# ma921/SOBER

Hardware: AMD Instinct MI355X
Metric: recombination-step candidates/sec (N_rec=100000, N_nys=500, d=10, batch=100) (higher is better)
Workload: dtype f64

## Files before the change

include/sober_hip.h:

```cpp
#ifndef SOBER_HIP_H
#define SOBER_HIP_H

#include <stdint.h>

#ifdef __cplusplus
extern "C" {
#endif

#define SOBER_ABI_VERSION 7

#define SOBER_KIND_RBF       0
#define SOBER_KIND_MATERN52  1
#define SOBER_KIND_TANIMOTO  2

#define SOBER_E_ARG      -1
#define SOBER_E_DIM      -2
#define SOBER_E_WS       -3
#define SOBER_E_EXCHANGE -5

int sober_abi_version(void);
int sober_diag_build(void);
int sober_reload_switches(void);
int sober_level_job_size(void);
int sober_nystrom_job_size(void);

int sober_padded_dim(int d);
int sober_bit_words(int d);

int sober_mt19937_uniform53(uint8_t* state, int64_t state_bytes, int64_t numel, double* out);
int sober_box_muller(const double* u, int64_t numel, double* out, void* stream);

int sober_scale_points(const double* X, int64_t n, int d, int64_t ldx,
                       const double* lengthscale, int ls_len,
                       double* out, int dt, void* stream);

int sober_scale_points_idx(const double* X, const int32_t* idx, int64_t n, int d, int64_t ldx, const double* lengthscale,
                           int ls_len, double* out, int dt, const double* gather_src, double* gather_out, void* stream);
int sober_pack_bits(const double* X, int64_t n, int d, int64_t ldx,
                    uint64_t* words, int nwords, double* norms, int32_t* bad_flag, void* stream);

int sober_pairwise(int kind, const void* a, const double* a_norm, int64_t m,
                   const void* b, const double* b_norm, const int32_t* idx, int64_t n,
                   int dt, double outputscale, double* out, int64_t ldo, void* stream);

int sober_kernel_matvec(int kind, const void* a, const double* a_norm, const double* v, int64_t m,
                        const void* b, const double* b_norm, int64_t n,
                        int dt, double outputscale, double c0, double* out, void* stream);

int sober_level_reduce(int kind, const void* rows, const double* rows_norm, int n_rows,
                       const void* cand, const double* cand_norm, int dt,
                       const int32_t* idx, int64_t pos0, int64_t count, int S,
                       const double* mu, const double* wmul, double outputscale,
                       int n_chunks, double* partG, int ldg, int col0,
                       double* partTot, int64_t tot_limit, void* stream);
int sober_aug_dim(int d);
int sober_augment_plan(const double* X_nys, int64_t M, int64_t ld_nys, const double* X_obs, int64_t n_obs, int64_t ld_obs,
                       const double* X_cand, int64_t N, int64_t ld_cand, int d, const double* lengthscale, int ls_len,
                       double* center, double* rows_aug, double* cand_aug, int da, void* stream);
int sober_augment_points(const double* X, int64_t n, int d, int64_t ldx, const double* lengthscale,
                         int ls_len, const double* center, int side, double* out, int da, void* stream);
int sober_level_reduce_mfma(int kind, const double* rows, int n_rows, const double* cand, int da,
                            const int32_t* idx, int64_t pos0, int64_t count, int S,
                            const double* mu, const double* wmul, double outputscale,
                            int n_chunks, double* partG, int ldg, int col0,
                            double* partTot, int64_t tot_limit, void* stream);

int64_t sober_nonzero_ws_bytes(int64_t N);
int sober_nonzero_i32(const double* mu, int64_t N, int32_t* idx_out, int64_t* count_out, void* ws, int64_t ws_bytes,
                      void* stream);

int sober_level_chunks(int n_rows, int64_t pos0, int64_t count, int S);
int sober_level_parts_mfma(int n_rows, int64_t pos0, int64_t count, int S);
int sober_level_parts_mfma_cap(int n_rows, int64_t e_total_ub, int S);

int sober_sum_partials(const double* partG, const double* partTot, int n_chunks, int n_rows,
                       int ldg, int S, const double* extraG, const double* extraTot,
                       int n_xchunks, int n_xcols, double* G, int ldo, double* tot, void* stream);

int sober_dgemm(int transa, int transb, int m, int n, int k, double alpha,
                const double* A, int lda, const double* B, int ldb,
                double beta, double* C, int ldc, void* stream);

int sober_barycentres(const double* Xtr, int ldx, int n, int S, const double* tot,
                      double* X_tmp, void* stream);
int sober_dgemm_coldiv_t(int m, int n, int k, const double* A, int lda, const double* B, int ldb, const double* coldiv,
                         double* Ct, int ldct, void* stream);

int sober_level_update(const int32_t* idx_cur, int64_t pos0, int64_t count, int S, int64_t E,
                       const int32_t* keep_rank, const double* w_star, const double* tot,
                       int n_keep, double* mu, int32_t* idx_new, int64_t new_pos0, void* stream);

int sober_scatter_weights(const int32_t* idx_cur, const int32_t* sel, const double* w, int n_sel,
                          double* mu, int64_t* out_idx, void* stream);

int sober_gather_f64(const double* src, const int32_t* idx, int64_t n, double* out, void* stream);
int sober_final_scatter(const int32_t* idx, int n, const int32_t* keep_rank, const double* w_star,
                        int64_t row_offset, double* mu, int64_t* out_idx, double* out_w, void* stream);
int sober_final_commit(const int32_t* idx, int n, const int32_t* keep_rank, const double* w_star, const int32_t* n_keep,
                       int64_t row_offset, double* mu, int64_t N, int64_t* out_idx, double* out_w, void* stream);

int sober_i64_to_i32(const int64_t* in, int64_t n, int32_t* out, void* stream);

int sober_car_pivot_host(double* h_Phi, int N, int m, double* h_mu);
int sober_car_pivot_host_fast(double* h_Phi, int N, int m, double* h_mu);

int sober_car_supported(int N, int m);
int64_t sober_car_ws_bytes(int N, int m);
int sober_car_device(const double* X, int ldx, int N, int m, const double* mu_in,
                     int32_t* keep_rank, double* w_star, int32_t* n_keep, double* mu_out,
                     double* phi_out, void* ws, int64_t ws_bytes, void* stream);
int sober_probe_rcp(const double* x, double* out, int64_t n, void* stream);

#define SOBER_CAR_DEFAULT 0
#define SOBER_CAR_SAFE 1
int sober_car_safe_supported(int N, int m);
int sober_car_giveup_forced(void);
int sober_car_device_ex(const double* X, int ldx, int N, int m, const double* mu_in,
                        int32_t* keep_rank, double* w_star, int32_t* n_keep, double* mu_out,
                        double* phi_out, void* ws, int64_t ws_bytes, int mode, void* stream);
int sober_obj_set_sums(const double* obj, const double* mu, const int32_t* idx, int64_t pos0, int64_t count, int S, int64_t E,
                       double* out, void* stream);
int sober_second_elimination(const double* phi, const double* objp, const double* w1, const int32_t* rank1, int n1,
                             int Nsets, int32_t* keep_rank, double* w_star, int32_t* n_keep, void* stream);
int sober_null_vector_supported(int nfun);
int sober_null_vector(const double* X, int ldx, int Nsets, int nfun, const int32_t* rank1, const int32_t* n_keep1, int n1,
                      double* null_row, int32_t* status, void* stream);
int sober_second_elimination_rows(const double* null_row, const double* obj_row, const double* w1, const int32_t* rank1,
                                  const int32_t* n_keep1, const int32_t* status, int n1, int Nsets, int32_t* keep_rank,
                                  double* w_star, int32_t* n_keep, void* stream);
int sober_obj_set_sums_queued(const double* obj, const double* mu, const int32_t* idx, int S, const int64_t* dR, int64_t R_known,
                              const double* tot, double* xcol, int ldx, double* ocol, void* stream);

int sober_car_mc_supported(int N, int m);
int64_t sober_car_mc_ws_bytes(int N, int m);
int sober_car_mc_device(const double* X, int ldx, int N, int m, const double* mu_in,
                        int32_t* keep_rank, double* w_star, int32_t* n_keep, double* mu_out,
                        double* phi_out, void* ws, int64_t ws_bytes, void* stream);
int sober_car_big_supported(int N, int m);
int64_t sober_car_big_ws_bytes(int N, int m);
int sober_car_big_device(const double* X, int ldx, int N, int m, const double* mu_in,
                         int32_t* keep_rank, double* w_star, int32_t* n_keep, double* mu_out,
                         double* phi_out, void* ws, int64_t ws_bytes, void* stream);
int sober_mc_selftest(const double* in, double* out, void* stream);

int sober_chol_max_n(void);
int sober_nystrom_max_n(void);
int sober_cholesky_probe_batched(const double* src, int n, int ld_src, const double* shifts, int n_shifts,
                                 double* work, int32_t* info, double* min_pivot, void* xinv_ws, int64_t ws_bytes,
                                 void* stream);
int sober_cholesky(double* A, int n, int ld, double shift, int32_t* info, double* min_pivot, void* stream);
int sober_cholesky_inv(double* A, int n, int ld, double shift, int32_t* info, double* min_pivot, double* xinv,
                       void* stream);
int sober_cholesky_inv_ratio(double* A, int n, int ld, double shift, int32_t* info, double* min_pivot, double* xinv,
                             double* ratio_out, void* stream);
int sober_trsm_blocks(const double* Y, int64_t m, int q, int ldy, const double* L, int ldl, const double* Xinv,
                      double* Q, int ldq, void* stream);
int sober_cholesky_probe(const double* src, int n, int ld_src, const double* shifts, int n_shifts,
                         double* work, int32_t* info, void* stream);
int sober_cholesky_probe_piv(const double* src, int n, int ld_src, const double* shifts, int n_shifts,
                             double* work, int32_t* info, double* min_pivot, void* stream);

int64_t sober_cholesky_probe_mc_ws_bytes(int n, int n_shifts);
int sober_cholesky_probe_mc(const double* src, int n, int ld_src, const double* shifts, int n_shifts,
                            double* work, int32_t* info, double* min_pivot, void* ws, int64_t ws_bytes,
// ... 235 lines not shown
```

sober_amd/_engine.py:

```python
from __future__ import annotations

import os
import time
import warnings
from typing import Optional

import numpy as np
import torch

from . import _native as nat
from ._utils import SafeTensorOperator


class SoloComm:
    rank, world = 0, 1

    def allreduce_sum(self, *tensors):
        return

    def allgather_counts(self, n: int):
        return [n]

    def allgather_rows(self, t: torch.Tensor, counts):
        return t
# ... 165 lines not shown
    ES = E * S
    if p <= ES:
        return (p // S) * n_keep + kept_prefix[p % S]
    return E * n_keep + ((p - ES) if last_kept else 0)


class RecombinationEngine:
    def __init__(self, ops, comm=None, row_offset: int = 0):
        self.ops = ops
        self.comm = comm or SoloComm()
        self.row_offset = int(row_offset)
        self.tm = SafeTensorOperator()
        self.trace = None
        self.timers = {}
        self.force_host_car = False
        self.force_host_nystrom = False
        self.basis_override = None
        self.cutover_R = int(os.environ.get("SOBER_CUTOVER_R", "32768"))
        self.force_sharded = bool(os.environ.get("SOBER_FORCE_SHARDED"))

    def _tick(self, name, t0):
        t1 = time.perf_counter()
        self.timers[name] = self.timers.get(name, 0.0) + (t1 - t0)
        return t1

    def nystrom_basis(self, plan, s: int, overlap=None, literal=False, early=None):
        if self.basis_override is not None:
            return self.basis_override
        t0 = time.perf_counter()
        dev_route = getattr(self.ops, "nystrom_basis_device", None)
        if dev_route is not None and not self.force_host_nystrom and not literal:
            res = dev_route(plan, s, self.tm.max_iter, overlap, early) if (overlap is not None or early is not None) \
                else dev_route(plan, s, self.tm.max_iter)
            if res is not None:
                U, gram = res
                self._tick("nystrom_device", t0)
                if self.trace is not None:
                    (gram_h, U_h) = self.ops.to_host(gram, U)
                    self.trace.update(gram=gram_h, U=U_h)
                return U
        gram = self.ops.gram(plan)
        (gram_h,) = self.ops.to_host(gram)
        t0 = self._tick("gram_device", t0)
        _, U = ker_svd_sparsify_host(gram_h, s, self.tm)
        self._tick("nystrom_host", t0)
        if self.trace is not None:
            self.trace.update(gram=gram_h.clone(), U=U.clone())
        return U

    def run(self, plan, mu: torch.Tensor, num_pts: int, obj: Optional[torch.Tensor] = None, live=None):
        ops, comm = self.ops, self.comm
        self.obj = obj
        self.obj_head = None
        if obj is not None:
            head = obj[:2 * num_pts].clone()
            if comm.world > 1:
                cnt = comm.allgather_counts(int(head.numel()))
                head = comm.allgather_rows(head, cnt)[:2 * num_pts]
            self.obj_head = head
        n = num_pts - 1
        S = 2 * (n + 1)
        state = {}
        can_start = getattr(ops, "nonzero_start", None) is not None and live is None
        pend = {}

        def start_list():
            if can_start and "p" not in pend:
                pend["p"] = ops.nonzero_start(mu)
        sharded = comm.world > 1 or (self.force_sharded and getattr(comm, "native_allreduce", None) is not None)

        def first_sums():
            if live is not None:
                idx_cur, count = live, int(live.numel())
            else:
                start_list()
                idx_cur, count = ops.nonzero_finish(pend["p"]) if "p" in pend else ops.nonzero_i32(mu)
            counts = comm.allgather_counts(count)
            bounds = [0]
            for c in counts:
                bounds.append(bounds[-1] + c)
            state.update(idx_cur=idx_cur, count=count, pos0=bounds[comm.rank], R=bounds[-1], bounds=bounds)
            cut = sharded and obj is None and self.cutover_R > 0 and state["R"] <= self.cutover_R
            if state["R"] > S and getattr(ops, "level_car", None) is not None and count > 0 and not cut:
                ops.level_moments(plan, idx_cur, state["pos0"], count, S, state["R"] // S, mu, phase=1, n=n)
                state["sums_ready"] = True

        def head_once():
            if not state:
                first_sums()

        n_fun = n + 1 + (1 if obj is not None else 0)
        car_on_host = self.force_host_car or getattr(ops, "car_supported", None) is None \
            or not ops.car_supported(S, n_fun) or (obj is not None and getattr(ops, "car_obj_device", None) is None)
        if car_on_host and not self.force_host_car and getattr(ops, "size_cliff", None) is not None \
                and getattr(ops, "car_supported", None) is not None and not ops.car_supported(S, n_fun):
            ops.size_cliff("car", f"batch = {n + 1}: a Caratheodory step on 2 x batch = {S} points with {n_fun} test functions is beyond "
                                  "the device kernels (registers of one compute unit: batch <= 100, of nine: batch <= 224, memory-resident: "
                                  "2 x batch <= 2048); every level's step runs on host LAPACK + the C++ pivots instead -- seconds per level")
        if comm.world > 1:
            start_list()
        U = self.nystrom_basis(plan, n, overlap=head_once if comm.world == 1 else None, literal=car_on_host,
                               early=start_list if comm.world == 1 else None)
        if comm.world > 1:
            U = comm.broadcast0(ops.from_host(U.contiguous()) if U.device != ops.device else U.contiguous())
            if hasattr(plan, "_proj_src"):
                plan._proj_src = None
        ops.set_projection(plan, U)
        head_once()
        idx_cur, count, pos0, R = state["idx_cur"], state["count"], state["pos0"], state["R"]
        bounds = state["bounds"]
        sums_ready = state.get("sums_ready", False)
        idx_new = ops.empty_i32(count)
        levels = [] if self.trace is not None else None

        if self.trace is not None:
            self.trace["levels"] = levels
        if not sharded and obj is None and levels is None and not self.force_host_car and R > S \
                and getattr(ops, "level_loop", None) is not None and ops.car_supported(S, n + 1):
            t0 = time.perf_counter()
            idx_cur, idx_new, R = ops.level_loop(plan, idx_cur, idx_new, R, S, mu, sums_ready, self.row_offset)
            pos0, count, bounds, sums_ready = 0, R, [0, R], False
            self._tick("levels_device", t0)
        elif not sharded and obj is not None and levels is None and not self.force_host_car and R > S \
                and getattr(ops, "level_loop_obj", None) is not None:
            t0 = time.perf_counter()
            res = ops.level_loop_obj(plan, idx_cur, idx_new, R, S, mu, obj, sums_ready)
            if res is not None and res[3] > 0:
                idx_cur, idx_new, R = res[:3]
                pos0, count, bounds, sums_ready = 0, R, [0, R], False
            self._tick("levels_device", t0)
        elif sharded and obj is None and levels is None and not self.force_host_car and R > S \
                and getattr(ops, "level_loop_sharded", None) is not None and ops.car_supported(S, n + 1) \
                and getattr(comm, "native_allreduce", None) is not None:
            t0 = time.perf_counter()
            idx_cur, idx_new, bounds = ops.level_loop_sharded(plan, idx_cur, idx_new, bounds, S, mu, sums_ready, comm,
                                                              self.cutover_R)
            R, pos0, count, sums_ready = bounds[-1], bounds[comm.rank], bounds[comm.rank + 1] - bounds[comm.rank], False
            self._tick("levels_device", t0)
            if R > S:
                return self._finish_replicated(plan, idx_cur, bounds, mu, num_pts, U)
        while True:
            if R <= n + 1:
                return self._finish_small(mu)
            if R <= S:
                return self._finish_direct(plan, idx_cur, bounds, R, mu, levels)

            E = R // S
            r = R - E * S
            t0 = time.perf_counter()
            if sums_ready:
                Xtr, tot = ops.level_moments(plan, idx_cur, pos0, count, S, E, mu, phase=2)
                sums_ready = False
            else:
                Xtr, tot = ops.level_moments(plan, idx_cur, pos0, count, S, E, mu)
            if obj is None:
                flat = getattr(ops, "level_flat", None)
                if flat is not None:
                    comm.allreduce_sum(flat(plan))
                else:
                    comm.allreduce_sum(Xtr, tot)
            else:
                orow = self._obj_set_sums(obj, mu, idx_cur, pos0, count, S, E)
                comm.allreduce_sum(Xtr, tot, orow)
                Xtr = torch.cat([Xtr, orow.unsqueeze(0)], 0)
            if obj is None and not self.force_host_car and getattr(ops, "level_car", None) is not None \
                    and ops.car_supported(S, n + 1):
                res = ops.level_car(plan, S)
# ... 169 lines not shown
```

sober_amd/_native.py:

```python
from __future__ import annotations

import ctypes as C
import os
from typing import Optional

import torch

_HERE = os.path.dirname(os.path.abspath(__file__))
LIB_PATH = os.environ.get("SOBER_HIP_LIB") or os.path.join(_HERE, "libsober_hip.so")
ABI_VERSION = 7

KIND_RBF, KIND_MATERN52, KIND_TANIMOTO = 0, 1, 2
KIND_BY_NAME = {"rbf": KIND_RBF, "matern52": KIND_MATERN52, "tanimoto": KIND_TANIMOTO}

_vp, _i32, _i64, _f64 = C.c_void_p, C.c_int, C.c_int64, C.c_double

SIGNATURES = {
    "sober_abi_version": (_i32, []),
    "sober_diag_build": (_i32, []),
    "sober_reload_switches": (_i32, []),
    "sober_level_job_size": (_i32, []),
    "sober_nystrom_job_size": (_i32, []),
    "sober_final_job_size": (_i32, []),
    "sober_set_i64": (_i32, [_vp, _i64, _vp]),
    "sober_rank_scatter": (_i32, [_vp, _i32, _i32, _i32, _vp, _vp, _i32, _vp, _vp, _vp]),
    "sober_plan_rows": (_i32, [_i32, _vp, _i32, _i64, _vp, _i32, _i64, _i32, _vp, _i32, _f64, _vp, _i32, _vp, _i32, _vp,
                               _vp, _vp, _vp, _vp]),
    "sober_level_loop_final": (_i32, [_vp, _vp, _i64, _vp, _vp, _i32, _vp, _i32, _vp, _vp, _vp, _vp, _vp]),
    "sober_padded_dim": (_i32, [_i32]),
    "sober_bit_words": (_i32, [_i32]),
    "sober_scale_points": (_i32, [_vp, _i64, _i32, _i64, _vp, _i32, _vp, _i32, _vp]),
    "sober_augment_plan": (_i32, [_vp, _i64, _i64, _vp, _i64, _i64, _vp, _i64, _i64, _i32, _vp, _i32, _vp, _vp, _vp, _i32, _vp]),
    "sober_scale_points_idx": (_i32, [_vp, _vp, _i64, _i32, _i64, _vp, _i32, _vp, _i32, _vp, _vp, _vp]),
    "sober_pack_bits": (_i32, [_vp, _i64, _i32, _i64, _vp, _i32, _vp, _vp, _vp]),
    "sober_mt19937_uniform53": (_i32, [_vp, _i64, _i64, _vp]),
    "sober_box_muller": (_i32, [_vp, _i64, _vp, _vp]),
    "sober_pairwise": (_i32, [_i32, _vp, _vp, _i64, _vp, _vp, _vp, _i64, _i32, _f64, _vp, _i64, _vp]),
    "sober_kernel_matvec": (_i32, [_i32, _vp, _vp, _vp, _i64, _vp, _vp, _i64, _i32, _f64, _f64, _vp, _vp]),
    "sober_level_reduce": (_i32, [_i32, _vp, _vp, _i32, _vp, _vp, _i32, _vp, _i64, _i64, _i32, _vp, _vp,
                                  _f64, _i32, _vp, _i32, _i32, _vp, _i64, _vp]),
    "sober_nonzero_ws_bytes": (_i64, [_i64]),
    "sober_nonzero_i32": (_i32, [_vp, _i64, _vp, _vp, _vp, _i64, _vp]),
    "sober_dgemm_coldiv_t": (_i32, [_i32, _i32, _i32, _vp, _i32, _vp, _i32, _vp, _vp, _i32, _vp]),
    "sober_level_chunks": (_i32, [_i32, _i64, _i64, _i32]),
    "sober_level_parts_mfma": (_i32, [_i32, _i64, _i64, _i32]),
    "sober_level_parts_mfma_cap": (_i32, [_i32, _i64, _i32]),
    "sober_aug_dim": (_i32, [_i32]),
    "sober_augment_points": (_i32, [_vp, _i64, _i32, _i64, _vp, _i32, _vp, _i32, _vp, _i32, _vp]),
    "sober_level_reduce_mfma": (_i32, [_i32, _vp, _i32, _vp, _i32, _vp, _i64, _i64, _i32, _vp, _vp, _f64, _i32,
                                       _vp, _i32, _i32, _vp, _i64, _vp]),
    "sober_sum_partials": (_i32, [_vp, _vp, _i32, _i32, _i32, _i32, _vp, _vp, _i32, _i32, _vp, _i32, _vp, _vp]),
    "sober_dgemm": (_i32, [_i32, _i32, _i32, _i32, _i32, _f64, _vp, _i32, _vp, _i32, _f64, _vp, _i32, _vp]),
    "sober_barycentres": (_i32, [_vp, _i32, _i32, _i32, _vp, _vp, _vp]),
    "sober_level_update": (_i32, [_vp, _i64, _i64, _i32, _i64, _vp, _vp, _vp, _i32, _vp, _vp, _i64, _vp]),
    "sober_scatter_weights": (_i32, [_vp, _vp, _vp, _i32, _vp, _vp, _vp]),
    "sober_i64_to_i32": (_i32, [_vp, _i64, _vp, _vp]),
    "sober_car_pivot_host": (_i32, [_vp, _i32, _i32, _vp]),
    "sober_car_pivot_host_fast": (_i32, [_vp, _i32, _i32, _vp]),
    "sober_car_supported": (_i32, [_i32, _i32]),
    "sober_car_ws_bytes": (_i64, [_i32, _i32]),
    "sober_car_device": (_i32, [_vp, _i32, _i32, _i32, _vp, _vp, _vp, _vp, _vp, _vp, _vp, _i64, _vp]),
    "sober_probe_rcp": (_i32, [_vp, _vp, _i64, _vp]),
    "sober_second_elimination": (_i32, [_vp, _vp, _vp, _vp, _i32, _i32, _vp, _vp, _vp, _vp]),
    "sober_car_mc_supported": (_i32, [_i32, _i32]),
    "sober_car_mc_ws_bytes": (_i64, [_i32, _i32]),
    "sober_car_mc_device": (_i32, [_vp, _i32, _i32, _i32, _vp, _vp, _vp, _vp, _vp, _vp, _vp, _i64, _vp]),
    "sober_car_big_supported": (_i32, [_i32, _i32]),
    "sober_car_big_ws_bytes": (_i64, [_i32, _i32]),
    "sober_car_big_device": (_i32, [_vp, _i32, _i32, _i32, _vp, _vp, _vp, _vp, _vp, _vp, _vp, _i64, _vp]),
    "sober_car_device_ex": (_i32, [_vp, _i32, _i32, _i32, _vp, _vp, _vp, _vp, _vp, _vp, _vp, _i64, _i32, _vp]),
    "sober_obj_set_sums": (_i32, [_vp, _vp, _vp, _i64, _i64, _i32, _i64, _vp, _vp]),
    "sober_null_vector_supported": (_i32, [_i32]),
    "sober_null_vector": (_i32, [_vp, _i32, _i32, _i32, _vp, _vp, _i32, _vp, _vp, _vp]),
    "sober_second_elimination_rows": (_i32, [_vp, _vp, _vp, _vp, _vp, _vp, _i32, _i32, _vp, _vp, _vp, _vp]),
    "sober_obj_set_sums_queued": (_i32, [_vp, _vp, _vp, _i32, _vp, _i64, _vp, _vp, _i32, _vp, _vp]),
    "sober_obj_job_size": (_i32, []),
    "sober_level_loop_obj": (_i32, [_vp, _vp, _i64, _vp, _vp, _i32, _i32, _vp, _vp, _vp, _vp, _vp]),
    "sober_car_safe_supported": (_i32, [_i32, _i32]),
    "sober_car_giveup_forced": (_i32, []),
    "sober_final_commit": (_i32, [_vp, _i32, _vp, _vp, _vp, _i64, _vp, _i64, _vp, _vp, _vp]),
    "sober_level_car_retry": (_i32, [_vp, _vp]),
    "sober_mc_selftest": (_i32, [_vp, _vp, _vp]),
    "sober_chol_max_n": (_i32, []),
    "sober_nystrom_max_n": (_i32, []),
    "sober_cholesky_probe_batched": (_i32, [_vp, _i32, _i32, _vp, _i32, _vp, _vp, _vp, _vp, _i64, _vp]),
    "sober_cholesky": (_i32, [_vp, _i32, _i32, _f64, _vp, _vp, _vp]),
    "sober_cholesky_inv": (_i32, [_vp, _i32, _i32, _f64, _vp, _vp, _vp, _vp]),
    "sober_cholesky_inv_ratio": (_i32, [_vp, _i32, _i32, _f64, _vp, _vp, _vp, _vp, _vp]),
    "sober_trsm_blocks": (_i32, [_vp, _i64, _i32, _i32, _vp, _i32, _vp, _vp, _i32, _vp]),
    "sober_cholesky_probe": (_i32, [_vp, _i32, _i32, _vp, _i32, _vp, _vp, _vp]),
    "sober_cholesky_probe_piv": (_i32, [_vp, _i32, _i32, _vp, _i32, _vp, _vp, _vp, _vp]),
    "sober_cholesky_probe_mc_ws_bytes": (_i64, [_i32, _i32]),
    "sober_cholesky_probe_mc": (_i32, [_vp, _i32, _i32, _vp, _i32, _vp, _vp, _vp, _vp, _i64, _vp]),
    "sober_abs_sym": (_i32, [_vp, _i32, _i32, _vp, _i32, _vp, _vp]),
    "sober_abs_sym_dmax": (_i32, [_vp, _i32, _i32, _vp, _i32, _vp, _vp, _vp]),
    "sober_jitter_ladder": (_i32, [_vp, _i32, _i32, _i32, _vp]),
    "sober_jitter_ladder_auto": (_i32, [_vp, _i32, _i32, _vp, _i32, _vp, _vp]),
    "sober_kmeans_ws_bytes": (_i64, [_i64, _i32, _i32]),
    "sober_kmeans_stat_offset": (_i64, [_i64, _i32, _i32]),
    "sober_kmeans_ws_bytes_screened": (_i64, [_i64, _i32, _i32]),
    "sober_kmeans_lloyd": (_i32, [_vp, _i64, _i32, _i32, _i32, _vp, _vp, _vp, _i64, _vp]),
    "sober_predict_fused_supported": (_i32, [_i32, _i32, _i32]),
    "sober_predict_fused": (_i32, [_i32, _vp, _vp, _i32, _vp, _vp, _i64, _i32, _f64, _vp, _i32, _vp, _f64, _f64, _f64, _vp, _vp,
                                   _f64, _vp, _vp, _i32, _vp]),
    "sober_predict_fused_root": (_i32, [_i32, _vp, _vp, _i32, _vp, _vp, _i64, _i32, _f64, _vp, _i32, _vp, _vp, _f64, _f64, _f64, _vp,
                                        _vp, _f64, _vp, _vp, _i32, _vp]),
    "sober_predict_finish": (_i32, [_vp, _vp, _i32, _i64, _i64, _vp, _f64, _vp, _f64, _f64, _vp, _f64, _vp, _i32, _vp]),
    "sober_reduce_ws_bytes": (_i64, [_i64]),
    "sober_cleansing_weights": (_i32, [_vp, _i64, _f64, _vp, _i64, _vp]),
    "sober_level_gather": (_i32, [_vp, _i32, _i64, _vp, _i64, _i64, _i32, _vp, _vp, _i32, _vp, _i32, _i32, _vp, _i64,
                                  _vp]),
    "sober_gspace_finish": (_i32, [_vp, _vp, _i64, _i32, _i64, _i64, _vp, _vp, _vp]),
    "sober_wkde_draw": (_i32, [_vp, _i64, _i32, _vp, _vp, _i32, _vp, _vp, _vp, _vp, _vp, _vp]),
    "sober_level_moments": (_i32, [_vp, _vp]),
    "sober_level_car": (_i32, [_vp, _vp]),
    "sober_level_reduce_tani_supported": (_i32, [_i32]),
    "sober_level_reduce_tani": (_i32, [_vp, _vp, _i32, _vp, _vp, _i32, _vp, _i64, _i64, _i32, _vp, _vp, _f64, _i32, _vp,
                                       _i32, _i32, _vp, _i64, _vp]),
    "sober_level_loop_sharded": (_i32, [_vp, _i32, _i32, _vp, _vp, _vp, _i32, _vp, _vp, _i64, _i32, _vp, _vp, _vp, _vp]),
    "sober_rccl_load": (_i32, [C.c_char_p]),
    "sober_rccl_unique_id": (_i32, [_vp]),
    "sober_rccl_comm_init": (_i32, [_vp, _i32, _i32, _vp]),
    "sober_rccl_comm_destroy": (_i32, [_vp]),
    "sober_rccl_allreduce_f64": (_i32, [_vp, _vp, _i64, _vp]),
    "sober_rccl_allreduce_ptr": (_i64, []),
    "sober_peer_region_bytes": (_i64, [_i64]),
    "sober_peer_create": (_i32, [_i32, _i32, _i64, _vp, _vp]),
    "sober_peer_connect": (_i32, [_vp, C.c_char_p]),
    "sober_peer_connect_ptrs": (_i32, [_vp, _vp]),
    "sober_peer_region": (_i64, [_vp]),
    "sober_peer_set_spin_limit": (_i32, [_vp, C.c_uint]),
    "sober_peer_allreduce_f64": (_i32, [_vp, _vp, _i64, _vp]),
    "sober_peer_allreduce_ptr": (_i64, []),
    "sober_peer_status": (_i32, [_vp, _vp, _i64, _vp]),
    "sober_peer_destroy": (_i32, [_vp]),
# ... 175 lines not shown

def fused_dim_supported(kind: int, d: int) -> bool:
    r = load().sober_bit_words(d) if kind == KIND_TANIMOTO else load().sober_padded_dim(d)
    return r > 0


def scale_points_idx(X, idx, n, lengthscale, out):
    _req(lengthscale, torch.float64, "lengthscale"); _req(out, torch.float64, "out"); _req(idx, torch.int32, "idx")
    if X.dtype != torch.float64 or X.stride(-1) != 1:
        raise SoberHipError("scale_points_idx: X must be float64 with unit inner stride")
    _check(load().sober_scale_points_idx(X.data_ptr(), idx.data_ptr(), int(n), X.shape[1], X.stride(0), lengthscale.data_ptr(),
                                         lengthscale.numel(), out.data_ptr(), out.shape[1], None, None, _stream(X)),
           "sober_scale_points_idx")


def scale_points(X, lengthscale, out):
    n, d = X.shape
    _req(X, torch.float64, "X"); _req(lengthscale, torch.float64, "lengthscale"); _req(out, torch.float64, "out")
    _check(load().sober_scale_points(X.data_ptr(), n, d, X.stride(0), lengthscale.data_ptr(),
                                     lengthscale.numel(), out.data_ptr(), out.shape[1], _stream(X)),
           "sober_scale_points")


def mt19937_uniform53(state, numel, out):
    _req(state, torch.uint8, "state"); _req(out, torch.float64, "out")
    if state.is_cuda or out.is_cuda or out.numel() < numel + 16:
        raise ValueError("mt19937_uniform53 takes host tensors, out of numel + 16 doubles")
    _check(load().sober_mt19937_uniform53(state.data_ptr(), state.numel(), numel, out.data_ptr()),
           "sober_mt19937_uniform53")


def box_muller(u, numel, out):
    _req(u, torch.float64, "u"); _req(out, torch.float64, "out")
    if u.numel() < numel + 16 or out.numel() < numel:
        raise ValueError("box_muller: u holds numel + 16 uniforms, out numel normals")
    _check(load().sober_box_muller(u.data_ptr(), numel, out.data_ptr(), _stream(out)), "sober_box_muller")


def pack_bits(X, words, norms, bad_flag):
    n, d = X.shape
    _req(X, torch.float64, "X"); _req(words, torch.int64, "words"); _req(norms, torch.float64, "norms")
    _req(bad_flag, torch.int32, "bad_flag")
    _check(load().sober_pack_bits(X.data_ptr(), n, d, X.stride(0), words.data_ptr(), words.shape[1],
                                  norms.data_ptr(), bad_flag.data_ptr(), _stream(X)), "sober_pack_bits")


def rank_scatter(X, n, ocol, rank, n1, Xp, objp):
    _req(X, torch.float64, "X"); _req(ocol, torch.float64, "ocol"); _req(rank, torch.int32, "rank")
    _check(load().sober_rank_scatter(X.data_ptr(), X.stride(0), X.shape[0], n, ocol.data_ptr(), rank.data_ptr(), n1,
                                     Xp.data_ptr(), objp.data_ptr(), _stream(X)), "sober_rank_scatter")


def plan_rows(kind, X_nys, X_obs, lengthscale, outputscale, S_cache, rows, Kall, W, T, G):
    M, d = X_nys.shape
    n_obs = 0 if X_obs is None else X_obs.shape[0]
    for t in (X_nys, X_obs, S_cache, rows, Kall, W, T, G):
        if t is not None and (t.dtype != torch.float64 or t.stride(-1) != 1):
            raise SoberHipError("plan_rows: float64 tensors with unit inner stride")
    _check(load().sober_plan_rows(kind, X_nys.data_ptr(), M, X_nys.stride(0), _ptr(X_obs), n_obs,
                                  X_obs.stride(0) if X_obs is not None else 0, d, lengthscale.data_ptr(),
                                  lengthscale.numel(), float(outputscale), _ptr(S_cache),
                                  S_cache.stride(0) if S_cache is not None else 0, rows.data_ptr(), rows.shape[1],
                                  _ptr(Kall), _ptr(W), _ptr(T), G.data_ptr(), _stream(G)), "sober_plan_rows")


def pairwise(kind, a, a_norm, b, b_norm, idx, n, dt, outputscale, out):
    _check(load().sober_pairwise(kind, a.data_ptr(), _ptr(a_norm), a.shape[0], b.data_ptr(), _ptr(b_norm),
                                 _ptr(idx), n, dt, float(outputscale), out.data_ptr(), out.stride(0),
                                 _stream(out)), "sober_pairwise")


def kernel_matvec(kind, a, a_norm, v, b, b_norm, dt, outputscale, c0, out):
    _check(load().sober_kernel_matvec(kind, a.data_ptr(), _ptr(a_norm), v.data_ptr(), a.shape[0],
                                      b.data_ptr(), _ptr(b_norm), b.shape[0], dt, float(outputscale),
                                      float(c0), out.data_ptr(), _stream(out)), "sober_kernel_matvec")


def nonzero_ws_bytes(N) -> int:
    r = load().sober_nonzero_ws_bytes(N)
    _check(min(int(r), 0), "sober_nonzero_ws_bytes")
    return int(r)


def nonzero_i32(mu, idx_out, count_out, ws):
    _req(mu, torch.float64, "mu"); _req(idx_out, torch.int32, "idx_out"); _req(count_out, torch.int64, "count_out")
    _check(load().sober_nonzero_i32(mu.data_ptr(), mu.numel(), idx_out.data_ptr(), count_out.data_ptr(), ws.data_ptr(),
                                    ws.numel() * ws.element_size(), _stream(mu)), "sober_nonzero_i32")


def level_chunks(n_rows, pos0, count, S) -> int:
    r = load().sober_level_chunks(n_rows, pos0, count, S)
    _check(min(r, 0), "sober_level_chunks")
    return r


def level_parts_mfma(n_rows, pos0, count, S) -> int:
    r = load().sober_level_parts_mfma(n_rows, pos0, count, S)
    _check(min(r, 0), "sober_level_parts_mfma")
    return r


def level_reduce(kind, rows, rows_norm, cand, cand_norm, dt, idx, idx_off, pos0, count, S, mu, wmul,
                 outputscale, n_chunks, partG, ldg, col0, partTot, tot_limit):
    _req(idx, torch.int32, "idx"); _req(mu, torch.float64, "mu")
    _check(load().sober_level_reduce(kind, rows.data_ptr(), _ptr(rows_norm), rows.shape[0], cand.data_ptr(),
                                     _ptr(cand_norm), dt, idx.data_ptr() + 4 * idx_off, pos0, count, S,
                                     mu.data_ptr(), _ptr(wmul), float(outputscale), n_chunks,
                                     partG.data_ptr(), ldg, col0, _ptr(partTot), tot_limit, _stream(mu)),
           "sober_level_reduce")


def aug_dim(d: int) -> int:
    r = load().sober_aug_dim(d)
    return r if r > 0 else -1


def augment_plan(X_nys, X_obs, X_cand, lengthscale, center, rows_aug, cand_aug):
    for t_, nm in ((X_nys, "X_nys"), (X_cand, "X_cand"), (X_obs, "X_obs")):
        if t_ is not None and (t_.dtype != torch.float64 or t_.stride(-1) != 1):
            raise SoberHipError(f"augment_plan: {nm} must be float64 with unit inner stride")
    _req(rows_aug, torch.float64, "rows_aug"); _req(cand_aug, torch.float64, "cand_aug"); _req(center, torch.float64, "center")
    n_obs = 0 if X_obs is None else X_obs.shape[0]
    _check(load().sober_augment_plan(X_nys.data_ptr(), X_nys.shape[0], X_nys.stride(0), _ptr(X_obs), n_obs,
                                     X_obs.stride(0) if n_obs else 0, X_cand.data_ptr(), X_cand.shape[0], X_cand.stride(0),
                                     X_nys.shape[1], lengthscale.data_ptr(), lengthscale.numel(), center.data_ptr(),
                                     rows_aug.data_ptr(), cand_aug.data_ptr(), rows_aug.shape[1], _stream(X_cand)),
           "sober_augment_plan")


def augment_points(X, lengthscale, center, side, out):
    n, d = X.shape
    _req(X, torch.float64, "X"); _req(out, torch.float64, "out"); _req(center, torch.float64, "center")
    _check(load().sober_augment_points(X.data_ptr(), n, d, X.stride(0), lengthscale.data_ptr(),
                                       lengthscale.numel(), center.data_ptr(), side, out.data_ptr(),
                                       out.shape[1], _stream(X)), "sober_augment_points")


def level_reduce_mfma(kind, rows, cand, da, idx, idx_off, pos0, count, S, mu, wmul, outputscale, n_chunks,
                      partG, ldg, col0, partTot, tot_limit):
    _req(idx, torch.int32, "idx"); _req(mu, torch.float64, "mu")
    _check(load().sober_level_reduce_mfma(kind, rows.data_ptr(), rows.shape[0], cand.data_ptr(), da,
                                          idx.data_ptr() + 4 * idx_off, pos0, count, S, mu.data_ptr(),
                                          _ptr(wmul), float(outputscale), n_chunks, partG.data_ptr(), ldg,
                                          col0, _ptr(partTot), tot_limit, _stream(mu)),
           "sober_level_reduce_mfma")


def sum_partials(partG, partTot, n_chunks, n_rows, ldg, S, extraG, extraTot, n_xchunks, n_xcols, G, tot):
    _check(load().sober_sum_partials(partG.data_ptr(), _ptr(partTot), n_chunks, n_rows, ldg, S,
                                     _ptr(extraG), _ptr(extraTot), n_xchunks, n_xcols, G.data_ptr(),
                                     G.stride(0), _ptr(tot), _stream(G)), "sober_sum_partials")


def dgemm(A, B, C_, transa=False, transb=False, alpha=1.0, beta=0.0):
    m, n = C_.shape
    k = A.shape[0] if transa else A.shape[1]
    for t, nm in ((A, "A"), (B, "B"), (C_, "C")):
        if t.dtype != torch.float64 or t.stride(1) != 1:
            raise SoberHipError(f"dgemm {nm}: need float64 with unit inner stride")
    ka = B.shape[1] if transb else B.shape[0]
    ma = A.shape[1] if transa else A.shape[0]
    na = B.shape[0] if transb else B.shape[1]
    if (ma, na, ka) != (m, n, k):
        raise SoberHipError(f"dgemm shape mismatch {A.shape} {B.shape} -> {C_.shape}")
    _check(load().sober_dgemm(int(transa), int(transb), m, n, k, float(alpha), A.data_ptr(), A.stride(0),
                              B.data_ptr(), B.stride(0), float(beta), C_.data_ptr(), C_.stride(0),
                              _stream(C_)), "sober_dgemm")


def barycentres(Xtr, n, S, tot, X_tmp):
# ... 456 lines not shown
```

sober_amd/_ops_hip.py:

```python
from __future__ import annotations

import os
import warnings

import torch

from . import _native as nat
from ._ops_levels import _LevelOps
from ._ops_nystrom import _NystromOps
from ._ops_plan import Plan, _PlanOps


class HipOps(_PlanOps, _NystromOps, _LevelOps):
    name = "hip"

    def __init__(self, device):
        self.device = torch.device(device)
        if self.device.type != "cuda":
            raise nat.SoberHipError("sober_amd needs a HIP device (torch device 'cuda'); got "
                                    f"{self.device}.  There is no CPU fallback.")
        nat.load()
        self._pin = {}
        self.prof = None
        self.use_mfma = True
        self.queue_levels = os.environ.get("SOBER_NO_QUEUE") is None
        self.level_classes = True
        self.obj_null_kernel = True
        self.queue_obj_levels = True
        self.lazy_scaled_pool = True
        self.last_levels = None
        self._probe_mc = torch.cuda.get_device_properties(self.device).multi_processor_count >= 256
        self.car_mode = nat.CAR_DEFAULT

    def size_cliff(self, which: str, message: str):
        seen = self.__dict__.setdefault("_cliffs_seen", set())
        if which not in seen:
            seen.add(which)
            import warnings
            warnings.warn("sober_amd: " + message, RuntimeWarning, stacklevel=3)

    def prof_reserve(self, n_pairs: int):
        pool = getattr(self, "_ev_pool", None)
        if pool is None:
            pool = self._ev_pool = []
        st = torch.cuda.current_stream(self.device)
        for _ in range(n_pairs):
            e0, e1 = torch.cuda.Event(enable_timing=True), torch.cuda.Event(enable_timing=True)
            e0.record(st); e1.record(st)
            pool.append((e0, e1))

    def _prof_pair(self):
        pool = getattr(self, "_ev_pool", None)
        if not pool:
            self.prof_reserve(1)
            pool = self._ev_pool
        return pool.pop()

    def _buf(self, p, name, numel):
        t = p.ws.get(name)
        if t is None or t.numel() < numel:
            t = torch.empty(numel, dtype=torch.float64, device=self.device)
            p.ws[name] = t
        return t

    def _buf_u8(self, p, name, nbytes):
        t = p.ws.get(name)
        if t is None or t.numel() < nbytes:
            t = torch.empty(max(nbytes, 8), dtype=torch.uint8, device=self.device)
            p.ws[name] = t
        return t

    def nonzero_start(self, mu):
        N = mu.numel()
        key = ("nz", N)
        bufs = self._pin.get(key)
        if bufs is None:
            ws = torch.zeros(nat.nonzero_ws_bytes(N), dtype=torch.uint8, device=self.device)
            bufs = self._pin[key] = (ws, torch.zeros(1, dtype=torch.int64, device=self.device),
                                     torch.zeros(1, dtype=torch.int64).pin_memory())
        ws, cnt, pin = bufs
        out = torch.empty(N, dtype=torch.int32, device=self.device)
        nat.nonzero_i32(mu, out, cnt, ws)
        pin.copy_(cnt, non_blocking=True)
        ev = torch.cuda.Event()
        ev.record(torch.cuda.current_stream(self.device))
        return out, pin, ev

    def nonzero_finish(self, pending):
        out, pin, ev = pending
        ev.synchronize()
        return out, int(pin[0])

    def nonzero_i32(self, mu):
        nz = torch.nonzero(mu != 0).flatten()
        out = torch.empty(max(nz.numel(), 1), dtype=torch.int32, device=self.device)
        if nz.numel():
            nat.i64_to_i32(nz, out)
        return out, int(nz.numel())

    def empty_i32(self, n):
        return torch.empty(max(n, 1), dtype=torch.int32, device=self.device)

    def to_host(self, *tensors, before_sync=None):
        outs = []
        for i, t in enumerate(tensors):
            key = (i, t.dtype, tuple(t.shape))
            buf = self._pin.get(key)
            if buf is None:
                buf = torch.empty(t.shape, dtype=t.dtype, pin_memory=True)
                self._pin[key] = buf
            buf.copy_(t, non_blocking=True)
            outs.append(buf)
        if before_sync is None:
            torch.cuda.current_stream(self.device).synchronize()
        else:
            ev = torch.cuda.Event()
            ev.record(torch.cuda.current_stream(self.device))
            before_sync()
            ev.synchronize()
        return [o.clone() for o in outs]

    def from_host(self, t, dtype=None):
        return t.to(self.device, dtype=dtype, non_blocking=False)


class MatrixKernelOps(HipOps):

    CHUNK_ROWS = 1 << 15

    def build_plan(self, kernel_fn, mode, X_nys, X_cand, pool_owner=None) -> Plan:
        p = Plan()
        p.kernel_fn, p.mode = kernel_fn, "matrix"
        p.X_nys, p.X_cand = X_nys, X_cand
        p.M = p.Mtot = X_nys.shape[0]
        p.weighted, p.T, p.P, p.wmul, p.da = False, None, None, None, -1
        p.ws = {}
        N = X_cand.shape[0]
        if hasattr(kernel_fn, "materialise"):
            p.Kmat = kernel_fn.materialise(X_cand, X_nys)
        else:
            p.Kmat = torch.empty(N, p.M, dtype=torch.float64, device=self.device)
            for lo in range(0, N, self.CHUNK_ROWS):
                hi = min(N, lo + self.CHUNK_ROWS)
                p.Kmat[lo:hi] = kernel_fn(X_nys, X_cand[lo:hi]).to(torch.float64).T
        if tuple(p.Kmat.shape) != (N, p.M) or p.Kmat.dtype != torch.float64 or p.Kmat.stride(1) != 1:
            raise nat.SoberHipError(f"kernel matrix must be ({N}, {p.M}) float64 row-major, got "
                                    f"{tuple(p.Kmat.shape)} {p.Kmat.dtype}")
        return p

    def gram(self, p):
        if hasattr(p.kernel_fn, "materialise"):
            return p.kernel_fn.materialise(p.X_nys, p.X_nys, gram=True)
        return p.kernel_fn(p.X_nys, p.X_nys).to(torch.float64).contiguous()

    def set_projection(self, p, U):
        p.P = U.to(self.device, torch.float64).contiguous()
        p.n = p.P.shape[0]

    def direct_columns(self, p, idx, count):
        Kc = p.Kmat[idx[:count].long()].contiguous()
        Xtr = torch.empty(p.n, count, dtype=torch.float64, device=self.device)
        nat.dgemm(p.P, Kc, Xtr, transb=True)
        out = torch.empty(count, p.n, dtype=torch.float64, device=self.device)
        nat.barycentres(Xtr, p.n, count, None, out)
        return out

# ... 3 lines not shown
```

sober_amd/_ops_levels.py:

```python
from __future__ import annotations

import warnings

import torch

from . import _native as nat
from ._ops_plan import Plan


class _LevelOps:

    def _job(self, p: Plan, S: int, n: int = None) -> nat.LevelJob:
        n = p.n if n is None else n
        job = p.ws.get("job")
        if job is not None and job.S == S and job.n == n:
            if p.P is not None and job.P != p.P.data_ptr():
                if p.P.stride(0) != p.Mtot or p.P.stride(1) != 1:
                    p.P = p.P.contiguous()
                job.P = p.P.data_ptr()
            job.car_mode = min(self.car_mode, nat.CAR_SAFE)
            return job
        dev, f64 = self.device, torch.float64
        job = nat.LevelJob()
        Kmat = getattr(p, "Kmat", None)
        if Kmat is not None:
            job.variant, job.kind = nat.LEVEL_GATHER, 0
            job.cand, job.kmat_ld, job.n_rows = Kmat.data_ptr(), Kmat.stride(0), Kmat.shape[1]
            job.outputscale = 1.0
        elif p.da > 0:
            job.variant, job.kind = nat.LEVEL_MFMA, p.kind
            job.rows, job.cand, job.dim, job.n_rows = p.rows_aug.data_ptr(), p.cand_aug.data_ptr(), p.da, p.Mtot
            job.outputscale = float(p.spec.outputscale)
        else:
            tani = p.kind == nat.KIND_TANIMOTO and self.use_mfma and bool(nat.load().sober_level_reduce_tani_supported(p.rows.dt))
            job.variant, job.kind = (nat.LEVEL_TANI if tani else nat.LEVEL_VALU), p.kind
            job.rows, job.rows_norm = p.rows.data.data_ptr(), nat._ptr(p.rows.norm)
            job.cand, job.cand_norm = p.cand.data.data_ptr(), nat._ptr(p.cand.norm)
            job.dim, job.n_rows = p.rows.dt, p.Mtot
            job.outputscale = float(p.spec.outputscale)
        job.wmul = nat._ptr(p.wmul)
        if p.P is not None and (p.P.stride(0) != p.Mtot or p.P.stride(1) != 1):
            p.P = p.P.contiguous()
        job.S, job.n, job.P = S, n, nat._ptr(p.P)
        nr, mc, xs = job.n_rows, nat.LEVEL_MAX_CHUNKS, nat.LEVEL_XS
        w = p.ws
        w["partG"], w["partTot"] = torch.empty(mc * nr * S, dtype=f64, device=dev), torch.empty(mc * S, dtype=f64, device=dev)
        w["extraG"], w["extraTot"] = torch.empty(mc * nr * xs, dtype=f64, device=dev), torch.empty(mc * xs, dtype=f64, device=dev)
        w["G"] = torch.empty(nr, S, dtype=f64, device=dev)
        w["XT"] = torch.empty(n * S + S, dtype=f64, device=dev)
        w["Xtr"], w["tot"] = w["XT"][:n * S].view(n, S), w["XT"][n * S:]
        w["X_tmp"] = torch.empty(S, n, dtype=f64, device=dev)
        w["keep_rank"] = torch.empty(S + 1, dtype=torch.int32, device=dev)
        w["w_star"], w["mu_out"] = torch.empty(S, dtype=f64, device=dev), torch.empty(S, dtype=f64, device=dev)
        w["h_flags"] = torch.empty(S + 1, dtype=torch.int32, pin_memory=True)
        w["h_flags_np"] = w["h_flags"].numpy()
        if job.variant in (nat.LEVEL_MFMA, nat.LEVEL_TANI) and self.queue_levels:
            w["dR"] = torch.empty(nat.LEVEL_QUEUE + 1, dtype=torch.int64, device=dev)
            w["h_dR"] = torch.zeros(nat.LEVEL_QUEUE + 1, dtype=torch.int64, pin_memory=True)
            job.dR, job.h_dR = w["dR"].data_ptr(), w["h_dR"].data_ptr()
            if S % 2 == 0:
                cl = 1 << nat.CLASS_MAX_DEPTH
                w["Gc"] = [torch.empty(nr * S * (cl >> k), dtype=f64, device=dev) for k in (0, 1)]
                w["totc"] = [torch.empty(S * (cl >> k), dtype=f64, device=dev) for k in (0, 1)]
                w["cls_scale"], w["cls_sof"] = torch.empty(S, dtype=f64, device=dev), torch.empty(S, dtype=torch.int32, device=dev)
                for k in (0, 1):
                    job.Gc[k], job.totc[k] = w["Gc"][k].data_ptr(), w["totc"][k].data_ptr()
                job.cls_scale, job.cls_sof = w["cls_scale"].data_ptr(), w["cls_sof"].data_ptr()
        for k in ("partG", "partTot", "extraG", "extraTot", "G", "Xtr", "tot", "X_tmp", "keep_rank", "w_star", "mu_out",
                  "h_flags"):
            setattr(job, k, w[k].data_ptr())
        if nat.car_supported(S, n + 1):
            nbytes = nat.car_ws_bytes(S, n + 1)
            w["car_ws"] = torch.empty(max(nbytes // 8, 1), dtype=f64, device=dev)
            job.car_ws, job.car_ws_bytes = w["car_ws"].data_ptr(), nbytes
        job.car_mode = min(self.car_mode, nat.CAR_SAFE)
        w["job"] = job
        return job

    def _car_downgrade(self, mode: int, why: str):
        if mode > self.car_mode:
            self.car_mode = mode
            warnings.warn("sober_amd: a multi-workgroup Caratheodory launch gave up waiting for its partner workgroups "
                          f"({why}); this and the following steps use "
                          + ("the kernels without such waits (one workgroup, or a launch per dependency beyond batch 100)" if mode == nat.CAR_SAFE
                             else "the host LAPACK route")
                          + " for that step -- same result, slower")

    def level_moments(self, p: Plan, idx, pos0, count, S, E, mu, phase: int = 0, n: int = None):
        job = self._job(p, S, n)
        job.phase = phase
        if count <= 0 and phase != 2:
            p.ws["XT"].zero_(); p.ws["G"].zero_()
            return p.ws["Xtr"], p.ws["tot"]
        if phase == 2:
            nat.level_moments(job, nat._stream(p.ws["G"]))
            return p.ws["Xtr"], p.ws["tot"]
        nat._req(idx, torch.int32, "idx"); nat._req(mu, torch.float64, "mu")
        job.idx, job.pos0, job.count, job.E, job.mu = idx.data_ptr(), pos0, count, E, mu.data_ptr()
        job.class_depth = 0
        if phase == 1 and pos0 == 0 and count == E * S and job.Gc[0] and job.dR and self.level_classes:
            job.class_depth = int(nat.load().sober_level_class_depth(job.variant, job.n_rows, count, S))
        pair = None
        if self.prof is not None:
            n_left = max(pos0 + count - max(pos0, E * S), 0)
            pair, pair2 = self._prof_pair(), (self._prof_pair() if n_left > 0 else None)
            job.ev[0], job.ev[1] = pair[0].cuda_event, pair[1].cuda_event
            job.ev[2], job.ev[3] = (pair2[0].cuda_event, pair2[1].cuda_event) if pair2 else (None, None)
        nat.level_moments(job, nat._stream(mu))
        if pair is not None:
            self.prof.append((pair[0], pair[1], int(count * job.n_rows), 1))
            if pair2 is not None:
                self.prof.append((pair2[0], pair2[1], int(n_left * job.n_rows), 1))
            for k in range(4):
                job.ev[k] = None
        return p.ws["Xtr"], p.ws["tot"]

    def level_loop_obj(self, p: Plan, idx_cur, idx_new, R: int, S: int, mu, obj, sums_ready: bool):
        job = self._job(p, S)
        n = job.n
        if not self.queue_obj_levels or not self.queue_levels or not job.dR or job.variant not in (nat.LEVEL_MFMA, nat.LEVEL_TANI):
            return None
        if self.car_mode == nat.CAR_HOST or not self.obj_null_kernel or not self.car_supported(S, n + 2) \
                or not bool(nat.load().sober_null_vector_supported(n)):
            return None
        nat._req(mu, torch.float64, "mu"); nat._req(idx_cur, torch.int32, "idx"); nat._req(idx_new, torch.int32, "idx")
        nat._req(obj, torch.float64, "obj")
        dev, f64, w = self.device, torch.float64, p.ws
        if "obj_job" not in w:
            oj = nat.ObjJob()
            w["obj_X"] = torch.empty(S, n + 1, dtype=f64, device=dev)
            w["obj_f"] = torch.empty(3, S, dtype=f64, device=dev)
            w["obj_i"] = torch.empty(S + 2, dtype=torch.int32, device=dev)
            nbytes = nat.car_ws_bytes(S, n + 2)
            w["obj_car_ws"] = (torch.empty(max(nbytes // 8, 1), dtype=f64, device=dev), nbytes)
            oj.X_tmp, oj.ocol, oj.w1, oj.null_row = (w["obj_X"].data_ptr(), w["obj_f"][0].data_ptr(), w["obj_f"][1].data_ptr(),
                                                       w["obj_f"][2].data_ptr())
            oj.kr1, oj.nk1, oj.status = w["obj_i"].data_ptr(), w["obj_i"][S:].data_ptr(), w["obj_i"][S + 1:].data_ptr()
            w["obj_job"] = oj
        oj = w["obj_job"]
        oj.obj = obj.data_ptr()
        job.mu = mu.data_ptr()
        saved = (job.car_ws, job.car_ws_bytes, job.class_depth)
        job.car_ws, job.car_ws_bytes, job.class_depth = w["obj_car_ws"][0].data_ptr(), w["obj_car_ws"][1], 0
        try:
            level_R, R_final, in_b = nat.level_loop_obj(job, oj, R, idx_cur, idx_new, sums_ready, nat._stream(mu))
        finally:
            job.car_ws, job.car_ws_bytes, job.class_depth = saved
        if in_b:
            idx_cur, idx_new = idx_new, idx_cur
        return idx_cur, idx_new, R_final, len(level_R)

    def level_loop(self, p: Plan, idx_cur, idx_new, R: int, S: int, mu, sums_ready: bool, row_offset: int = 0):
        import math
        job = self._job(p, S)
        nat._req(mu, torch.float64, "mu"); nat._req(idx_cur, torch.int32, "idx"); nat._req(idx_new, torch.int32, "idx")
        job.mu = mu.data_ptr()
        if not sums_ready:
            job.class_depth = 0
        events = pairs = None
        if self.prof is not None:
            n_max = min(nat.MAX_LEVELS, int(math.log2(max(R / S, 1.0))) + 3)
            pairs = [(self._prof_pair(), self._prof_pair()) for _ in range(n_max)]
            events = [None] * (4 * nat.MAX_LEVELS)
            for l, (a, b) in enumerate(pairs):
                events[4 * l:4 * l + 4] = [a[0].cuda_event, a[1].cuda_event, b[0].cuda_event, b[1].cuda_event]
        fin = None
        p.ws.pop("final_done", None)
        if not p.weighted and getattr(p, "Kmat", None) is None and self.car_mode != nat.CAR_HOST and job.car_ws:
            fin = self._final_job(p, S, mu, row_offset)
        level_R, R_final, in_b, gave_up = nat.level_loop(job, R, idx_cur, idx_new, sums_ready, events, nat._stream(mu), fin)
        self.last_levels = {"R": [int(v) for v in level_R], "derived": int(job.class_depth) if sums_ready else 0}
        if fin is not None and fin.done:
            n_keep = int(p.ws["h_flags_np"][S])
            if n_keep >= 0:
                lst = idx_new if in_b else idx_cur
                p.ws["final_done"] = (lst.data_ptr(), R_final, row_offset, p._fin_out[0][:n_keep], p._fin_out[1][:n_keep])
        if job.car_mode > min(self.car_mode, nat.CAR_SAFE):
            self._car_downgrade(nat.CAR_SAFE, "level loop")
        if gave_up:
            self._car_downgrade(nat.CAR_HOST, "level loop")
        if pairs is not None:
            for l, (a, b) in enumerate(pairs):
                Rl = level_R[l] if l < len(level_R) else 0
# ... 210 lines not shown
```

sober_amd/_ops_nystrom.py:

```python
from __future__ import annotations

import os
import warnings

import torch

from . import _native as nat
from . import _rng
from ._ops_plan import Plan


class _NystromOps:

    NITER = 2

    def nystrom_basis_device(self, p: Plan, s: int, max_iter: int = 10, overlap=None, early=None):
        dev, M = self.device, p.M
        if M > nat.nystrom_max_n() or s > 2 * nat.chol_max_n() or s >= M:
            if s < M:
                self.size_cliff("nystrom", f"N_nys = {M}, batch = {s + 1}: beyond the device Nystrom route (N_nys <= "
                                           f"{nat.nystrom_max_n()}, batch <= {2 * nat.chol_max_n() + 1}); make_cov_psd and svd_lowrank run on host LAPACK "
                                           "instead -- about 5-10x the device route's time for this phase")
            self.gram(p)
            return None
        G = self.gram(p)
        n_r, niter = max_iter + 1, self.NITER
        n_orth2 = 2 * (1 + 2 * niter)
        if getattr(p, "ws", None) is None:
            p.ws = {}
        key = ("nys", M, s, n_r)
        st = self._pin.get(key)
        if st is None:
            f64 = torch.float64
            nbytes = nat.nystrom_flags_bytes(n_r, niter)
            st = self._pin[key] = {
                "job": nat.NystromJob(), "C": torch.empty(M, M, dtype=f64, device=dev),
                "Y0": torch.empty(M, s, dtype=f64, device=dev), "Y1": torch.empty(M, s, dtype=f64, device=dev),
                "Gm": torch.empty(s, s, dtype=f64, device=dev),
                "xinv": torch.empty(((s + 31) // 32) * 1024, dtype=f64, device=dev),
                "flags": torch.empty(nbytes, dtype=torch.uint8, device=dev),
                "h_flags": torch.empty(nbytes, dtype=torch.uint8, pin_memory=True),
                "Ut": torch.empty(s, M, dtype=f64, device=dev),
            }
            skey = ("shifts", n_r)
            if skey not in self._pin:
                self._pin[skey] = torch.tensor([1e-5 * (2 ** k - 1) for k in range(n_r)], dtype=f64, device=dev)
            j = st["job"]
            j.M, j.s, j.n_rungs, j.niter = M, s, n_r, niter
            j.shifts, j.C = self._pin[skey].data_ptr(), st["C"].data_ptr()
            j.Y[0], j.Y[1], j.Gm, j.xinv = st["Y0"].data_ptr(), st["Y1"].data_ptr(), st["Gm"].data_ptr(), st["xinv"].data_ptr()
            j.flags_block, j.flags_bytes, j.h_flags_block = st["flags"].data_ptr(), nbytes, st["h_flags"].data_ptr()
            j.Ut = st["Ut"].data_ptr()
        j = st["job"]
        work = self._buf(p, "chol_work", n_r * M * M)
        j.G, j.chol_work = G.data_ptr(), work.data_ptr()
        j.probe_mc = 1 if (M >= self.PROBE_MC_MIN and n_r <= 16 and self._probe_mc and M <= nat.chol_max_n()) else 0
        if j.probe_mc:
            pws = self._buf_u8(p, "chol_mc_ws", nat.cholesky_probe_mc_ws_bytes(M, n_r))
            j.probe_ws, j.probe_ws_bytes = pws.data_ptr(), pws.numel()
        elif M > nat.chol_max_n():
            pws = self._buf_u8(p, "chol_cb_ws", n_r * 8192)
            j.probe_ws, j.probe_ws_bytes = pws.data_ptr(), pws.numel()
        proj = hasattr(p, "weighted")
        if proj:
            T = p.T
            P = torch.empty(s, p.Mtot if T is not None else M, dtype=torch.float64, device=dev)
            j.T, j.n_obs = nat._ptr(T), (T.shape[1] if T is not None else 0)
            j.mean_nys, j.P = (p.mean_nys.data_ptr() if p.weighted else None), P.data_ptr()
        else:
            j.P = None
        stream = torch.cuda.current_stream(dev)
        nat.nystrom_basis(j, 1, stream.cuda_stream)
        if early is not None:
            early()
        rng_state = torch.get_rng_state()
        R = _rng.device_randn(M, s, dev)
        j.R = R.data_ptr()
        nat.nystrom_basis(j, 2, stream.cuda_stream)
        ev = torch.cuda.Event()
        ev.record(stream)
        Ut = st["Ut"]
        if proj:
            p.P, p.n, p._proj_src = P, s, Ut
        if overlap is not None:
            overlap()
        ev.synchronize()
        hb = st["h_flags"]
        n8 = 8 * (n_r + 1 + n_orth2)
        f64s, i32s = hb[:n8].view(torch.float64), hb[n8:].view(torch.int32)
        piv_h, pivs_rf = f64s[:n_r + 1], f64s[n_r + 1:n_r + 1 + n_orth2]
        flags_h, infos_rf = i32s[:2 + n_r], i32s[2 + n_r:]
        if any(int(v) == nat.PROBE_NO_VERDICT for v in flags_h[2:]):
            self._probe_mc = False
            warnings.warn("sober_amd: the multi-CU Cholesky probe lost contact between its workgroups; "
                          "falling back to one workgroup per rung")
            torch.set_rng_state(rng_state)
            return None
        last = 2 * niter
        if os.environ.get("SOBER_NYSTROM_DEBUG"):
            print("nystrom: pivot ratios of the range finder's blocks", [float(pivs_rf[k + 1]) for k in range(0, n_orth2, 2)])
        single = [k for k in range(0, n_orth2, 2) if k // 2 != last]
        rank_lost = bool((infos_rf != 0).any()) or float(pivs_rf[2 * last + 1]) < 0.5 \
            or any(not (float(pivs_rf[k + 1]) >= self.ORTH1_MIN_RATIO) for k in single)
        if int(flags_h[0]) == 0 or rank_lost or self.ladder_borderline(flags_h[2:], piv_h[:n_r], float(piv_h[n_r])):
            torch.set_rng_state(rng_state)
            return None
        warnings.warn("Estimated covariance matrix was not positive semi-definite. Conveting...")
        return Ut, G

    LADDER_GUARD = 1e-9
    PROBE_MC_MIN = 160

    @classmethod
    def ladder_borderline(cls, info, min_pivot, dmax) -> bool:
        thr = cls.LADDER_GUARD * max(dmax, 0.0)
        ok = [int(v) == 0 for v in info]
        piv = [float(v) for v in min_pivot]
        if not (dmax == dmax) or any(v != v for v in piv):
            return True
        k = ok.index(True) if any(ok) else len(ok)
        if k < len(ok) and piv[k] < thr:
            return True
        if k > 0 and piv[k - 1] > -thr:
            return True
# ... 18 lines not shown
```

sober_amd/csrc/compact.hip:

```cpp
#include "common.hpp"

namespace sober {

constexpr int NZ_T = 256, NZ_PER = 8, NZ_TILE = NZ_T * NZ_PER;
constexpr unsigned long long NZ_LOCAL = 1ull << 32, NZ_INCL = 2ull << 32;

__device__ __forceinline__ int nz_wave_sum(int v) {
#pragma unroll
    for (int o = 32; o > 0; o >>= 1) v += __shfl_xor(v, o);
    return v;
}

__global__ __launch_bounds__(NZ_T) void k_nonzero(const double* __restrict__ mu, int64_t N, int32_t* __restrict__ out,
                                                  int64_t* __restrict__ count_out, unsigned long long* __restrict__ ws, int nb) {
    __shared__ int s_tile, s_total, s_prefix, s_last;
    __shared__ int s_cnt[NZ_PER * 4];
    if (threadIdx.x == 0) s_tile = (int)atomicAdd((unsigned*)ws, 1u);
    __syncthreads();
    const int tile = s_tile;
    const int lane = threadIdx.x & 63, w = threadIdx.x >> 6;
    const int64_t base = (int64_t)tile * NZ_TILE;
    unsigned long long m[NZ_PER];
#pragma unroll
    for (int k = 0; k < NZ_PER; ++k) {
        const int64_t i = base + k * NZ_T + threadIdx.x;
        const bool nz = i < N && mu[i] != 0.0;
        m[k] = __ballot(nz);
        if (lane == 0) s_cnt[k * 4 + w] = __popcll(m[k]);
    }
    __syncthreads();
    unsigned long long* status = ws + 2;
    if (w == 0) {
        const int v = lane < NZ_PER * 4 ? s_cnt[lane] : 0;
        int incl = v;
#pragma unroll
        for (int o = 1; o < NZ_PER * 4; o <<= 1) {
            const int u = __shfl_up(incl, o);
            if (lane >= o) incl += u;
        }
        if (lane < NZ_PER * 4) s_cnt[lane] = incl - v;
        const int total = __shfl(incl, NZ_PER * 4 - 1);
        int run = 0;
        if (tile == 0) {
            if (lane == 0) __hip_atomic_store(status, NZ_INCL | (unsigned long long)total, __ATOMIC_RELEASE, __HIP_MEMORY_SCOPE_AGENT);
        } else {
            if (lane == 0)
                __hip_atomic_store(status + tile, NZ_LOCAL | (unsigned long long)total, __ATOMIC_RELEASE, __HIP_MEMORY_SCOPE_AGENT);
            for (int p = tile - 1; p >= 0; p -= 64) {
                const int q = p - lane;
                unsigned long long st = 0;
                if (q >= 0) {
                    do st = __hip_atomic_load(status + q, __ATOMIC_RELAXED, __HIP_MEMORY_SCOPE_AGENT); while ((st >> 32) == 0);
                }
                const unsigned long long bi = __ballot(q >= 0 && (st >> 32) == 2);
                if (bi != 0) {
                    const int first = __ffsll((long long)bi) - 1;
                    run += nz_wave_sum(lane <= first ? (int)(unsigned)st : 0);
                    break;
                }
                run += nz_wave_sum(q >= 0 ? (int)(unsigned)st : 0);
            }
            if (lane == 0)
                __hip_atomic_store(status + tile, NZ_INCL | (unsigned long long)(run + total), __ATOMIC_RELEASE, __HIP_MEMORY_SCOPE_AGENT);
        }
        if (lane == 0) { s_prefix = run; s_total = total; }
    }
    __syncthreads();
    const int prefix = s_prefix;
#pragma unroll
    for (int k = 0; k < NZ_PER; ++k) {
        if ((m[k] >> lane) & 1ull)
            out[prefix + s_cnt[k * 4 + w] + __popcll(m[k] & ((1ull << lane) - 1ull))] = (int32_t)(base + k * NZ_T + threadIdx.x);
    }
    if (threadIdx.x == 0) {
        if (tile == nb - 1) *count_out = (int64_t)prefix + s_total;
        s_last = atomicAdd((unsigned*)(ws + 1), 1u) == (unsigned)(nb - 1);
    }
    __syncthreads();
    if (s_last)
        for (int t = threadIdx.x; t < nb + 2; t += NZ_T) ws[t] = 0ull;
}

}

extern "C" int64_t sober_nonzero_ws_bytes(int64_t N) {
    if (N <= 0 || N > 0x7fffffffLL) return SOBER_E_ARG;
    const int64_t nb = (N + sober::NZ_TILE - 1) / sober::NZ_TILE;
    return ((2 + nb) * 8 + 255) / 256 * 256;
}

extern "C" int sober_nonzero_i32(const double* mu, int64_t N, int32_t* idx_out, int64_t* count_out, void* ws,
                                 int64_t ws_bytes, void* stream) {
    if (!mu || !idx_out || !count_out || !ws || N <= 0 || N > 0x7fffffffLL) return SOBER_E_ARG;
    if (ws_bytes < sober_nonzero_ws_bytes(N)) return SOBER_E_WS;
    const int nb = (int)((N + sober::NZ_TILE - 1) / sober::NZ_TILE);
    hipLaunchKernelGGL(sober::k_nonzero, dim3((unsigned)nb), dim3(sober::NZ_T), 0, (hipStream_t)stream, mu, N, idx_out, count_out,
                       (unsigned long long*)ws, nb);
    LAUNCH_CHECK();
    return 0;
}
```

sober_amd/csrc/dgemm.hip:

```cpp
#include "common.hpp"

namespace sober {

typedef double double4_t __attribute__((ext_vector_type(4)));

__device__ __forceinline__ double ld_op(const double* M, int ld, int trans, int r, int c, int R, int C) {
    const bool ok = (r < R) & (c < C);
    const int rc = min(r, R - 1), cc = min(c, C - 1);
    const double v = trans ? M[(size_t)cc * ld + rc] : M[(size_t)rc * ld + cc];
    return ok ? v : 0.0;
}

template <int SPLIT>
__global__ __launch_bounds__(256) void k_dgemm(int transa, int transb, int m, int n, int k,
                                               double alpha, const double* __restrict__ A, int lda,
                                               const double* __restrict__ B, int ldb, double beta,
                                               double* __restrict__ C, int ldc,
                                               const double* __restrict__ coldiv, double* __restrict__ Ct, int ldct) {
    __shared__ double red[SPLIT == 4 ? 3 * 256 : 1];
    const int wave = threadIdx.x >> 6, lane = threadIdx.x & 63;
    int i0, j0, kbeg, kend;
    if constexpr (SPLIT == 4) {
        i0 = blockIdx.y * 16;
        j0 = blockIdx.x * 16;
        const int kq = (((k + 3) / 4) + 15) / 16 * 16;
        kbeg = min(wave * kq, k);
        kend = min(kbeg + kq, k);
    } else {
        i0 = blockIdx.y * 32 + (wave >> 1) * 16;
        j0 = blockIdx.x * 32 + (wave & 1) * 16;
        kbeg = 0;
        kend = k;
        if (i0 >= m || j0 >= n) return;
    }
    const int li = lane & 15, lk = lane >> 4;

    double4_t acc = (double4_t){0.0, 0.0, 0.0, 0.0};
    double af[4], bf[4], an[4], bn[4];
#define DG_LOAD(AF, BF, K0)                                                                   \
    _Pragma("unroll") for (int u = 0; u < 4; ++u) {                                           \
        AF[u] = ld_op(A, lda, transa, i0 + li, (K0) + 4 * u + lk, m, kend);                   \
        BF[u] = ld_op(B, ldb, transb, (K0) + 4 * u + lk, j0 + li, kend, n);                   \
    }
    DG_LOAD(af, bf, kbeg)
    for (int k0 = kbeg; k0 < kend; k0 += 16) {
        DG_LOAD(an, bn, k0 + 16)
#pragma unroll
        for (int u = 0; u < 4; ++u)
            acc = __builtin_amdgcn_mfma_f64_16x16x4f64(af[u], bf[u], acc, 0, 0, 0);
#pragma unroll
        for (int u = 0; u < 4; ++u) { af[u] = an[u]; bf[u] = bn[u]; }
    }
#undef DG_LOAD
    if constexpr (SPLIT == 4) {
        if (wave > 0) {
#pragma unroll
            for (int r = 0; r < 4; ++r) red[(wave - 1) * 256 + r * 64 + lane] = acc[r];
        }
        __syncthreads();
        if (wave > 0) return;
#pragma unroll
        for (int r = 0; r < 4; ++r) acc[r] = ((acc[r] + red[r * 64 + lane]) + red[256 + r * 64 + lane]) + red[512 + r * 64 + lane];
    }
#pragma unroll
    for (int r = 0; r < 4; ++r) {
        const int row = i0 + lk + 4 * r;
        const int col = j0 + li;
        if (row < m && col < n) {
            const double v = alpha * acc[r];
            if (Ct != nullptr) {
                Ct[(size_t)col * ldct + row] = coldiv ? v / coldiv[col] : v;
            } else {
                double* c = C + (size_t)row * ldc + col;
                *c = (beta == 0.0) ? v : fma(beta, *c, v);
            }
        }
    }
}

}

extern "C" int sober_dgemm(int transa, int transb, int m, int n, int k, double alpha, const double* A,
                           int lda, const double* B, int ldb, double beta, double* C, int ldc,
                           void* stream) {
    if (!A || !B || !C || m <= 0 || n <= 0 || k <= 0) return SOBER_E_ARG;
    if (lda < (transa ? m : k) || ldb < (transb ? k : n) || ldc < n) return SOBER_E_ARG;
    const long tiles = (long)((n + 15) / 16) * ((m + 15) / 16);
    if (tiles <= 2048 && k >= 64) {
        dim3 grid((n + 15) / 16, (m + 15) / 16);
        hipLaunchKernelGGL(sober::k_dgemm<4>, grid, dim3(256), 0, (hipStream_t)stream, transa, transb, m, n, k,
                           alpha, A, lda, B, ldb, beta, C, ldc, (const double*)nullptr, (double*)nullptr, 0);
    } else {
        dim3 grid((n + 31) / 32, (m + 31) / 32);
        hipLaunchKernelGGL(sober::k_dgemm<1>, grid, dim3(256), 0, (hipStream_t)stream, transa, transb, m, n, k,
                           alpha, A, lda, B, ldb, beta, C, ldc, (const double*)nullptr, (double*)nullptr, 0);
    }
    LAUNCH_CHECK();
    return 0;
}

extern "C" int sober_dgemm_coldiv_t(int m, int n, int k, const double* A, int lda, const double* B, int ldb,
                                    const double* coldiv, double* Ct, int ldct, void* stream) {
    if (!A || !B || !Ct || m <= 0 || n <= 0 || k <= 0 || lda < k || ldb < n || ldct < m) return SOBER_E_ARG;
    const long tiles = (long)((n + 15) / 16) * ((m + 15) / 16);
    if (tiles <= 2048 && k >= 64) {
        dim3 grid((n + 15) / 16, (m + 15) / 16);
        hipLaunchKernelGGL(sober::k_dgemm<4>, grid, dim3(256), 0, (hipStream_t)stream, 0, 0, m, n, k, 1.0, A, lda, B, ldb,
                           0.0, (double*)nullptr, 0, coldiv, Ct, ldct);
    } else {
        dim3 grid((n + 31) / 32, (m + 31) / 32);
        hipLaunchKernelGGL(sober::k_dgemm<1>, grid, dim3(256), 0, (hipStream_t)stream, 0, 0, m, n, k, 1.0, A, lda, B, ldb,
                           0.0, (double*)nullptr, 0, coldiv, Ct, ldct);
    }
    LAUNCH_CHECK();
    return 0;
}
```

sober_amd/csrc/internal.hpp:

```cpp
#pragma once
#include <cstdint>

namespace sober {

int scale_points2(const double* Xa, int64_t na, int64_t lda, const double* Xb, int64_t nb, int64_t ldb, int d,
                  const double* lengthscale, int ls_len, double* out, int dt, void* stream);

int transpose_projection(const double* Q, int s, int M, const double* mean, double* Ut, double* P, int ldp, void* stream);

int64_t probe_mc_flag_bytes(int n_shifts);
int nystrom_flags_init(void* flags_block, int64_t flags_bytes, void* probe_ws, int64_t ws_flag_bytes, int32_t* info,
                       int n_info, void* stream);
int cholesky_probe_mc(const double* src, int n, int ld_src, const double* shifts, int n_shifts, double* work, int32_t* info,
                      double* min_pivot, void* ws, int64_t ws_bytes, bool init, void* stream);

int orth_merge(int32_t* info, double* piv, double* ratio, const int32_t* info2, const double* piv2, const double* ratio2, void* stream);

}
```

sober_amd/csrc/level_exec.cpp:

```cpp
#include <hip/hip_runtime.h>
#include <cstdio>
#include <cstdlib>

#include "../../include/sober_hip.h"
#include "switches.hpp"

extern "C" int sober_level_job_size(void) { return (int)sizeof(sober_level_job); }
extern "C" int sober_obj_job_size(void) { return (int)sizeof(sober_obj_job); }

#define LX_TRY(call)                 \
    do {                             \
        const int rc_ = (call);      \
        if (rc_ != 0) return rc_;    \
    } while (0)

static inline bool lx_timed_in_dispatch(const sober_level_job* j) {
    return j->variant == SOBER_LEVEL_MFMA || j->variant == SOBER_LEVEL_TANI;
}
#define LX_EVENTS_BEFORE(A, B)                                                                   \
    if ((A) && (B)) {                                                                            \
        if (lx_timed_in_dispatch(j)) { LX_TRY(sober_set_launch_events((A), (B))); }              \
        else { const hipError_t e_ = hipEventRecord((hipEvent_t)(A), (hipStream_t)stream); if (e_ != hipSuccess) return (int)e_; } \
    }
#define LX_EVENTS_AFTER(A, B)                                                                    \
    if ((A) && (B) && !lx_timed_in_dispatch(j)) {                                                \
        const hipError_t e_ = hipEventRecord((hipEvent_t)(B), (hipStream_t)stream);              \
        if (e_ != hipSuccess) return (int)e_;                                                    \
    }

static int lx_reduce(const sober_level_job* j, const int32_t* idx, int64_t pos0, int64_t count, int S, int n_chunks,
                     double* partG, double* partTot, int64_t tot_limit, void* stream) {
    switch (j->variant) {
        case SOBER_LEVEL_MFMA:
            return sober_level_reduce_mfma(j->kind, (const double*)j->rows, j->n_rows, (const double*)j->cand, j->dim,
                                           idx, pos0, count, S, j->mu, j->wmul, j->outputscale, n_chunks, partG, S, 0,
                                           partTot, tot_limit, stream);
        case SOBER_LEVEL_VALU:
            return sober_level_reduce(j->kind, j->rows, j->rows_norm, j->n_rows, j->cand, j->cand_norm, j->dim, idx,
                                      pos0, count, S, j->mu, j->wmul, j->outputscale, n_chunks, partG, S, 0, partTot,
                                      tot_limit, stream);
        case SOBER_LEVEL_TANI:
            return sober_level_reduce_tani(j->rows, j->rows_norm, j->n_rows, j->cand, j->cand_norm, j->dim, idx, pos0, count,
                                           S, j->mu, j->wmul, j->outputscale, n_chunks, partG, S, 0, partTot, tot_limit,
                                           stream);
        case SOBER_LEVEL_GATHER:
            return sober_level_gather((const double*)j->cand, j->n_rows, j->kmat_ld, idx, pos0, count, S, j->mu,
                                      j->wmul, n_chunks, partG, S, 0, partTot, tot_limit, stream);
        default:
            return SOBER_E_ARG;
    }
}

extern "C" int sober_level_class_depth(int variant, int n_rows, int64_t R, int S) {
    if (n_rows <= 0 || R <= 0 || S <= 0 || (S & 1) || sober::switches().level_no_classes) return 0;
    if (variant != SOBER_LEVEL_MFMA && variant != SOBER_LEVEL_TANI) return 0;
    int D = 0;
    while (D < SOBER_CLASS_MAX_DEPTH) {
        const int64_t SC = (int64_t)S << (D + 1);
        if (R % SC != 0 || R / SC < 2) break;
        int slots;
        if (variant == SOBER_LEVEL_MFMA) {
            const int wpt = sober_level_class_wpt(n_rows, R / SC, (int)SC);
            slots = wpt > 0 ? sober_level_class_slots(wpt) : 0;
        } else {
            slots = sober_level_chunks_tani(n_rows, 0, R, (int)SC);
            const int64_t rb = (n_rows + 255) / 256;
            const int64_t wg_c = (int64_t)slots * ((SC + 15) / 16 + 1) * rb;
            const int64_t wg_0 = (int64_t)sober_level_chunks_tani(n_rows, 0, R, S) * ((S + 15) / 16 + 1) * rb;
            if (slots > 0 && wg_c * 100 < wg_0 * 85) break;
        }
        if (slots <= 0 || slots * (1 << (D + 1)) > SOBER_LEVEL_MAX_CHUNKS) break;
        ++D;
    }
    return D;
}

static int lx_class_first(const sober_level_job* j, void* stream) {
    const int S = j->S, D = j->class_depth, CL = 1 << D, SC = S * CL;
    if ((j->variant != SOBER_LEVEL_MFMA && j->variant != SOBER_LEVEL_TANI) || D < 1 || D > SOBER_CLASS_MAX_DEPTH ||
        j->pos0 != 0 || j->count % SC != 0 || j->count / SC < 2 || !j->Gc[0] || !j->totc[0])
        return SOBER_E_ARG;
    int nch;
    if (j->variant == SOBER_LEVEL_MFMA) {
        const int wpt = sober_level_class_wpt(j->n_rows, j->count / SC, SC);
        if (wpt <= 0) return wpt < 0 ? wpt : SOBER_E_ARG;
        nch = sober_level_class_slots(wpt);
        if (nch <= 0 || nch * CL > SOBER_LEVEL_MAX_CHUNKS) return SOBER_E_WS;
// ... 28 lines not shown
    const bool tani_k = j->variant == SOBER_LEVEL_TANI;
    const int n_chunks = mfma ? sober_level_parts_mfma(j->n_rows, j->pos0, j->count, S)
                              : (tani_k ? sober_level_chunks_tani(j->n_rows, j->pos0, j->count, S)
                                        : sober_level_chunks(j->n_rows, j->pos0, j->count, S));
    if (n_chunks <= 0 || n_chunks > SOBER_LEVEL_MAX_CHUNKS) return n_chunks <= 0 ? n_chunks : SOBER_E_WS;
    LX_EVENTS_BEFORE(j->ev[0], j->ev[1])
    LX_TRY(lx_reduce(j, j->idx, j->pos0, j->count, S, n_chunks, j->partG, j->partTot, ES, stream));
    LX_EVENTS_AFTER(j->ev[0], j->ev[1])
    const int64_t lo = j->pos0 > ES ? j->pos0 : ES;
    const int64_t n_left = j->pos0 + j->count - lo;
    int n_xchunks = 0;
    if (n_left > 0) {
        if (!j->extraG || !j->extraTot) return SOBER_E_ARG;
        n_xchunks = mfma ? sober_level_parts_mfma(j->n_rows, 0, n_left, SOBER_LEVEL_XS)
                         : (tani_k ? sober_level_chunks_tani(j->n_rows, 0, n_left, SOBER_LEVEL_XS)
                                   : sober_level_chunks(j->n_rows, 0, n_left, SOBER_LEVEL_XS));
        if (n_xchunks <= 0 || n_xchunks > SOBER_LEVEL_MAX_CHUNKS) return n_xchunks <= 0 ? n_xchunks : SOBER_E_WS;
        LX_EVENTS_BEFORE(j->ev[2], j->ev[3])
        LX_TRY(lx_reduce(j, j->idx + (lo - j->pos0), 0, n_left, SOBER_LEVEL_XS, n_xchunks, j->extraG, j->extraTot,
                         n_left, stream));
        LX_EVENTS_AFTER(j->ev[2], j->ev[3])
    }
    LX_TRY(sober_sum_partials(j->partG, j->partTot, n_chunks, j->n_rows, S, S, n_left > 0 ? j->extraG : nullptr,
                              n_left > 0 ? j->extraTot : nullptr, n_xchunks, SOBER_LEVEL_XS, j->G, S, j->tot, stream));
    if (j->phase == 1) return 0;
    return sober_dgemm(0, 0, j->n, S, j->n_rows, 1.0, j->P, j->n_rows, j->G, S, 0.0, j->Xtr, S, stream);
}

extern "C" int sober_level_car(const sober_level_job* j, void* stream) {
    if (!j || !j->Xtr || !j->tot || !j->X_tmp || !j->keep_rank || !j->w_star || !j->mu_out || !j->car_ws || !j->h_flags)
        return SOBER_E_ARG;
    const int S = j->S, n = j->n;
    if (!sober_car_supported(S, n + 1)) return SOBER_E_DIM;
    LX_TRY(sober_barycentres(j->Xtr, S, n, S, j->tot, j->X_tmp, stream));
    LX_TRY(sober_car_device_ex(j->X_tmp, n, S, n + 1, j->tot, j->keep_rank, j->w_star, j->keep_rank + S, j->mu_out,
                               nullptr, j->car_ws, j->car_ws_bytes, j->car_mode, stream));
    const hipError_t e = hipMemcpyAsync(j->h_flags, j->keep_rank, sizeof(int32_t) * (size_t)(S + 1),
                                        hipMemcpyDeviceToHost, (hipStream_t)stream);
    return e == hipSuccess ? 0 : (int)e;
}

extern "C" int sober_level_car_retry(sober_level_job* j, void* stream) {
    if (!j || !j->X_tmp || !j->tot || !j->keep_rank || !j->w_star || !j->mu_out || !j->car_ws || !j->h_flags) return SOBER_E_ARG;
    const int S = j->S, n = j->n;
    if (j->car_mode == SOBER_CAR_SAFE || !sober_car_safe_supported(S, n + 1)) return SOBER_E_EXCHANGE;
    j->car_mode = SOBER_CAR_SAFE;
    LX_TRY(sober_car_device_ex(j->X_tmp, n, S, n + 1, j->tot, j->keep_rank, j->w_star, j->keep_rank + S, j->mu_out,
                               nullptr, j->car_ws, j->car_ws_bytes, SOBER_CAR_SAFE, stream));
    hipError_t e = hipMemcpyAsync(j->h_flags, j->keep_rank, sizeof(int32_t) * (size_t)(S + 1), hipMemcpyDeviceToHost,
                                  (hipStream_t)stream);
    if (e == hipSuccess) e = hipStreamSynchronize((hipStream_t)stream);
    if (e != hipSuccess) return (int)e;
    return j->h_flags[S] < 0 ? SOBER_E_EXCHANGE : 0;
}

static int lx_chunks(int n_rows, int64_t e_total, int S) { return sober_level_parts_mfma_cap(n_rows, e_total, S); }

static int lx_loop_queued(sober_level_job* j, const sober_obj_job* oj, int64_t R0, int32_t* idx_a, int32_t* idx_b,
                          int first_sums_ready, void** events, int max_levels, int64_t* level_R, int* done, int64_t* R_out,
                          void* stream) {
    const int S = j->S, n = j->n, b = n + 1;
    *done = 0;
    *R_out = R0;
    int64_t Rlo[SOBER_LEVEL_QUEUE + 1], Rub[SOBER_LEVEL_QUEUE + 1];
    Rlo[0] = Rub[0] = R0;
    int L = 0;
    while (L < SOBER_LEVEL_QUEUE && L < max_levels && Rlo[L] > S) {
        Rlo[L + 1] = (Rlo[L] / S) * b;
        Rub[L + 1] = (Rub[L] / S) * b + (Rlo[L] == Rub[L] ? Rub[L] % S : S - 1);
        ++L;
    }
    if (L < 2) return 0;
    if (!sober_car_supported(S, oj ? b + 1 : b)) return SOBER_E_DIM;
    if (oj && (!sober_null_vector_supported(n) || b + 1 > 512)) return SOBER_E_DIM;
    int D = 0;
    if (first_sums_ready && j->class_depth > 0 && !oj) {
        D = j->class_depth;
        if ((j->variant != SOBER_LEVEL_MFMA && j->variant != SOBER_LEVEL_TANI) || D > SOBER_CLASS_MAX_DEPTH || D >= L ||
            R0 % ((int64_t)S << D) != 0 ||
            !j->Gc[0] || !j->Gc[1] || !j->totc[0] || !j->totc[1] || !j->cls_scale || !j->cls_sof)
            return SOBER_E_ARG;
    }
    hipStream_t st = (hipStream_t)stream;
    if (!first_sums_ready) LX_TRY(sober_set_i64(j->dR, R0, stream));
    hipError_t e = hipSuccess;
    for (int l = 0; l < L; ++l) {
        int32_t* cur = (l & 1) ? idx_b : idx_a;
        int32_t* nxt = (l & 1) ? idx_a : idx_b;
        for (int k = 0; k < 4; ++k) j->ev[k] = events ? events[4 * l + k] : nullptr;
        if (l >= 1 && l <= D) {
            LX_TRY(sober_class_derive_queued(j->Gc[(l - 1) & 1], j->totc[(l - 1) & 1], j->n_rows, S, 1 << (D - l + 1),
                                             j->cls_scale, j->cls_sof, j->Gc[l & 1], j->totc[l & 1], j->G, j->tot, j->dR + l,
                                             stream));
        } else if (!(l == 0 && first_sums_ready)) {
            const bool tani = j->variant == SOBER_LEVEL_TANI;
            const int64_t e_ub = (Rub[l] + S - 1) / S, ex_ub = (S - 1 + SOBER_LEVEL_XS - 1) / SOBER_LEVEL_XS;
            const int nch = tani ? sober_level_chunks_tani_cap(j->n_rows, e_ub, S) : lx_chunks(j->n_rows, e_ub, S);
            const int nxch = tani ? sober_level_chunks_tani_cap(j->n_rows, ex_ub, SOBER_LEVEL_XS) : lx_chunks(j->n_rows, ex_ub, SOBER_LEVEL_XS);
            if (nch <= 0 || nch > SOBER_LEVEL_MAX_CHUNKS || nxch <= 0 || nxch > SOBER_LEVEL_MAX_CHUNKS) return SOBER_E_WS;
            LX_EVENTS_BEFORE(j->ev[0], j->ev[1])
            if (j->ev[0] && j->ev[1]) j->ev_used[0] |= 1ull << l;
            const bool no_left = Rlo[l] == Rub[l] && Rub[l] % S == 0;
            if (tani && !no_left && !sober::switches().level_two_launches) {
                LX_TRY(sober_level_reduce_tani_queued_pair(j->rows, j->rows_norm, j->n_rows, j->cand, j->cand_norm, j->dim, cur,
                                                           Rub[l], S, SOBER_LEVEL_XS, j->mu, j->wmul, j->outputscale, nch,
                                                           j->partG, S, j->partTot, nxch, j->extraG, j->extraTot, j->dR + l,
                                                           stream));
            } else if (tani) {
                LX_TRY(sober_level_reduce_tani_queued(j->rows, j->rows_norm, j->n_rows, j->cand, j->cand_norm, j->dim, cur,
                                                      Rub[l], S, S, 0, j->mu, j->wmul, j->outputscale, nch, j->partG, S,
                                                      j->partTot, j->dR + l, stream));
                if (!no_left) {
                    LX_EVENTS_BEFORE(j->ev[2], j->ev[3])
                    if (j->ev[2] && j->ev[3]) j->ev_used[1] |= 1ull << l;
                    LX_TRY(sober_level_reduce_tani_queued(j->rows, j->rows_norm, j->n_rows, j->cand, j->cand_norm, j->dim, cur,
                                                          S - 1, SOBER_LEVEL_XS, S, 1, j->mu, j->wmul, j->outputscale, nxch,
                                                          j->extraG, SOBER_LEVEL_XS, j->extraTot, j->dR + l, stream));
                }
            } else if (no_left || sober::switches().level_two_launches) {
                LX_TRY(sober_level_reduce_mfma_queued(j->kind, (const double*)j->rows, j->n_rows, (const double*)j->cand,
                                                      j->dim, cur, Rub[l], S, S, 0, j->mu, j->wmul, j->outputscale, nch,
                                                      j->partG, S, j->partTot, j->dR + l, stream));
                if (!no_left) {
                    LX_EVENTS_BEFORE(j->ev[2], j->ev[3])
                    if (j->ev[2] && j->ev[3]) j->ev_used[1] |= 1ull << l;
                    LX_TRY(sober_level_reduce_mfma_queued(j->kind, (const double*)j->rows, j->n_rows, (const double*)j->cand,
                                                          j->dim, cur, S - 1, SOBER_LEVEL_XS, S, 1, j->mu, j->wmul,
                                                          j->outputscale, nxch, j->extraG, SOBER_LEVEL_XS, j->extraTot,
                                                          j->dR + l, stream));
                }
            } else {
                LX_TRY(sober_level_reduce_mfma_queued_pair(j->kind, (const double*)j->rows, j->n_rows, (const double*)j->cand,
                                                           j->dim, cur, Rub[l], S, SOBER_LEVEL_XS, j->mu, j->wmul,
                                                           j->outputscale, nch, j->partG, S, j->partTot, nxch, j->extraG,
                                                           j->extraTot, j->dR + l, stream));
            }
            LX_TRY(sober_sum_partials_queued(j->partG, j->partTot, j->n_rows, S, S, j->extraG, j->extraTot,
                                             SOBER_LEVEL_XS, j->G, S, j->tot, j->dR + l, tani ? 1 : 0, stream));
        }
        if (oj) {
            LX_TRY(sober_dgemm_coldiv_t(n, S, j->n_rows, j->P, j->n_rows, j->G, S, j->tot, oj->X_tmp, n + 1, stream));
            LX_TRY(sober_obj_set_sums_queued(oj->obj, j->mu, cur, S, j->dR + l, (l == 0 && first_sums_ready) ? R0 : (int64_t)-1,
                                             j->tot, oj->X_tmp + n, n + 1, oj->ocol, stream));
            LX_TRY(sober_car_device_ex(oj->X_tmp, n + 1, S, n + 2, j->tot, oj->kr1, oj->w1, oj->nk1, j->mu_out, nullptr,
                                       j->car_ws, j->car_ws_bytes, j->car_mode, stream));
            LX_TRY(sober_null_vector(oj->X_tmp, n + 1, S, n, oj->kr1, oj->nk1, n + 2, oj->null_row, oj->status, stream));
            LX_TRY(sober_second_elimination_rows(oj->null_row, oj->ocol, oj->w1, oj->kr1, oj->nk1, oj->status, n + 2, S,
                                                 j->keep_rank, j->w_star, j->keep_rank + S, stream));
        } else {
            LX_TRY(sober_dgemm_coldiv_t(n, S, j->n_rows, j->P, j->n_rows, j->G, S, j->tot, j->X_tmp, n, stream));
            LX_TRY(sober_car_device_ex(j->X_tmp, n, S, n + 1, j->tot, j->keep_rank, j->w_star, j->keep_rank + S, j->mu_out,
                                       nullptr, j->car_ws, j->car_ws_bytes, j->car_mode, stream));
        }
        LX_TRY(sober_level_update_queued_ex(cur, Rub[l], S, j->keep_rank, j->w_star, j->tot, j->mu, nxt, j->dR + l,
                                            j->dR + l + 1, Rub[l + 1], l < D ? b : 0, j->cls_scale, j->cls_sof,
                                            (l == 0 && first_sums_ready) ? R0 : (int64_t)-1, stream));
    }
    for (int k = 0; k < 4; ++k) j->ev[k] = nullptr;
    e = hipMemcpyAsync(j->h_dR, j->dR, sizeof(int64_t) * (size_t)(L + 1), hipMemcpyDeviceToHost, st);
    if (e != hipSuccess) return (int)e;
    e = hipStreamSynchronize(st);
    if (e != hipSuccess) return (int)e;
    j->h_dR[0] = R0;
    int d = 0;
    while (d < L && j->h_dR[d + 1] >= 0) { level_R[d] = j->h_dR[d]; ++d; }
    *done = d;
    *R_out = j->h_dR[d];
    return 0;
}

extern "C" int sober_level_loop_obj(sober_level_job* j, const sober_obj_job* oj, int64_t R, int32_t* idx_a, int32_t* idx_b,
                                    int first_sums_ready, int max_levels, int64_t* level_R, int32_t* n_levels, int64_t* R_final,
                                    int32_t* in_b, void* stream) {
    if (!j || !oj || !idx_a || !idx_b || !level_R || !n_levels || !R_final || !in_b || !j->mu || R <= 0 || !j->dR || !j->h_dR)
        return SOBER_E_ARG;
    if (!oj->obj || !oj->X_tmp || !oj->ocol || !oj->kr1 || !oj->w1 || !oj->nk1 || !oj->null_row || !oj->status) return SOBER_E_ARG;
    if (j->variant != SOBER_LEVEL_MFMA && j->variant != SOBER_LEVEL_TANI) return SOBER_E_ARG;
    int done = 0;
    int64_t R_after = R;
    j->ev_used[0] = j->ev_used[1] = 0;
    LX_TRY(lx_loop_queued(j, oj, R, idx_a, idx_b, first_sums_ready, nullptr, max_levels, level_R, &done, &R_after, stream));
    *n_levels = done;
    *R_final = R_after;
    *in_b = (done & 1) ? 1 : 0;
    return 0;
}

extern "C" int sober_level_loop(sober_level_job* j, int64_t R, int32_t* idx_a, int32_t* idx_b, int first_sums_ready,
                                void** events, int max_levels, int64_t* level_R, int32_t* n_levels, int64_t* R_final,
                                int32_t* in_b, void* stream) {
    if (!j || !idx_a || !idx_b || !level_R || !n_levels || !R_final || !in_b || !j->h_flags || !j->mu || R <= 0)
        return SOBER_E_ARG;
    const int S = j->S;
    int32_t *cur = idx_a, *nxt = idx_b;
    int levels = 0;
    j->ev_used[0] = j->ev_used[1] = 0;
    if (j->dR && j->h_dR && (j->variant == SOBER_LEVEL_MFMA || (j->variant == SOBER_LEVEL_TANI && !sober::switches().tani_no_queue))) {
        int done = 0;
        int64_t R_after = R;
        LX_TRY(lx_loop_queued(j, nullptr, R, idx_a, idx_b, first_sums_ready, events, max_levels, level_R, &done, &R_after, stream));
        if (done > 0) {
            levels = done;
            R = R_after;
            first_sums_ready = 0;
            if (done & 1) { cur = idx_b; nxt = idx_a; }
        }
    }
    while (R > S) {
        if (levels >= max_levels) return SOBER_E_WS;
        const int64_t E = R / S, r = R - E * S;
        j->idx = cur; j->pos0 = 0; j->count = R; j->E = E;
        j->phase = (levels == 0 && first_sums_ready) ? 2 : 0;
        for (int k = 0; k < 4; ++k) j->ev[k] = (events && levels < max_levels) ? events[4 * levels + k] : nullptr;
        if (j->phase != 2 && levels < 64) {
            if (j->ev[0] && j->ev[1]) j->ev_used[0] |= 1ull << levels;
            if (j->ev[2] && j->ev[3] && r > 0) j->ev_used[1] |= 1ull << levels;
        }
        LX_TRY(sober_level_moments(j, stream));
        LX_TRY(sober_level_car(j, stream));
        const hipError_t e = hipStreamSynchronize((hipStream_t)stream);
        if (e != hipSuccess) return (int)e;
        if (j->h_flags[S] < 0) {
            const int rc = sober_level_car_retry(j, stream);
            if (rc != 0) {
                *n_levels = levels; *R_final = R; *in_b = (cur == idx_b) ? 1 : 0;
                for (int k = 0; k < 4; ++k) j->ev[k] = nullptr;
                j->phase = 0;
                return rc;
            }
        }
        const int n_keep = j->h_flags[S];
        const bool last_kept = j->h_flags[S - 1] >= 0;
        const int64_t R_new = E * n_keep + (last_kept ? r : 0);
        level_R[levels++] = R;
        if (R_new >= R) { *n_levels = levels; return SOBER_E_NOPROGRESS; }
        LX_TRY(sober_level_update(cur, 0, R, S, E, j->keep_rank, j->w_star, j->tot, n_keep, j->mu, nxt, 0, stream));
        int32_t* t = cur; cur = nxt; nxt = t;
        R = R_new;
    }
    for (int k = 0; k < 4; ++k) j->ev[k] = nullptr;
    j->phase = 0;
    *n_levels = levels;
    *R_final = R;
    *in_b = (cur == idx_b) ? 1 : 0;
    return 0;
}

extern "C" int sober_level_final_job(const sober_level_job* j, const sober_final_job* f, const int32_t* idx, int R,
                                     void* stream) {
    if (!j || !f || !f->rows_sc || (!f->cand_sc && (!f->cand_raw || !f->ls || !f->sc_buf)) || !idx || !f->K || !f->mu_live ||
        !f->out_idx || !f->out_w || !j->P || !j->Xtr || !j->X_tmp || !j->keep_rank || !j->w_star || !j->mu_out || !j->car_ws ||
        !j->h_flags || !j->mu)
        return SOBER_E_ARG;
    const int S = j->S, n = j->n;
    if (R <= n + 1 || R > S || f->N <= 0) return SOBER_E_ARG;
    if (!sober_car_supported(R, n + 1)) return SOBER_E_DIM;
    if (f->cand_sc) {
        LX_TRY(sober_pairwise(j->kind, f->rows_sc, f->rows_norm, j->n_rows, f->cand_sc, f->cand_norm, idx, R, f->dt,
                              j->outputscale, f->K, R, stream));
    } else {
        LX_TRY(sober_scale_points_idx(f->cand_raw, idx, R, f->d_raw, f->ld_raw, f->ls, f->ls_len, f->sc_buf, f->dt, j->mu,
                                      f->mu_live, stream));
        LX_TRY(sober_pairwise(j->kind, f->rows_sc, f->rows_norm, j->n_rows, f->sc_buf, nullptr, nullptr, R, f->dt,
                              j->outputscale, f->K, R, stream));
    }
    LX_TRY(sober_dgemm_coldiv_t(n, R, j->n_rows, j->P, j->n_rows, f->K, R, nullptr, j->X_tmp, n, stream));
    if (f->cand_sc) LX_TRY(sober_gather_f64(j->mu, idx, R, f->mu_live, stream));
    LX_TRY(sober_car_device_ex(j->X_tmp, n, R, n + 1, f->mu_live, j->keep_rank, j->w_star, j->keep_rank + S, j->mu_out,
                               nullptr, j->car_ws, j->car_ws_bytes, j->car_mode, stream));
    LX_TRY(sober_final_commit(idx, R, j->keep_rank, j->w_star, j->keep_rank + S, f->row_offset, j->mu, f->N, f->out_idx,
                              f->out_w, stream));
    hipError_t e = hipMemcpyAsync(j->h_flags + S, j->keep_rank + S, sizeof(int32_t), hipMemcpyDeviceToHost, (hipStream_t)stream);
    return e == hipSuccess ? 0 : (int)e;
}

extern "C" int sober_level_final(const sober_level_job* j, const void* rows_sc, const double* rows_norm,
                                 const void* cand_sc, const double* cand_norm, int dt, const int32_t* idx, int R,
                                 int64_t N, int64_t row_offset, double* K, double* mu_live, int64_t* out_idx,
                                 double* out_w, void* stream) {
    if (!cand_sc) return SOBER_E_ARG;
    sober_final_job f = {};
    f.rows_sc = rows_sc; f.rows_norm = rows_norm; f.cand_sc = cand_sc; f.cand_norm = cand_norm; f.dt = dt;
    f.N = N; f.row_offset = row_offset; f.K = K; f.mu_live = mu_live; f.out_idx = out_idx; f.out_w = out_w;
    return sober_level_final_job(j, &f, idx, R, stream);
}

extern "C" int sober_final_job_size(void) { return (int)sizeof(sober_final_job); }

extern "C" int sober_level_loop_final(sober_level_job* j, sober_final_job* f, int64_t R, int32_t* idx_a, int32_t* idx_b,
                                      int first_sums_ready, void** events, int max_levels, int64_t* level_R,
                                      int32_t* n_levels, int64_t* R_final, int32_t* in_b, void* stream) {
    if (f) f->done = 0;
    const int rc = sober_level_loop(j, R, idx_a, idx_b, first_sums_ready, events, max_levels, level_R, n_levels, R_final,
                                    in_b, stream);
    if (rc != 0 || !f) return rc;
    const int S = j->S, n = j->n;
    const int64_t Rf = *R_final;
    if (Rf <= n + 1 || Rf > S) return 0;
    if (j->car_mode != SOBER_CAR_DEFAULT && j->car_mode != SOBER_CAR_SAFE) return 0;
    if (!sober_car_supported((int)Rf, n + 1)) return 0;
    if (j->car_mode == SOBER_CAR_SAFE && !sober_car_safe_supported((int)Rf, n + 1)) return 0;
    LX_TRY(sober_level_final_job(j, f, *in_b ? idx_b : idx_a, (int)Rf, stream));
    const hipError_t e = hipStreamSynchronize((hipStream_t)stream);
    if (e != hipSuccess) return (int)e;
    f->done = 1;
    return 0;
}

extern "C" int sober_record_event_pair(void* ev0, void* ev1, void* stream) {
    if (!ev0 || !ev1) return SOBER_E_ARG;
    hipError_t e = hipEventRecord((hipEvent_t)ev0, (hipStream_t)stream);
    if (e == hipSuccess) e = hipEventRecord((hipEvent_t)ev1, (hipStream_t)stream);
    return e == hipSuccess ? 0 : (int)e;
}

static int64_t lx_survivors_before(int64_t p, int S, int64_t E, const int32_t* kept_prefix, int n_keep, bool last_kept) {
    const int64_t ES = E * S;
    if (p <= ES) return (p / S) * n_keep + kept_prefix[p % S];
    return E * (int64_t)n_keep + (last_kept ? (p - ES) : 0);
}

extern "C" int sober_level_loop_sharded(sober_level_job* j, int rank, int world, int64_t* bounds, int32_t* idx_a,
                                        int32_t* idx_b, int first_sums_ready, sober_allreduce_fn allreduce,
                                        void* comm, int64_t R_stop, int max_levels, int64_t* level_R,
                                        int32_t* n_levels, int32_t* in_b, void* stream) {
    if (!j || !bounds || !idx_a || !idx_b || !allreduce || !level_R || !n_levels || !in_b || !j->h_flags || !j->mu ||
        world <= 0 || rank < 0 || rank >= world || world > 1024)
        return SOBER_E_ARG;
    const int S = j->S, n = j->n;
    if (j->Xtr + (size_t)n * S != j->tot) return SOBER_E_ARG;
    if (!sober_car_supported(S, n + 1)) return SOBER_E_DIM;
    hipStream_t st = (hipStream_t)stream;
    int32_t *cur = idx_a, *nxt = idx_b;
    int levels = 0;
    int32_t kept_prefix[1024 + 1];
    if (S > 1024) return SOBER_E_DIM;
    while (bounds[world] > S && bounds[world] > R_stop) {
        if (levels >= max_levels) return SOBER_E_WS;
        const int64_t R = bounds[world], E = R / S, r = R - E * S;
        const int64_t pos0 = bounds[rank], count = bounds[rank + 1] - bounds[rank];
        if (levels == 0 && first_sums_ready) {
            j->phase = 2;
            LX_TRY(sober_level_moments(j, stream));
        } else if (count > 0) {
            j->idx = cur; j->pos0 = pos0; j->count = count; j->E = E; j->phase = 0;
            LX_TRY(sober_level_moments(j, stream));
        } else {
            hipError_t e = hipMemsetAsync(j->Xtr, 0, sizeof(double) * ((size_t)n * S + S), st);
            if (e != hipSuccess) return (int)e;
        }
        if (world > 1 || comm) LX_TRY(allreduce(comm, j->Xtr, (int64_t)n * S + S, stream));
        LX_TRY(sober_level_car(j, stream));
        hipError_t e = hipStreamSynchronize(st);
        if (e != hipSuccess) return (int)e;
// ... 28 lines not shown
```

sober_amd/csrc/misc.hip:

```cpp
#include "common.hpp"
#include "internal.hpp"

namespace sober {

__global__ void k_scale_points(const double* __restrict__ X, int64_t n, int d, int64_t ldx,
                               const double* __restrict__ ls, int ls_len, double* __restrict__ out,
                               int dt) {
    const int64_t t = (int64_t)blockIdx.x * blockDim.x + threadIdx.x;
    if (t >= n * dt) return;
    const int64_t i = t / dt;
    const int j = (int)(t % dt);
    double v = 0.0;
    if (j < d) v = X[i * ldx + j] / ls[ls_len == 1 ? 0 : j];
    out[t] = v;
}

__global__ void k_scale_points2(const double* __restrict__ Xa, int64_t na, int64_t lda, const double* __restrict__ Xb, int64_t nb,
                                int64_t ldb, int d, const double* __restrict__ ls, int ls_len, double* __restrict__ out, int dt) {
    const int64_t t = (int64_t)blockIdx.x * blockDim.x + threadIdx.x;
    if (t >= (na + nb) * dt) return;
    const int64_t i = t / dt;
    const int j = (int)(t % dt);
    double v = 0.0;
    if (j < d) v = (i < na ? Xa[i * lda + j] : Xb[(i - na) * ldb + j]) / ls[ls_len == 1 ? 0 : j];
// ... 48 lines not shown

template <int KIND, int DT>
__global__ __launch_bounds__(256) void k_kernel_matvec(
    const double* __restrict__ a, const double* __restrict__ an, const double* __restrict__ v,
    int64_t m, const double* __restrict__ b, const double* __restrict__ bn, int64_t n, double os,
    double c0, double* __restrict__ out) {
    constexpr int TA = 64;
    __shared__ double s_a[TA][DT];
    __shared__ double s_v[TA];
    __shared__ double s_n[TA];
    const int64_t j = (int64_t)blockIdx.x * blockDim.x + threadIdx.x;
    double y[DT];
    double ny = 0.0;
    if (j < n) {
#pragma unroll
        for (int q = 0; q < DT; ++q) y[q] = b[j * DT + q];
        if constexpr (KIND == SOBER_KIND_TANIMOTO) ny = bn[j];
    } else {
#pragma unroll
        for (int q = 0; q < DT; ++q) y[q] = 0.0;
    }
    double acc = 0.0;
    for (int64_t i0 = 0; i0 < m; i0 += TA) {
        const int cnt = (int)min((int64_t)TA, m - i0);
        __syncthreads();
        for (int t = threadIdx.x; t < cnt * DT; t += blockDim.x) s_a[t / DT][t % DT] = a[i0 * DT + t];
        if (threadIdx.x < cnt) {
            s_v[threadIdx.x] = v[i0 + threadIdx.x];
            s_n[threadIdx.x] = (KIND == SOBER_KIND_TANIMOTO) ? an[i0 + threadIdx.x] : 0.0;
        }
        __syncthreads();
        for (int i = 0; i < cnt; ++i) {
            double xa[DT];
#pragma unroll
            for (int q = 0; q < DT; ++q) xa[q] = s_a[i][q];
            acc = fma(kern_eval<KIND, DT>(xa, s_n[i], y, ny, os), s_v[i], acc);
        }
    }
    if (j < n) out[j] = c0 + acc;
}

__global__ void k_sum_partials(const double* __restrict__ partG, const double* __restrict__ partTot,
                               int n_chunks, int n_rows, int ldg, int S,
                               const double* __restrict__ extraG, const double* __restrict__ extraTot,
                               int n_xchunks, int n_xcols,
                               double* __restrict__ G, int ldo, double* __restrict__ tot,
                               const int64_t* __restrict__ dR, int chunked) {
    const int s = blockIdx.x * blockDim.x + threadIdx.x;
    const int row = blockIdx.y;
    if (s >= S) return;
    if (dR != nullptr) {
        const int64_t R = __hip_atomic_load(dR, __ATOMIC_RELAXED, __HIP_MEMORY_SCOPE_AGENT);
        if (R <= S) return;
        const int64_t E = R / S, left = R - E * S;
        n_chunks = chunked ? level_chunks_tani_for(n_rows, (R + S - 1) / S, S) : level_parts_mfma_for(n_rows, (R + S - 1) / S, S);
        n_xchunks = left <= 0 ? 0 : (chunked ? level_chunks_tani_for(n_rows, (left + n_xcols - 1) / n_xcols, n_xcols)
                                             : level_parts_mfma_for(n_rows, (left + n_xcols - 1) / n_xcols, n_xcols));
        if (left <= 0) { extraG = nullptr; extraTot = nullptr; }
    }
    const bool fold = (extraG != nullptr) && (s == S - 1);
    if (row < n_rows) {
        double acc = 0.0;
        for (int c = 0; c < n_chunks; ++c) acc += partG[((size_t)c * n_rows + row) * ldg + s];
        if (fold) {
            double ex = 0.0;
            for (int c = 0; c < n_xchunks; ++c)
                for (int q = 0; q < n_xcols; ++q) ex += extraG[((size_t)c * n_rows + row) * n_xcols + q];
            acc += ex;
        }
        G[(size_t)row * ldo + s] = acc;
    } else if (tot != nullptr && partTot != nullptr) {
        double acc = 0.0;
        for (int c = 0; c < n_chunks; ++c) acc += partTot[(size_t)c * ldg + s];
        if (fold && extraTot != nullptr) {
            double ex = 0.0;
            for (int c = 0; c < n_xchunks; ++c)
                for (int q = 0; q < n_xcols; ++q) ex += extraTot[(size_t)c * n_xcols + q];
            acc += ex;
        }
        tot[s] = acc;
    }
}

__global__ void k_barycentres(const double* __restrict__ Xtr, int ldx, int n, int S,
                              const double* __restrict__ tot, double* __restrict__ X_tmp) {
    const int t = blockIdx.x * blockDim.x + threadIdx.x;
    if (t >= n * S) return;
    const int s = t / n, i = t % n;
    double v = Xtr[(size_t)i * ldx + s];
    if (tot) v = v / tot[s];
    X_tmp[t] = v;
}

__global__ void k_level_update(const int32_t* __restrict__ idx_cur, int64_t pos0, int64_t count, int S,
                               int64_t E, const int32_t* __restrict__ keep_rank,
                               const double* __restrict__ w_star, const double* __restrict__ tot,
                               int n_keep, double* __restrict__ mu, int32_t* __restrict__ idx_new,
                               int64_t new_pos0) {
    const int64_t t = (int64_t)blockIdx.x * blockDim.x + threadIdx.x;
    if (t >= count) return;
    const int64_t p = pos0 + t;
    const int64_t ES = E * S;
    const int c = idx_cur[t];
    int s;
    int64_t dst;
    if (p < ES) {
        s = (int)(p % S);
        const int k = keep_rank[s];
        dst = (k >= 0) ? (p / S) * n_keep + k : -1;
    } else {
        s = S - 1;
        dst = (keep_rank[s] >= 0) ? E * n_keep + (p - ES) : -1;
    }
    if (dst >= 0) {
        const int k = keep_rank[s];
        mu[c] = (mu[c] * w_star[k]) / tot[s];
        idx_new[dst - new_pos0] = c;
    } else {
        mu[c] = 0.0;
    }
}

__global__ void k_level_update_queued(const int32_t* __restrict__ idx_cur, int S, const int32_t* __restrict__ keep_rank,
                                      const double* __restrict__ w_star, const double* __restrict__ tot,
                                      double* __restrict__ mu, int32_t* __restrict__ idx_new,
                                      const int64_t* __restrict__ dR_cur, int64_t* __restrict__ dR_next,
                                      int64_t R_ub_next, int need_keep, double* __restrict__ cls_scale,
                                      int32_t* __restrict__ cls_sof, int64_t R_known) {
    const int64_t t = (int64_t)blockIdx.x * blockDim.x + threadIdx.x;
    const int64_t R = R_known >= 0 ? R_known : __hip_atomic_load(dR_cur, __ATOMIC_RELAXED, __HIP_MEMORY_SCOPE_AGENT);
    const int64_t E = R > 0 ? R / S : 0, ES = E * S, r = R - ES;
    const int n_keep = keep_rank[S];
    const bool last_kept = keep_rank[S - 1] >= 0;
    const int64_t R_new = E * (int64_t)n_keep + (last_kept ? r : 0);
    const bool stop = R <= S || n_keep <= 0 || n_keep > S || R_new >= R || R_new > R_ub_next ||
                      (need_keep > 0 && (n_keep != need_keep || r != 0));
    if (t == 0) *dR_next = stop ? -1 : R_new;
    if (stop) return;
    if (cls_scale != nullptr && t < S) {
        const int k = keep_rank[t];
        if (k >= 0) { cls_sof[k] = (int32_t)t; cls_scale[k] = w_star[k] / tot[t]; }
    }
    if (t >= R) return;
    const int c = idx_cur[t];
    int s;
    int64_t dst;
    if (t < ES) {
        s = (int)(t % S);
        const int k = keep_rank[s];
        dst = (k >= 0) ? (t / S) * n_keep + k : -1;
    } else {
        s = S - 1;
        dst = last_kept ? E * n_keep + (t - ES) : -1;
    }
    if (dst >= 0) {
        mu[c] = (mu[c] * w_star[keep_rank[s]]) / tot[s];
        idx_new[dst] = c;
    } else {
        mu[c] = 0.0;
    }
}

__global__ void k_scatter_weights(const int32_t* __restrict__ idx_cur, const int32_t* __restrict__ sel,
                                  const double* __restrict__ w, int n_sel, double* __restrict__ mu,
                                  int64_t* __restrict__ out_idx) {
    const int k = blockIdx.x * blockDim.x + threadIdx.x;
    if (k >= n_sel) return;
    const int c = idx_cur[sel[k]];
    mu[c] = w[k];
    out_idx[k] = c;
}

__global__ void k_gather_f64(const double* __restrict__ src, const int32_t* __restrict__ idx, int64_t n,
                             double* __restrict__ out) {
    const int64_t t = (int64_t)blockIdx.x * blockDim.x + threadIdx.x;
    if (t < n) out[t] = src[idx[t]];
}

__global__ void k_final_scatter(const int32_t* __restrict__ idx, int n, const int32_t* __restrict__ keep_rank,
                                const double* __restrict__ w_star, int64_t row_offset, double* __restrict__ mu,
                                int64_t* __restrict__ out_idx, double* __restrict__ out_w) {
    const int t = blockIdx.x * blockDim.x + threadIdx.x;
    if (t >= n) return;
    const int k = keep_rank[t];
    if (k < 0) return;
    const int c = idx[t];
    const double w = w_star[k];
    mu[c] = w;
    out_idx[k] = (int64_t)c + row_offset;
    out_w[k] = w;
}

__global__ void k_zero_unless_failed(double* __restrict__ mu, int64_t N, const int32_t* __restrict__ n_keep) {
    if (*n_keep < 0) return;
    for (int64_t t = (int64_t)blockIdx.x * blockDim.x + threadIdx.x; t < N; t += (int64_t)gridDim.x * blockDim.x) mu[t] = 0.0;
}
__global__ void k_final_scatter_guarded(const int32_t* __restrict__ idx, int n, const int32_t* __restrict__ keep_rank,
                                        const double* __restrict__ w_star, const int32_t* __restrict__ n_keep,
                                        int64_t row_offset, double* __restrict__ mu, int64_t* __restrict__ out_idx,
                                        double* __restrict__ out_w) {
    if (*n_keep < 0) return;
    const int t = blockIdx.x * blockDim.x + threadIdx.x;
    if (t >= n) return;
    const int k = keep_rank[t];
    if (k < 0) return;
    const int c = idx[t];
    const double w = w_star[k];
    mu[c] = w;
    out_idx[k] = (int64_t)c + row_offset;
    out_w[k] = w;
}

__global__ __launch_bounds__(256) void k_final_commit(const int32_t* __restrict__ idx, int n, const int32_t* __restrict__ keep_rank,
                                                      const double* __restrict__ w_star, const int32_t* __restrict__ n_keep,
                                                      int64_t row_offset, double* __restrict__ mu, int64_t N,
                                                      int64_t* __restrict__ out_idx, double* __restrict__ out_w) {
    const int nk = *n_keep;
    if (nk < 0) return;
    __shared__ int s_c[512];
    __shared__ double s_w[512];
    __shared__ int s_unsorted;
    if (threadIdx.x == 0) s_unsorted = 0;
    __syncthreads();
    for (int t = threadIdx.x; t < n; t += blockDim.x) {
        const int k = keep_rank[t];
        if (k >= 0 && k < 512) { s_c[k] = idx[t]; s_w[k] = w_star[k]; }
    }
    __syncthreads();
    for (int k = threadIdx.x + 1; k < nk; k += blockDim.x)
        if (s_c[k] <= s_c[k - 1]) s_unsorted = 1;
    __syncthreads();
    const bool sorted = s_unsorted == 0;
    if (blockIdx.x == 0)
        for (int k = threadIdx.x; k < nk; k += blockDim.x) { out_idx[k] = (int64_t)s_c[k] + row_offset; out_w[k] = s_w[k]; }
    for (int64_t t = (int64_t)blockIdx.x * blockDim.x + threadIdx.x; t < N; t += (int64_t)gridDim.x * blockDim.x) {
        double v = 0.0;
        if (sorted) {
            int lo = 0, hi = nk;
            while (lo < hi) { const int mid = (lo + hi) >> 1; if ((int64_t)s_c[mid] < t) lo = mid + 1; else hi = mid; }
            if (lo < nk && (int64_t)s_c[lo] == t) v = s_w[lo];
        } else {
            for (int k = 0; k < nk; ++k) if ((int64_t)s_c[k] == t) v = s_w[k];
        }
        mu[t] = v;
    }
}

__global__ __launch_bounds__(256) void k_obj_set_sums(const double* __restrict__ obj, const double* __restrict__ mu,
                                                      const int32_t* __restrict__ idx, int64_t pos0, int64_t count, int S,
                                                      int64_t E, double* __restrict__ out) {
    __shared__ double s_p[256];
    const int s = blockIdx.x, tid = threadIdx.x;
    const int64_t ES = E * (int64_t)S, end = pos0 + count;
    double acc = 0.0;
    int64_t p = pos0 + ((s - pos0 % S) % S + S) % S;
    for (p += (int64_t)tid * S; p < end; p += (int64_t)256 * S) { const int c = idx[p - pos0]; acc += obj[c] * mu[c]; }
    if (s == S - 1)
        for (int64_t q = max(pos0, ES) + tid; q < end; q += 256) { const int c = idx[q - pos0]; acc += obj[c] * mu[c]; }
    s_p[tid] = acc;
    __syncthreads();
    for (int h = 128; h > 0; h >>= 1) {
        if (tid < h) s_p[tid] += s_p[tid + h];
        __syncthreads();
    }
    if (tid == 0) out[s] = s_p[0];
}

__global__ __launch_bounds__(256) void k_obj_set_sums_queued(const double* __restrict__ obj, const double* __restrict__ mu,
                                                             const int32_t* __restrict__ idx, int S, const int64_t* __restrict__ dR,
                                                             int64_t R_known, const double* __restrict__ tot,
                                                             double* __restrict__ xcol, int ldx, double* __restrict__ ocol) {
    __shared__ double s_p[256];
    const int s = blockIdx.x, tid = threadIdx.x;
    const int64_t R = R_known >= 0 ? R_known : __hip_atomic_load(dR, __ATOMIC_RELAXED, __HIP_MEMORY_SCOPE_AGENT);
    if (R <= S) return;
    const int64_t ES = (R / S) * (int64_t)S;
    double acc = 0.0;
    for (int64_t p = s + (int64_t)tid * S; p < R; p += (int64_t)256 * S) { const int c = idx[p]; acc += obj[c] * mu[c]; }
    if (s == S - 1)
        for (int64_t q = ES + tid; q < R; q += 256) { const int c = idx[q]; acc += obj[c] * mu[c]; }
    s_p[tid] = acc;
    __syncthreads();
    for (int h = 128; h > 0; h >>= 1) {
        if (tid < h) s_p[tid] += s_p[tid + h];
        __syncthreads();
    }
    if (tid == 0) {
        const double v = s_p[0] / tot[s];
        xcol[(size_t)s * ldx] = v;
        ocol[s] = v;
    }
}

__global__ void k_projection_left(const double* __restrict__ Ut, int s, int M, const double* __restrict__ mean,
                                  double* __restrict__ P, int ldp) {
    const int t = blockIdx.x * blockDim.x + threadIdx.x;
    if (t >= s * M) return;
    const int r = t / M, c = t - r * M;
    P[(size_t)r * ldp + c] = mean ? Ut[t] * mean[c] : Ut[t];
}

__global__ void k_transpose_projection(const double* __restrict__ Q, int s, int M, const double* __restrict__ mean,
                                       double* __restrict__ Ut, double* __restrict__ P, int ldp) {
    const int t = blockIdx.x * blockDim.x + threadIdx.x;
    if (t >= s * M) return;
    const int r = t / M, c = t - r * M;
    const double v = Q[(size_t)c * s + r];
    Ut[t] = v;
    if (P != nullptr) P[(size_t)r * ldp + c] = mean ? v * mean[c] : v;
}

__global__ void k_i64_to_i32(const int64_t* __restrict__ in, int64_t n, int32_t* __restrict__ out) {
    const int64_t t = (int64_t)blockIdx.x * blockDim.x + threadIdx.x;
    if (t < n) out[t] = (int32_t)in[t];
}

__global__ void k_predict_finish(const double* __restrict__ KX, const double* __restrict__ V, int n_obs,
                                 int64_t N, int64_t ld, const double* __restrict__ mean, double kxx_const,
                                 const double* __restrict__ norms, double outputscale, double noise,
                                 double* __restrict__ var_out, double eta, double* __restrict__ lfi_out,
                                 int log_flag) {
    const int64_t j = (int64_t)blockIdx.x * blockDim.x + threadIdx.x;
    if (j >= N) return;
    double q0 = 0.0, q1 = 0.0;
    int i = 0;
    for (; i + 1 < n_obs; i += 2) {
        q0 = fma(KX[(size_t)i * ld + j], V[(size_t)i * ld + j], q0);
        q1 = fma(KX[(size_t)(i + 1) * ld + j], V[(size_t)(i + 1) * ld + j], q1);
    }
    if (i < n_obs) q0 = fma(KX[(size_t)i * ld + j], V[(size_t)i * ld + j], q0);
    double kxx = kxx_const;
    if (norms != nullptr) {
        const double n2 = norms[j];
        kxx = (n2 + 1e-6) / (1e-6 + n2) * outputscale;
    }
    const double var = kxx - (q0 + q1) + noise;
    var_out[j] = var;
    if (lfi_out != nullptr) {
        const double z = (mean[j] - eta) / sqrt(var);
        double p = 0.5 * erfc(-z * 0.70710678118654752440);
        if (log_flag) p = log(p + 1.1920928955078125e-07);
        lfi_out[j] = p;
    }
}

constexpr int CW_BLOCKS = 256, CW_THREADS = 256;

__global__ __launch_bounds__(CW_THREADS) void k_clean_partial(double* __restrict__ w, int64_t n,
                                                              double eps, double* __restrict__ part) {
    __shared__ double s[CW_THREADS];
    double acc = 0.0;
    for (int64_t i = (int64_t)blockIdx.x * CW_THREADS + threadIdx.x; i < n;
         i += (int64_t)CW_BLOCKS * CW_THREADS) {
        double v = w[i];
        if (v < eps) v = 0.0;
        if (isinf(v)) v = eps;
        if (isnan(v)) v = eps;
        w[i] = v;
        acc += v;
    }
    s[threadIdx.x] = acc;
    __syncthreads();
    for (int o = CW_THREADS / 2; o > 0; o >>= 1) {
        if (threadIdx.x < o) s[threadIdx.x] += s[threadIdx.x + o];
        __syncthreads();
    }
    if (threadIdx.x == 0) part[blockIdx.x] = s[0];
}

__global__ __launch_bounds__(CW_BLOCKS) void k_clean_scale(double* __restrict__ w, int64_t n, const double* __restrict__ part) {
    __shared__ double s[CW_BLOCKS];
    s[threadIdx.x] = part[threadIdx.x];
    __syncthreads();
    for (int o = CW_BLOCKS / 2; o > 0; o >>= 1) {
        if (threadIdx.x < o) s[threadIdx.x] += s[threadIdx.x + o];
        __syncthreads();
    }
    const double tot = s[0];
    const int64_t i = (int64_t)blockIdx.x * blockDim.x + threadIdx.x;
    if (i >= n) return;
    w[i] = (tot != 0.0) ? w[i] / tot : 1.0 / (double)n;
}

__global__ void k_wkde_draw(const double* __restrict__ eps, int64_t n, int d, const int32_t* __restrict__ comp,
                            const double* __restrict__ Xobs, int ldx, const double* __restrict__ L,
                            const double* __restrict__ lo, const double* __restrict__ hi,
                            double* __restrict__ x, int32_t* __restrict__ inside) {
    extern __shared__ double sL[];
    for (int t = threadIdx.x; t < d * d; t += blockDim.x) sL[t] = L[t];
    __syncthreads();
    const int64_t r = (int64_t)blockIdx.x * blockDim.x + threadIdx.x;
    if (r >= n) return;
    const double* e = eps + r * d;
    const double* loc = Xobs + (size_t)comp[r] * ldx;
    bool ok = true;
    for (int k = 0; k < d; ++k) {
        double acc = 0.0;
        for (int j = 0; j <= k; ++j) acc = fma(sL[k * d + j], e[j], acc);
        const double v = loc[k] + acc;
        x[r * d + k] = v;
        if (lo) ok = ok && !(v < lo[k]) && !(v > hi[k]);
    }
    if (inside) inside[r] = ok ? 1 : 0;
}

}

#include <cstdlib>
using namespace sober;

static inline unsigned nblk(int64_t n, int b) { return (unsigned)((n + b - 1) / b); }

extern "C" int sober_abi_version(void) { return SOBER_ABI_VERSION; }
extern "C" int sober_diag_build(void) {
#ifdef SOBER_DIAG_BUILD
    return 1;
#else
    return 0;
#endif
}

namespace sober {
static Switches read_switches() {
    Switches w;
    w.level_two_launches = getenv("SOBER_LEVEL_TWO_LAUNCHES") != nullptr;
    w.tani_no_queue = getenv("SOBER_TANI_NO_QUEUE") != nullptr;
    w.car_force_giveup = getenv("SOBER_CAR_FORCE_GIVEUP") != nullptr;
    w.car_unfused = getenv("SOBER_CAR_UNFUSED") != nullptr;
    w.level_no_classes = getenv("SOBER_LEVEL_NO_CLASSES") != nullptr;
    w.car_exact_ratio = getenv("SOBER_CAR_EXACT_RATIO") != nullptr;
    return w;
}
static Switches g_switches = read_switches();
const Switches& switches() { return g_switches; }
}
extern "C" int sober_reload_switches(void) { sober::g_switches = sober::read_switches(); return 0; }
namespace sober {
LaunchEvents& launch_events() {
    static thread_local LaunchEvents le;
    return le;
}
}
extern "C" int sober_set_launch_events(void* start, void* stop) {
    if ((start == nullptr) != (stop == nullptr)) return SOBER_E_ARG;
    sober::launch_events() = sober::LaunchEvents{(hipEvent_t)start, (hipEvent_t)stop};
    return 0;
}

extern "C" int sober_padded_dim(int d) {
    if (d <= 0) return SOBER_E_ARG;
    const int dts[] = {4, 8, 12, 16, 20, 24, 32};
    for (int v : dts)
        if (d <= v) return v;
    return SOBER_E_DIM;
}

extern "C" int sober_bit_words(int d) {
    if (d <= 0) return SOBER_E_ARG;
    const int w = (d + 63) / 64;
    const int ws[] = {1, 2, 4, 8, 16, 32};
    for (int v : ws)
        if (w <= v) return v;
    return SOBER_E_DIM;
}

__global__ void k_box_muller(const double* __restrict__ u, int64_t numel, double* __restrict__ out) {
    const int64_t t = (int64_t)blockIdx.x * blockDim.x + threadIdx.x;
    const int64_t full = numel / 16;
    const bool tail = (numel % 16) != 0;
    const int64_t npairs = (full + (tail ? 1 : 0)) * 8;
    if (t >= npairs) return;
    const int64_t g = t >> 3;
    const int j = (int)(t & 7);
    const bool is_tail = g == full;
    const int64_t ub = is_tail ? numel : g * 16, ob = is_tail ? numel - 16 : g * 16;
    const double u1 = 1.0 - u[ub + j], u2 = u[ub + j + 8];
    const double radius = sqrt(-2.0 * log(u1));
    const double theta = 6.283185307179586 * u2;
    double sn, cs;
    sincos(theta, &sn, &cs);
    const int64_t keep_below = tail ? numel - 16 : numel;
    if (is_tail || ob + j < keep_below) out[ob + j] = radius * cs;
    if (is_tail || ob + j + 8 < keep_below) out[ob + j + 8] = radius * sn;
}

extern "C" int sober_box_muller(const double* u, int64_t numel, double* out, void* stream) {
    if (!u || !out || numel < 16) return SOBER_E_ARG;
    const int64_t npairs = ((numel + 15) / 16) * 8;
    hipLaunchKernelGGL(k_box_muller, dim3(nblk(npairs, 256)), dim3(256), 0, (hipStream_t)stream, u, numel, out);
    LAUNCH_CHECK();
    return 0;
}

extern "C" int sober_scale_points(const double* X, int64_t n, int d, int64_t ldx,
                                  const double* lengthscale, int ls_len, double* out, int dt,
                                  void* stream) {
    if (!X || !lengthscale || !out || n <= 0 || d <= 0 || dt < d || ldx < d) return SOBER_E_ARG;
    if (ls_len != 1 && ls_len != d) return SOBER_E_ARG;
    hipLaunchKernelGGL(k_scale_points, dim3(nblk(n * dt, 256)), dim3(256), 0, (hipStream_t)stream, X,
                       n, d, ldx, lengthscale, ls_len, out, dt);
    LAUNCH_CHECK();
    return 0;
}

int sober::scale_points2(const double* Xa, int64_t na, int64_t lda, const double* Xb, int64_t nb, int64_t ldb, int d,
                         const double* lengthscale, int ls_len, double* out, int dt, void* stream) {
    if (!Xa || !Xb || !lengthscale || !out || na <= 0 || nb <= 0 || d <= 0 || dt < d || lda < d || ldb < d) return SOBER_E_ARG;
    if (ls_len != 1 && ls_len != d) return SOBER_E_ARG;
    hipLaunchKernelGGL(k_scale_points2, dim3(nblk((na + nb) * dt, 256)), dim3(256), 0, (hipStream_t)stream, Xa, na, lda, Xb, nb,
                       ldb, d, lengthscale, ls_len, out, dt);
    LAUNCH_CHECK();
    return 0;
}

int sober::transpose_projection(const double* Q, int s, int M, const double* mean, double* Ut, double* P, int ldp, void* stream) {
    if (!Q || !Ut || s <= 0 || M <= 0 || (P && ldp < M)) return SOBER_E_ARG;
    hipLaunchKernelGGL(k_transpose_projection, dim3(nblk((int64_t)s * M, 256)), dim3(256), 0, (hipStream_t)stream, Q, s, M, mean,
                       Ut, P, ldp);
    LAUNCH_CHECK();
    return 0;
}

extern "C" int sober_scale_points_idx(const double* X, const int32_t* idx, int64_t n, int d, int64_t ldx,
                                      const double* lengthscale, int ls_len, double* out, int dt, const double* gather_src,
                                      double* gather_out, void* stream) {
    if (!X || !idx || !lengthscale || !out || n <= 0 || d <= 0 || dt < d || ldx < d) return SOBER_E_ARG;
    if ((ls_len != 1 && ls_len != d) || (gather_src && !gather_out)) return SOBER_E_ARG;
    hipLaunchKernelGGL(k_scale_points_idx, dim3(nblk(n * dt, 256)), dim3(256), 0, (hipStream_t)stream, X, idx, n, d, ldx,
                       lengthscale, ls_len, out, dt, gather_src, gather_out);
    LAUNCH_CHECK();
    return 0;
}

extern "C" int sober_pack_bits(const double* X, int64_t n, int d, int64_t ldx, uint64_t* words,
                               int nwords, double* norms, int32_t* bad_flag, void* stream) {
    if (!X || !words || !norms || !bad_flag || n <= 0 || d <= 0 || nwords * 64 < d || ldx < d)
        return SOBER_E_ARG;
    hipLaunchKernelGGL(k_pack_bits, dim3(nblk(n, 4)), dim3(256), 0, (hipStream_t)stream, X, n, d, ldx,
                       words, nwords, norms, bad_flag);
    LAUNCH_CHECK();
    return 0;
}

extern "C" int sober_pairwise(int kind, const void* a, const double* a_norm, int64_t m, const void* b,
                              const double* b_norm, const int32_t* idx, int64_t n, int dt,
                              double outputscale, double* out, int64_t ldo, void* stream) {
    if (!a || !b || !out || m <= 0 || n <= 0 || dt <= 0 || ldo < n || m > 65535) return SOBER_E_ARG;
    if (kind == SOBER_KIND_TANIMOTO && (!a_norm || !b_norm)) return SOBER_E_ARG;
    dim3 grid(nblk(n, 256), (unsigned)m);
    hipStream_t st = (hipStream_t)stream;
    const double* A = (const double*)a;
    const double* B = (const double*)b;
    switch (kind) {
        case SOBER_KIND_RBF:
            hipLaunchKernelGGL(k_pairwise<SOBER_KIND_RBF>, grid, dim3(256), 0, st, A, a_norm, m, B,
                               b_norm, idx, n, dt, outputscale, out, ldo);
            break;
        case SOBER_KIND_MATERN52:
            hipLaunchKernelGGL(k_pairwise<SOBER_KIND_MATERN52>, grid, dim3(256), 0, st, A, a_norm, m, B,
                               b_norm, idx, n, dt, outputscale, out, ldo);
            break;
        case SOBER_KIND_TANIMOTO:
            hipLaunchKernelGGL(k_pairwise<SOBER_KIND_TANIMOTO>, grid, dim3(256), 0, st, A, a_norm, m, B,
                               b_norm, idx, n, dt, outputscale, out, ldo);
            break;
        default: return SOBER_E_ARG;
    }
    LAUNCH_CHECK();
    return 0;
}

template <int KIND, int DT>
static int launch_mv(const void* a, const double* an, const double* v, int64_t m, const void* b,
                     const double* bn, int64_t n, double os, double c0, double* out, hipStream_t st) {
    hipLaunchKernelGGL((k_kernel_matvec<KIND, DT>), dim3(nblk(n, 256)), dim3(256), 0, st,
                       (const double*)a, an, v, m, (const double*)b, bn, n, os, c0, out);
    LAUNCH_CHECK();
    return 0;
}

extern "C" int sober_kernel_matvec(int kind, const void* a, const double* a_norm, const double* v,
                                   int64_t m, const void* b, const double* b_norm, int64_t n, int dt,
                                   double outputscale, double c0, double* out, void* stream) {
    if (!a || !v || !b || !out || m <= 0 || n <= 0) return SOBER_E_ARG;
    if (kind == SOBER_KIND_TANIMOTO && (!a_norm || !b_norm)) return SOBER_E_ARG;
    hipStream_t st = (hipStream_t)stream;
#define MV_CASE(K, D) \
    case D: return launch_mv<K, D>(a, a_norm, v, m, b, b_norm, n, outputscale, c0, out, st);
    switch (kind) {
        case SOBER_KIND_RBF:
            switch (dt) { MV_CASE(SOBER_KIND_RBF, 4) MV_CASE(SOBER_KIND_RBF, 8) MV_CASE(SOBER_KIND_RBF, 12)
                          MV_CASE(SOBER_KIND_RBF, 16) MV_CASE(SOBER_KIND_RBF, 20)
                          MV_CASE(SOBER_KIND_RBF, 24) MV_CASE(SOBER_KIND_RBF, 32)
                          default: return SOBER_E_DIM; }
        case SOBER_KIND_MATERN52:
            switch (dt) { MV_CASE(SOBER_KIND_MATERN52, 4) MV_CASE(SOBER_KIND_MATERN52, 8)
                          MV_CASE(SOBER_KIND_MATERN52, 12) MV_CASE(SOBER_KIND_MATERN52, 16)
                          MV_CASE(SOBER_KIND_MATERN52, 20) MV_CASE(SOBER_KIND_MATERN52, 24)
                          MV_CASE(SOBER_KIND_MATERN52, 32) default: return SOBER_E_DIM; }
        case SOBER_KIND_TANIMOTO:
            switch (dt) { MV_CASE(SOBER_KIND_TANIMOTO, 1) MV_CASE(SOBER_KIND_TANIMOTO, 2)
                          MV_CASE(SOBER_KIND_TANIMOTO, 4) MV_CASE(SOBER_KIND_TANIMOTO, 8)
                          MV_CASE(SOBER_KIND_TANIMOTO, 16) MV_CASE(SOBER_KIND_TANIMOTO, 32)
                          default: return SOBER_E_DIM; }
        default: return SOBER_E_ARG;
    }
#undef MV_CASE
}

extern "C" int sober_level_update_queued(const int32_t* idx_cur, int64_t R_ub, int S, const int32_t* keep_rank,
                                         const double* w_star, const double* tot, double* mu, int32_t* idx_new,
                                         const int64_t* dR_cur, int64_t* dR_next, int64_t R_ub_next, void* stream) {
    if (!idx_cur || !keep_rank || !w_star || !tot || !mu || !idx_new || !dR_cur || !dR_next || R_ub <= 0 || S <= 0)
        return SOBER_E_ARG;
    hipLaunchKernelGGL(k_level_update_queued, dim3(nblk(R_ub, 256)), dim3(256), 0, (hipStream_t)stream, idx_cur, S,
                       keep_rank, w_star, tot, mu, idx_new, dR_cur, dR_next, R_ub_next, 0, (double*)nullptr, (int32_t*)nullptr, (int64_t)-1);
    LAUNCH_CHECK();
    return 0;
}

extern "C" int sober_level_update_queued_ex(const int32_t* idx_cur, int64_t R_ub, int S, const int32_t* keep_rank,
                                            const double* w_star, const double* tot, double* mu, int32_t* idx_new,
                                            const int64_t* dR_cur, int64_t* dR_next, int64_t R_ub_next, int need_keep,
                                            double* cls_scale, int32_t* cls_sof, int64_t R_known, void* stream) {
    if (!idx_cur || !keep_rank || !w_star || !tot || !mu || !idx_new || (!dR_cur && R_known < 0) || !dR_next || R_ub <= 0 ||
        S <= 0 || need_keep < 0 || need_keep > S || (need_keep > 0 && (!cls_scale || !cls_sof)))
        return SOBER_E_ARG;
    hipLaunchKernelGGL(k_level_update_queued, dim3(nblk(R_ub, 256)), dim3(256), 0, (hipStream_t)stream, idx_cur, S,
                       keep_rank, w_star, tot, mu, idx_new, dR_cur, dR_next, R_ub_next, need_keep,
                       need_keep > 0 ? cls_scale : nullptr, need_keep > 0 ? cls_sof : nullptr, R_known);
    LAUNCH_CHECK();
    return 0;
}

extern "C" int sober_level_update_queued_cls(const int32_t* idx_cur, int64_t R_ub, int S, const int32_t* keep_rank,
                                             const double* w_star, const double* tot, double* mu, int32_t* idx_new,
                                             const int64_t* dR_cur, int64_t* dR_next, int64_t R_ub_next, int need_keep,
                                             double* cls_scale, int32_t* cls_sof, void* stream) {
    if (!idx_cur || !keep_rank || !w_star || !tot || !mu || !idx_new || !dR_cur || !dR_next || R_ub < S || S <= 0 ||
        need_keep <= 0 || need_keep > S || !cls_scale || !cls_sof)
        return SOBER_E_ARG;
    hipLaunchKernelGGL(k_level_update_queued, dim3(nblk(R_ub, 256)), dim3(256), 0, (hipStream_t)stream, idx_cur, S,
                       keep_rank, w_star, tot, mu, idx_new, dR_cur, dR_next, R_ub_next, need_keep, cls_scale, cls_sof, (int64_t)-1);
    LAUNCH_CHECK();
    return 0;
}

extern "C" int sober_sum_partials(const double* partG, const double* partTot, int n_chunks,
                                  int n_rows, int ldg, int S, const double* extraG,
                                  const double* extraTot, int n_xchunks, int n_xcols, double* G,
                                  int ldo, double* tot, void* stream) {
    if (!partG || !G || n_chunks <= 0 || n_rows <= 0 || S <= 0 || ldg < S || ldo < S) return SOBER_E_ARG;
    if (extraG && (n_xchunks <= 0 || n_xcols <= 0)) return SOBER_E_ARG;
    dim3 grid(nblk(S, 64), (unsigned)(n_rows + 1));
    hipLaunchKernelGGL(k_sum_partials, grid, dim3(64), 0, (hipStream_t)stream, partG, partTot, n_chunks,
                       n_rows, ldg, S, extraG, extraTot, n_xchunks, n_xcols, G, ldo, tot, (const int64_t*)nullptr, 0);
    LAUNCH_CHECK();
    return 0;
}

extern "C" int sober_sum_partials_queued(const double* partG, const double* partTot, int n_rows, int ldg, int S,
                                         const double* extraG, const double* extraTot, int n_xcols, double* G,
                                         int ldo, double* tot, const int64_t* dR, int chunked, void* stream) {
    if (!partG || !partTot || !extraG || !extraTot || !G || !tot || !dR || n_rows <= 0 || S <= 0 || ldg < S || ldo < S ||
        n_xcols <= 0)
        return SOBER_E_ARG;
    dim3 grid(nblk(S, 64), (unsigned)(n_rows + 1));
    hipLaunchKernelGGL(k_sum_partials, grid, dim3(64), 0, (hipStream_t)stream, partG, partTot, 0, n_rows, ldg, S,
                       extraG, extraTot, 0, n_xcols, G, ldo, tot, dR, chunked);
    LAUNCH_CHECK();
    return 0;
}


extern "C" int sober_barycentres(const double* Xtr, int ldx, int n, int S, const double* tot,
                                 double* X_tmp, void* stream) {
    if (!Xtr || !X_tmp || n <= 0 || S <= 0 || ldx < S) return SOBER_E_ARG;
    hipLaunchKernelGGL(k_barycentres, dim3(nblk((int64_t)n * S, 256)), dim3(256), 0,
                       (hipStream_t)stream, Xtr, ldx, n, S, tot, X_tmp);
    LAUNCH_CHECK();
    return 0;
}

extern "C" int sober_level_update(const int32_t* idx_cur, int64_t pos0, int64_t count, int S, int64_t E,
                                  const int32_t* keep_rank, const double* w_star, const double* tot,
                                  int n_keep, double* mu, int32_t* idx_new, int64_t new_pos0,
                                  void* stream) {
    if (!idx_cur || !keep_rank || !w_star || !tot || !mu || !idx_new) return SOBER_E_ARG;
    if (pos0 < 0 || count <= 0 || S <= 0 || E <= 0 || n_keep < 0 || n_keep > S || new_pos0 < 0)
        return SOBER_E_ARG;
    hipLaunchKernelGGL(k_level_update, dim3(nblk(count, 256)), dim3(256), 0, (hipStream_t)stream,
                       idx_cur, pos0, count, S, E, keep_rank, w_star, tot, n_keep, mu, idx_new, new_pos0);
    LAUNCH_CHECK();
    return 0;
}

extern "C" int sober_scatter_weights(const int32_t* idx_cur, const int32_t* sel, const double* w,
                                     int n_sel, double* mu, int64_t* out_idx, void* stream) {
    if (!idx_cur || !sel || !w || !mu || !out_idx || n_sel <= 0) return SOBER_E_ARG;
    hipLaunchKernelGGL(k_scatter_weights, dim3(nblk(n_sel, 256)), dim3(256), 0, (hipStream_t)stream,
                       idx_cur, sel, w, n_sel, mu, out_idx);
    LAUNCH_CHECK();
    return 0;
}

extern "C" int sober_gather_f64(const double* src, const int32_t* idx, int64_t n, double* out, void* stream) {
    if (!src || !idx || !out || n <= 0) return SOBER_E_ARG;
    hipLaunchKernelGGL(k_gather_f64, dim3(nblk(n, 256)), dim3(256), 0, (hipStream_t)stream, src, idx, n, out);
    LAUNCH_CHECK();
    return 0;
}

extern "C" int sober_final_scatter(const int32_t* idx, int n, const int32_t* keep_rank, const double* w_star,
                                   int64_t row_offset, double* mu, int64_t* out_idx, double* out_w, void* stream) {
    if (!idx || !keep_rank || !w_star || !mu || !out_idx || !out_w || n <= 0) return SOBER_E_ARG;
    hipLaunchKernelGGL(k_final_scatter, dim3(nblk(n, 256)), dim3(256), 0, (hipStream_t)stream, idx, n, keep_rank, w_star,
                       row_offset, mu, out_idx, out_w);
    LAUNCH_CHECK();
    return 0;
}

__global__ void k_set_i64(int64_t* dst, int64_t v) { *dst = v; }

__global__ void k_rank_scatter(const double* __restrict__ X, int ldx, int N, int n, const double* __restrict__ ocol,
                               const int32_t* __restrict__ rank, int n1, double* __restrict__ Xp, double* __restrict__ objp) {
    const int64_t t = (int64_t)blockIdx.x * blockDim.x + threadIdx.x;
    if (t >= (int64_t)N * (n + 1)) return;
    const int s = (int)(t / (n + 1)), j = (int)(t - (int64_t)s * (n + 1));
    const int r = rank[s];
    if (r < 0 || r >= n1) return;
    if (j < n) Xp[(size_t)r * n + j] = X[(size_t)s * ldx + j];
    else objp[r] = ocol[s];
}

extern "C" int sober_rank_scatter(const double* X, int ldx, int N, int n, const double* ocol, const int32_t* rank, int n1,
                                  double* Xp, double* objp, void* stream) {
    if (!X || !ocol || !rank || !Xp || !objp || N <= 0 || n <= 0 || n1 <= 0 || ldx < n) return SOBER_E_ARG;
    hipLaunchKernelGGL(k_rank_scatter, dim3(nblk((int64_t)N * (n + 1), 256)), dim3(256), 0, (hipStream_t)stream, X, ldx, N, n, ocol,
                       rank, n1, Xp, objp);
    LAUNCH_CHECK();
    return 0;
}

extern "C" int sober_set_i64(int64_t* dst, int64_t v, void* stream) {
    if (!dst) return SOBER_E_ARG;
    hipLaunchKernelGGL(k_set_i64, dim3(1), dim3(1), 0, (hipStream_t)stream, dst, v);
    LAUNCH_CHECK();
    return 0;
}

extern "C" int sober_final_commit(const int32_t* idx, int n, const int32_t* keep_rank, const double* w_star,
                                  const int32_t* n_keep, int64_t row_offset, double* mu, int64_t N, int64_t* out_idx,
                                  double* out_w, void* stream) {
    if (!idx || !keep_rank || !w_star || !n_keep || !mu || !out_idx || !out_w || n <= 0 || N <= 0) return SOBER_E_ARG;
    int64_t nb = nblk(N, 256);
    if (nb > 4096) nb = 4096;
    if (n <= 512) {
        hipLaunchKernelGGL(k_final_commit, dim3((unsigned)nb), dim3(256), 0, (hipStream_t)stream, idx, n, keep_rank, w_star, n_keep,
                           row_offset, mu, N, out_idx, out_w);
        LAUNCH_CHECK();
        return 0;
    }
    hipLaunchKernelGGL(k_zero_unless_failed, dim3((unsigned)nb), dim3(256), 0, (hipStream_t)stream, mu, N, n_keep);
    LAUNCH_CHECK();
    hipLaunchKernelGGL(k_final_scatter_guarded, dim3(nblk(n, 256)), dim3(256), 0, (hipStream_t)stream, idx, n, keep_rank,
                       w_star, n_keep, row_offset, mu, out_idx, out_w);
    LAUNCH_CHECK();
    return 0;
}

extern "C" int sober_obj_set_sums(const double* obj, const double* mu, const int32_t* idx, int64_t pos0, int64_t count, int S,
                                  int64_t E, double* out, void* stream) {
    if (!obj || !mu || !idx || !out || pos0 < 0 || count <= 0 || S <= 0 || E < 0) return SOBER_E_ARG;
    hipLaunchKernelGGL(k_obj_set_sums, dim3((unsigned)S), dim3(256), 0, (hipStream_t)stream, obj, mu, idx, pos0, count, S, E, out);
    LAUNCH_CHECK();
    return 0;
}

extern "C" int sober_obj_set_sums_queued(const double* obj, const double* mu, const int32_t* idx, int S, const int64_t* dR,
                                        int64_t R_known, const double* tot, double* xcol, int ldx, double* ocol, void* stream) {
    if (!obj || !mu || !idx || !tot || !xcol || !ocol || S <= 0 || ldx <= 0 || (!dR && R_known < 0)) return SOBER_E_ARG;
    hipLaunchKernelGGL(k_obj_set_sums_queued, dim3((unsigned)S), dim3(256), 0, (hipStream_t)stream, obj, mu, idx, S, dR, R_known,
                       tot, xcol, ldx, ocol);
    LAUNCH_CHECK();
    return 0;
}

extern "C" int sober_projection(const double* Ut, int s, int M, const double* mean, const double* T, int n_obs, double* P,
                                void* stream) {
    if (!Ut || !P || s <= 0 || M <= 0 || (T && n_obs <= 0)) return SOBER_E_ARG;
    const int ldp = M + (T ? n_obs : 0);
    hipLaunchKernelGGL(k_projection_left, dim3(nblk((int64_t)s * M, 256)), dim3(256), 0, (hipStream_t)stream, Ut, s, M,
                       mean, P, ldp);
    LAUNCH_CHECK();
    if (!T) return 0;
    return sober_dgemm(0, 0, s, n_obs, M, -1.0, P, ldp, T, n_obs, 0.0, P + M, ldp, stream);
}

extern "C" int sober_i64_to_i32(const int64_t* in, int64_t n, int32_t* out, void* stream) {
    if (!in || !out || n <= 0) return SOBER_E_ARG;
    hipLaunchKernelGGL(k_i64_to_i32, dim3(nblk(n, 256)), dim3(256), 0, (hipStream_t)stream, in, n, out);
    LAUNCH_CHECK();
    return 0;
}

extern "C" int sober_predict_finish(const double* KX, const double* V, int n_obs, int64_t N, int64_t ld,
                                    const double* mean, double kxx_const, const double* norms,
                                    double outputscale, double noise, double* var_out, double eta,
                                    double* lfi_out, int log_flag, void* stream) {
    if (!KX || !V || !var_out || n_obs <= 0 || N <= 0 || ld < N) return SOBER_E_ARG;
    if (lfi_out && !mean) return SOBER_E_ARG;
    hipLaunchKernelGGL(k_predict_finish, dim3(nblk(N, 256)), dim3(256), 0, (hipStream_t)stream, KX, V, n_obs, N, ld,
                       mean, kxx_const, norms, outputscale, noise, var_out, eta, lfi_out, log_flag);
    LAUNCH_CHECK();
    return 0;
}

extern "C" int64_t sober_reduce_ws_bytes(int64_t n) { (void)n; return (CW_BLOCKS + 1) * sizeof(double); }

extern "C" int sober_cleansing_weights(double* w, int64_t n, double eps, void* ws, int64_t ws_bytes,
                                       void* stream) {
    if (!w || !ws || n <= 0) return SOBER_E_ARG;
    if (ws_bytes < sober_reduce_ws_bytes(n)) return SOBER_E_WS;
    hipStream_t st = (hipStream_t)stream;
    double* part = (double*)ws;
    hipLaunchKernelGGL(k_clean_partial, dim3(CW_BLOCKS), dim3(CW_THREADS), 0, st, w, n, eps, part);
    LAUNCH_CHECK();
    hipLaunchKernelGGL(k_clean_scale, dim3(nblk(n, CW_BLOCKS)), dim3(CW_BLOCKS), 0, st, w, n, part);
    LAUNCH_CHECK();
    return 0;
}

extern "C" int sober_wkde_draw(const double* eps, int64_t n, int d, const int32_t* comp, const double* Xobs,
                               int ldx, const double* L, const double* lo, const double* hi, double* x,
                               int32_t* inside, void* stream) {
    if (!eps || !comp || !Xobs || !L || !x || n <= 0 || d <= 0 || d > 64 || ldx < d) return SOBER_E_ARG;
    if ((lo == nullptr) != (hi == nullptr) || (lo && !inside)) return SOBER_E_ARG;
    hipLaunchKernelGGL(k_wkde_draw, dim3(nblk(n, 256)), dim3(256), (size_t)d * d * sizeof(double),
                       (hipStream_t)stream, eps, n, d, comp, Xobs, ldx, L, lo, hi, x, inside);
    LAUNCH_CHECK();
    return 0;
}
```

sober_amd/csrc/nystrom_exec.cpp:

```cpp
#include <hip/hip_runtime.h>

#include "../../include/sober_hip.h"
#include "internal.hpp"

extern "C" int sober_nystrom_job_size(void) { return (int)sizeof(sober_nystrom_job); }

#define NX_TRY(call)                 \
    do {                             \
        const int rc_ = (call);      \
        if (rc_ != 0) return rc_;    \
    } while (0)
#define NX_HIP(call)                                   \
    do {                                               \
        const hipError_t e_ = (call);                  \
        if (e_ != hipSuccess) return (int)e_;          \
    } while (0)

extern "C" int64_t sober_nystrom_flags_bytes(int n_rungs, int niter) {
    const int64_t n_orth2 = 2 * (1 + 2 * (int64_t)niter);
    return 8 * (n_rungs + 1 + n_orth2) + 4 * (2 + n_rungs + n_orth2);
}

static int nx_orth_halves(const sober_nystrom_job* j, double* Y, double* O, int32_t* info, double* piv, double* ratio, void* stream) {
    const int M = j->M, s = j->s, s1 = (s + 1) / 2, s2 = s - s1;
// ... 2 lines not shown
    double* tail = j->xinv + (size_t)((s + 31) / 32 - 1) * 1024;
    double *piv2 = tail, *ratio2 = tail + 1;
    int32_t* info2 = (int32_t*)(tail + 2);
    NX_TRY(sober_dgemm(1, 0, s1, s1, M, 1.0, Y, s, Y, s, 0.0, G1, s1, stream));
    NX_TRY(sober_cholesky_inv_ratio(G1, s1, s1, 0.0, info, piv, j->xinv, ratio, stream));
    NX_TRY(sober_trsm_blocks(Y, M, s1, s, G1, s1, j->xinv, O, s, stream));
    NX_TRY(sober_dgemm(1, 0, s1, s2, M, 1.0, O, s, Y + s1, s, 0.0, W, s2, stream));
    NX_TRY(sober_dgemm(0, 0, M, s2, s1, -1.0, O, s, W, s2, 1.0, Y + s1, s, stream));
    NX_TRY(sober_dgemm(1, 0, s2, s2, M, 1.0, Y + s1, s, Y + s1, s, 0.0, G1, s2, stream));
    NX_TRY(sober_cholesky_inv_ratio(G1, s2, s2, 0.0, info2, piv2, j->xinv, ratio ? ratio2 : nullptr, stream));
    NX_TRY(sober_trsm_blocks(Y + s1, M, s2, s, G1, s2, j->xinv, O + s1, s, stream));
    return sober::orth_merge(info, piv, ratio, info2, piv2, ratio ? ratio2 : nullptr, stream);
}

static int nx_orth(const sober_nystrom_job* j, double** Y, double** other, int32_t* infos, double* pivs, int slot,
                   int passes, void* stream) {
    const int M = j->M, s = j->s;
    for (int it = 0; it < passes; ++it) {
        if (s > sober_chol_max_n()) {
            NX_TRY(nx_orth_halves(j, *Y, *other, infos + slot + it, pivs + slot + it, passes == 1 ? pivs + slot + 1 : nullptr, stream));
        } else {
            NX_TRY(sober_dgemm(1, 0, s, s, M, 1.0, *Y, s, *Y, s, 0.0, j->Gm, s, stream));
            NX_TRY(sober_cholesky_inv_ratio(j->Gm, s, s, 0.0, infos + slot + it, pivs + slot + it, j->xinv,
                                            passes == 1 ? pivs + slot + 1 : nullptr, stream));
            NX_TRY(sober_trsm_blocks(*Y, M, s, s, j->Gm, s, j->xinv, *other, s, stream));
        }
        double* t = *Y; *Y = *other; *other = t;
    }
    return 0;
}

extern "C" int sober_nystrom_basis(const sober_nystrom_job* j, int phase, void* stream) {
    if (phase < 0 || phase > 2) return SOBER_E_ARG;
    if (!j || !j->G || !j->shifts || (!j->R && phase != 1) || !j->C || !j->chol_work || !j->Y[0] || !j->Y[1] || !j->Gm ||
        !j->xinv || !j->flags_block || !j->h_flags_block || !j->Ut)
        return SOBER_E_ARG;
    const int M = j->M, s = j->s, n_r = j->n_rungs, niter = j->niter;
    if (M <= 0 || s <= 0 || s >= M || s > 2 * sober_chol_max_n() || n_r <= 0 || n_r > 64 || niter < 0 || niter > 8) return SOBER_E_ARG;
    if (M > sober_nystrom_max_n()) return SOBER_E_DIM;
    if (j->flags_bytes < sober_nystrom_flags_bytes(n_r, niter)) return SOBER_E_WS;
    hipStream_t st = (hipStream_t)stream;
    const int n_orth2 = 2 * (1 + 2 * niter);
    double* pivots = (double*)j->flags_block;
    double* pivs_rf = pivots + n_r + 1;
    int32_t* flags = (int32_t*)(pivs_rf + n_orth2);
    int32_t* infos_rf = flags + 2 + n_r;
    if (phase != 2) {
        const bool mc = M <= sober_chol_max_n() && j->probe_mc && j->probe_ws && (j->flags_bytes & 3) == 0 &&
                        j->probe_ws_bytes >= sober_cholesky_probe_mc_ws_bytes(M, n_r);
        if (mc) NX_TRY(sober::nystrom_flags_init(j->flags_block, j->flags_bytes, j->probe_ws, sober::probe_mc_flag_bytes(n_r),
                                                 flags + 2, n_r, stream));
        else NX_HIP(hipMemsetAsync(j->flags_block, 0, (size_t)j->flags_bytes, st));
        NX_TRY(sober_abs_sym_dmax(j->G, M, M, j->C, M, flags, pivots + n_r, stream));
        if (M > sober_chol_max_n()) {
            if (!j->probe_ws) return SOBER_E_ARG;
            NX_TRY(sober_cholesky_probe_batched(j->C, M, M, j->shifts, n_r, j->chol_work, flags + 2, pivots, j->probe_ws,
                                                j->probe_ws_bytes, stream));
        } else if (j->probe_mc) {
            if (!j->probe_ws) return SOBER_E_ARG;
            NX_TRY(sober::cholesky_probe_mc(j->C, M, M, j->shifts, n_r, j->chol_work, flags + 2, pivots, j->probe_ws,
                                            j->probe_ws_bytes, !mc, stream));
        } else {
            NX_TRY(sober_cholesky_probe_piv(j->C, M, M, j->shifts, n_r, j->chol_work, flags + 2, pivots, stream));
        }
        NX_TRY(sober_jitter_ladder_auto(j->C, M, M, flags + 2, n_r, flags + 1, stream));
    }
    if (phase == 1) return 0;
    const int last = 2 * niter;
    double *Q = j->Y[0], *free_buf = j->Y[1];
    NX_TRY(sober_dgemm(0, 0, M, s, M, 1.0, j->C, M, j->R, s, 0.0, Q, s, stream));
    NX_TRY(nx_orth(j, &Q, &free_buf, infos_rf, pivs_rf, 0, last > 0 ? 1 : 2, stream));
    int slot = 2, k = 0;
    for (int it = 0; it < niter; ++it) {
        for (int half = 0; half < 2; ++half) {
            ++k;
            NX_TRY(sober_dgemm(half == 0 ? 1 : 0, 0, M, s, M, 1.0, j->C, M, Q, s, 0.0, free_buf, s, stream));
            double* t = Q; Q = free_buf; free_buf = t;
            NX_TRY(nx_orth(j, &Q, &free_buf, infos_rf, pivs_rf, slot, (half == 1 && k == last) ? 2 : 1, stream));
            slot += 2;
        }
    }
    if (j->P && (j->T ? j->n_obs <= 0 : false)) return SOBER_E_ARG;
    const int ldp = M + (j->T ? j->n_obs : 0);
    NX_TRY(sober::transpose_projection(Q, s, M, j->mean_nys, j->Ut, j->P, ldp, stream));
    if (j->P && j->T) NX_TRY(sober_dgemm(0, 0, s, j->n_obs, M, -1.0, j->P, ldp, j->T, j->n_obs, 0.0, j->P + M, ldp, stream));
    NX_HIP(hipMemcpyAsync(j->h_flags_block, j->flags_block, (size_t)sober_nystrom_flags_bytes(n_r, niter),
                          hipMemcpyDeviceToHost, st));
    return 0;
}

extern "C" int sober_plan_rows(int kind, const double* X_nys, int M, int64_t ld_nys, const double* X_obs, int n_obs,
                               int64_t ld_obs, int d, const double* lengthscale, int ls_len, double outputscale,
                               const double* S_cache, int ld_s, double* rows, int dt, double* Kall, double* W, double* T,
                               double* G, void* stream) {
    if (!X_nys || !lengthscale || !rows || !G || M <= 0 || d <= 0 || n_obs < 0 || dt < d) return SOBER_E_ARG;
    if (kind != SOBER_KIND_RBF && kind != SOBER_KIND_MATERN52) return SOBER_E_ARG;
    if (n_obs == 0) {
        NX_TRY(sober_scale_points(X_nys, M, d, ld_nys, lengthscale, ls_len, rows, dt, stream));
        return sober_pairwise(kind, rows, nullptr, M, rows, nullptr, nullptr, M, dt, outputscale, G, M, stream);
    }
    if (!X_obs || !S_cache || !Kall || !W || !T || ld_s < n_obs) return SOBER_E_ARG;
    NX_TRY(sober::scale_points2(X_nys, M, ld_nys, X_obs, n_obs, ld_obs, d, lengthscale, ls_len, rows, dt, stream));
    NX_TRY(sober_pairwise(kind, rows, nullptr, (int64_t)M + n_obs, rows, nullptr, nullptr, M, dt, outputscale, Kall, M, stream));
    NX_TRY(sober_dgemm(0, 1, n_obs, n_obs, n_obs, 1.0, S_cache, ld_s, S_cache, ld_s, 0.0, W, n_obs, stream));
    const double* KXn = Kall + (size_t)M * M;
    NX_TRY(sober_dgemm(1, 0, M, n_obs, n_obs, 1.0, KXn, M, W, n_obs, 0.0, T, n_obs, stream));
    NX_HIP(hipMemcpyAsync(G, Kall, sizeof(double) * (size_t)M * M, hipMemcpyDeviceToDevice, (hipStream_t)stream));
    return sober_dgemm(0, 0, M, M, n_obs, -1.0, T, n_obs, KXn, M, 1.0, G, M, stream);
}
```

sober_amd/csrc/switches.hpp:

```cpp
#pragma once
namespace sober {
struct Switches {
    bool level_two_launches;
    bool tani_no_queue;
    bool car_force_giveup;
    bool car_unfused;
    bool car_exact_ratio;
    bool level_no_classes;
};
const Switches& switches();
}
```

Baseline: 27.40 million.

## Write readback flags directly to mapped host memory and fuse small copies into kernels

Kernels such as nonzero compaction, the Nystrom projection and the level updates now write their counts and flags straight into a device-visible mirror of pinned host memory, so the separate device-to-host memcpys are no longer issued. The dgemm gains a separate C-input pointer, which removes the device-to-device copy of Kall before the rank update. Partial-sum reduction moves to a flat grid-stride kernel. Level moments can skip class derivation in some modes. These changes cut launches and copies on a latency-bound path, at the cost of relying on host-mapped memory coherence.

```diff
diff --git a/include/sober_hip.h b/include/sober_hip.h
--- a/include/sober_hip.h
+++ b/include/sober_hip.h
@@ -7,7 +7,7 @@
 extern "C" {
 #endif
 
-#define SOBER_ABI_VERSION 7
+#define SOBER_ABI_VERSION 8
 
 #define SOBER_KIND_RBF       0
 #define SOBER_KIND_MATERN52  1
@@ -68,6 +68,8 @@
 int64_t sober_nonzero_ws_bytes(int64_t N);
 int sober_nonzero_i32(const double* mu, int64_t N, int32_t* idx_out, int64_t* count_out, void* ws, int64_t ws_bytes,
                       void* stream);
+int sober_nonzero_i32_host(const double* mu, int64_t N, int32_t* idx_out, int64_t* count_out, int64_t* h_count, void* ws,
+                           int64_t ws_bytes, void* stream);
 
 int sober_level_chunks(int n_rows, int64_t pos0, int64_t count, int S);
 int sober_level_parts_mfma(int n_rows, int64_t pos0, int64_t count, int S);
@@ -76,10 +78,17 @@
 int sober_sum_partials(const double* partG, const double* partTot, int n_chunks, int n_rows,
                        int ldg, int S, const double* extraG, const double* extraTot,
                        int n_xchunks, int n_xcols, double* G, int ldo, double* tot, void* stream);
+int sober_sum_partials_ref(const double* partG, const double* partTot, int n_chunks, int n_rows,
+                           int ldg, int S, const double* extraG, const double* extraTot,
+                           int n_xchunks, int n_xcols, double* G, int ldo, double* tot, const int64_t* dR, int chunked,
+                           void* stream);
 
 int sober_dgemm(int transa, int transb, int m, int n, int k, double alpha,
                 const double* A, int lda, const double* B, int ldb,
                 double beta, double* C, int ldc, void* stream);
+int sober_dgemm_cin(int transa, int transb, int m, int n, int k, double alpha,
+                    const double* A, int lda, const double* B, int ldb,
+                    double beta, const double* Cin, int ldcin, double* C, int ldc, void* stream);
 
 int sober_barycentres(const double* Xtr, int ldx, int n, int S, const double* tot,
                       double* X_tmp, void* stream);
diff --git a/sober_amd/_engine.py b/sober_amd/_engine.py
--- a/sober_amd/_engine.py
+++ b/sober_amd/_engine.py
@@ -271,7 +271,8 @@
             state.update(idx_cur=idx_cur, count=count, pos0=bounds[comm.rank], R=bounds[-1], bounds=bounds)
             cut = sharded and obj is None and self.cutover_R > 0 and state["R"] <= self.cutover_R
             if state["R"] > S and getattr(ops, "level_car", None) is not None and count > 0 and not cut:
-                ops.level_moments(plan, idx_cur, state["pos0"], count, S, state["R"] // S, mu, phase=1, n=n)
+                ops.level_moments(plan, idx_cur, state["pos0"], count, S, state["R"] // S, mu, phase=1, n=n,
+                                  derive=not sharded and obj is None and self.trace is None and not self.force_host_car)
                 state["sums_ready"] = True
 
         def head_once():
diff --git a/sober_amd/_native.py b/sober_amd/_native.py
--- a/sober_amd/_native.py
+++ b/sober_amd/_native.py
@@ -8,7 +8,7 @@
 
 _HERE = os.path.dirname(os.path.abspath(__file__))
 LIB_PATH = os.environ.get("SOBER_HIP_LIB") or os.path.join(_HERE, "libsober_hip.so")
-ABI_VERSION = 7
+ABI_VERSION = 8
 
 KIND_RBF, KIND_MATERN52, KIND_TANIMOTO = 0, 1, 2
 KIND_BY_NAME = {"rbf": KIND_RBF, "matern52": KIND_MATERN52, "tanimoto": KIND_TANIMOTO}
@@ -41,6 +41,7 @@
                                   _f64, _i32, _vp, _i32, _i32, _vp, _i64, _vp]),
     "sober_nonzero_ws_bytes": (_i64, [_i64]),
     "sober_nonzero_i32": (_i32, [_vp, _i64, _vp, _vp, _vp, _i64, _vp]),
+    "sober_nonzero_i32_host": (_i32, [_vp, _i64, _vp, _vp, _vp, _vp, _i64, _vp]),
     "sober_dgemm_coldiv_t": (_i32, [_i32, _i32, _i32, _vp, _i32, _vp, _i32, _vp, _vp, _i32, _vp]),
     "sober_level_chunks": (_i32, [_i32, _i64, _i64, _i32]),
     "sober_level_parts_mfma": (_i32, [_i32, _i64, _i64, _i32]),
@@ -51,6 +52,8 @@
                                        _vp, _i32, _i32, _vp, _i64, _vp]),
     "sober_sum_partials": (_i32, [_vp, _vp, _i32, _i32, _i32, _i32, _vp, _vp, _i32, _i32, _vp, _i32, _vp, _vp]),
     "sober_dgemm": (_i32, [_i32, _i32, _i32, _i32, _i32, _f64, _vp, _i32, _vp, _i32, _f64, _vp, _i32, _vp]),
+    "sober_dgemm_cin": (_i32, [_i32, _i32, _i32, _i32, _i32, _f64, _vp, _i32, _vp, _i32, _f64, _vp, _i32, _vp, _i32, _vp]),
+    "sober_sum_partials_ref": (_i32, [_vp, _vp, _i32, _i32, _i32, _i32, _vp, _vp, _i32, _i32, _vp, _i32, _vp, _vp, _i32, _vp]),
     "sober_barycentres": (_i32, [_vp, _i32, _i32, _i32, _vp, _vp, _vp]),
     "sober_level_update": (_i32, [_vp, _i64, _i64, _i32, _i64, _vp, _vp, _vp, _i32, _vp, _vp, _i64, _vp]),
     "sober_scatter_weights": (_i32, [_vp, _vp, _vp, _i32, _vp, _vp, _vp]),
@@ -392,10 +395,14 @@
     return int(r)
 
 
-def nonzero_i32(mu, idx_out, count_out, ws):
+def nonzero_i32(mu, idx_out, count_out, ws, h_count=None):
     _req(mu, torch.float64, "mu"); _req(idx_out, torch.int32, "idx_out"); _req(count_out, torch.int64, "count_out")
-    _check(load().sober_nonzero_i32(mu.data_ptr(), mu.numel(), idx_out.data_ptr(), count_out.data_ptr(), ws.data_ptr(),
-                                    ws.numel() * ws.element_size(), _stream(mu)), "sober_nonzero_i32")
+    if h_count is not None:
+        _req(h_count, torch.int64, "h_count")
+        if h_count.is_cuda:
+            raise SoberHipError("nonzero_i32: h_count is host memory")
+    _check(load().sober_nonzero_i32_host(mu.data_ptr(), mu.numel(), idx_out.data_ptr(), count_out.data_ptr(), _ptr(h_count),
+                                         ws.data_ptr(), ws.numel() * ws.element_size(), _stream(mu)), "sober_nonzero_i32")
 
 
 def level_chunks(n_rows, pos0, count, S) -> int:
diff --git a/sober_amd/_ops_hip.py b/sober_amd/_ops_hip.py
--- a/sober_amd/_ops_hip.py
+++ b/sober_amd/_ops_hip.py
@@ -31,6 +31,7 @@
         self.last_levels = None
         self._probe_mc = torch.cuda.get_device_properties(self.device).multi_processor_count >= 256
         self.car_mode = nat.CAR_DEFAULT
+        self.pin_readbacks = True
 
     def size_cliff(self, which: str, message: str):
         seen = self.__dict__.setdefault("_cliffs_seen", set())
@@ -77,11 +78,10 @@
         if bufs is None:
             ws = torch.zeros(nat.nonzero_ws_bytes(N), dtype=torch.uint8, device=self.device)
             bufs = self._pin[key] = (ws, torch.zeros(1, dtype=torch.int64, device=self.device),
-                                     torch.zeros(1, dtype=torch.int64).pin_memory())
+                                     torch.zeros(1, dtype=torch.int64, pin_memory=self.pin_readbacks))
         ws, cnt, pin = bufs
         out = torch.empty(N, dtype=torch.int32, device=self.device)
-        nat.nonzero_i32(mu, out, cnt, ws)
-        pin.copy_(cnt, non_blocking=True)
+        nat.nonzero_i32(mu, out, cnt, ws, pin)
         ev = torch.cuda.Event()
         ev.record(torch.cuda.current_stream(self.device))
         return out, pin, ev
diff --git a/sober_amd/_ops_levels.py b/sober_amd/_ops_levels.py
--- a/sober_amd/_ops_levels.py
+++ b/sober_amd/_ops_levels.py
@@ -52,11 +52,11 @@
         w["X_tmp"] = torch.empty(S, n, dtype=f64, device=dev)
         w["keep_rank"] = torch.empty(S + 1, dtype=torch.int32, device=dev)
         w["w_star"], w["mu_out"] = torch.empty(S, dtype=f64, device=dev), torch.empty(S, dtype=f64, device=dev)
-        w["h_flags"] = torch.empty(S + 1, dtype=torch.int32, pin_memory=True)
+        w["h_flags"] = torch.empty(S + 1, dtype=torch.int32, pin_memory=self.pin_readbacks)
         w["h_flags_np"] = w["h_flags"].numpy()
         if job.variant in (nat.LEVEL_MFMA, nat.LEVEL_TANI) and self.queue_levels:
             w["dR"] = torch.empty(nat.LEVEL_QUEUE + 1, dtype=torch.int64, device=dev)
-            w["h_dR"] = torch.zeros(nat.LEVEL_QUEUE + 1, dtype=torch.int64, pin_memory=True)
+            w["h_dR"] = torch.zeros(nat.LEVEL_QUEUE + 1, dtype=torch.int64, pin_memory=self.pin_readbacks)
             job.dR, job.h_dR = w["dR"].data_ptr(), w["h_dR"].data_ptr()
             if S % 2 == 0:
                 cl = 1 << nat.CLASS_MAX_DEPTH
@@ -86,7 +86,7 @@
                              else "the host LAPACK route")
                           + " for that step -- same result, slower")
 
-    def level_moments(self, p: Plan, idx, pos0, count, S, E, mu, phase: int = 0, n: int = None):
+    def level_moments(self, p: Plan, idx, pos0, count, S, E, mu, phase: int = 0, n: int = None, derive: bool = True):
         job = self._job(p, S, n)
         job.phase = phase
         if count <= 0 and phase != 2:
@@ -98,7 +98,7 @@
         nat._req(idx, torch.int32, "idx"); nat._req(mu, torch.float64, "mu")
         job.idx, job.pos0, job.count, job.E, job.mu = idx.data_ptr(), pos0, count, E, mu.data_ptr()
         job.class_depth = 0
-        if phase == 1 and pos0 == 0 and count == E * S and job.Gc[0] and job.dR and self.level_classes:
+        if phase == 1 and derive and pos0 == 0 and count == E * S and job.Gc[0] and job.dR and self.level_classes:
             job.class_depth = int(nat.load().sober_level_class_depth(job.variant, job.n_rows, count, S))
         pair = None
         if self.prof is not None:
diff --git a/sober_amd/_ops_nystrom.py b/sober_amd/_ops_nystrom.py
--- a/sober_amd/_ops_nystrom.py
+++ b/sober_amd/_ops_nystrom.py
@@ -39,7 +39,7 @@
                 "Gm": torch.empty(s, s, dtype=f64, device=dev),
                 "xinv": torch.empty(((s + 31) // 32) * 1024, dtype=f64, device=dev),
                 "flags": torch.empty(nbytes, dtype=torch.uint8, device=dev),
-                "h_flags": torch.empty(nbytes, dtype=torch.uint8, pin_memory=True),
+                "h_flags": torch.empty(nbytes, dtype=torch.uint8, pin_memory=self.pin_readbacks),
                 "Ut": torch.empty(s, M, dtype=f64, device=dev),
             }
             skey = ("shifts", n_r)
diff --git a/sober_amd/csrc/compact.hip b/sober_amd/csrc/compact.hip
--- a/sober_amd/csrc/compact.hip
+++ b/sober_amd/csrc/compact.hip
@@ -1,4 +1,5 @@
 #include "common.hpp"
+#include "internal.hpp"
 
 namespace sober {
 
@@ -12,12 +13,14 @@
 }
 
 __global__ __launch_bounds__(NZ_T) void k_nonzero(const double* __restrict__ mu, int64_t N, int32_t* __restrict__ out,
-                                                  int64_t* __restrict__ count_out, unsigned long long* __restrict__ ws, int nb) {
+                                                  int64_t* __restrict__ count_out, unsigned long long* __restrict__ ws, int nb,
+                                                  int64_t* __restrict__ h_count) {
     __shared__ int s_tile, s_total, s_prefix, s_last;
     __shared__ int s_cnt[NZ_PER * 4];
     if (threadIdx.x == 0) s_tile = (int)atomicAdd((unsigned*)ws, 1u);
     __syncthreads();
     const int tile = s_tile;
+    if (tile >= nb) return;
     const int lane = threadIdx.x & 63, w = threadIdx.x >> 6;
     const int64_t base = (int64_t)tile * NZ_TILE;
     unsigned long long m[NZ_PER];
@@ -73,7 +76,10 @@
             out[prefix + s_cnt[k * 4 + w] + __popcll(m[k] & ((1ull << lane) - 1ull))] = (int32_t)(base + k * NZ_T + threadIdx.x);
     }
     if (threadIdx.x == 0) {
-        if (tile == nb - 1) *count_out = (int64_t)prefix + s_total;
+        if (tile == nb - 1) {
+            *count_out = (int64_t)prefix + s_total;
+            if (h_count != nullptr) *h_count = (int64_t)prefix + s_total;
+        }
         s_last = atomicAdd((unsigned*)(ws + 1), 1u) == (unsigned)(nb - 1);
     }
     __syncthreads();
@@ -91,11 +97,21 @@
 
 extern "C" int sober_nonzero_i32(const double* mu, int64_t N, int32_t* idx_out, int64_t* count_out, void* ws,
                                  int64_t ws_bytes, void* stream) {
+    return sober_nonzero_i32_host(mu, N, idx_out, count_out, nullptr, ws, ws_bytes, stream);
+}
+
+extern "C" int sober_nonzero_i32_host(const double* mu, int64_t N, int32_t* idx_out, int64_t* count_out, int64_t* h_count,
+                                      void* ws, int64_t ws_bytes, void* stream) {
     if (!mu || !idx_out || !count_out || !ws || N <= 0 || N > 0x7fffffffLL) return SOBER_E_ARG;
     if (ws_bytes < sober_nonzero_ws_bytes(N)) return SOBER_E_WS;
     const int nb = (int)((N + sober::NZ_TILE - 1) / sober::NZ_TILE);
+    int64_t* h_dev = (int64_t*)sober::host_mirror(h_count);
     hipLaunchKernelGGL(sober::k_nonzero, dim3((unsigned)nb), dim3(sober::NZ_T), 0, (hipStream_t)stream, mu, N, idx_out, count_out,
-                       (unsigned long long*)ws, nb);
+                       (unsigned long long*)ws, nb, h_dev);
     LAUNCH_CHECK();
+    if (h_count && !h_dev) {
+        const hipError_t e = hipMemcpyAsync(h_count, count_out, sizeof(int64_t), hipMemcpyDeviceToHost, (hipStream_t)stream);
+        if (e != hipSuccess) return (int)e;
+    }
     return 0;
 }
diff --git a/sober_amd/csrc/dgemm.hip b/sober_amd/csrc/dgemm.hip
--- a/sober_amd/csrc/dgemm.hip
+++ b/sober_amd/csrc/dgemm.hip
@@ -16,7 +16,8 @@
                                                double alpha, const double* __restrict__ A, int lda,
                                                const double* __restrict__ B, int ldb, double beta,
                                                double* __restrict__ C, int ldc,
-                                               const double* __restrict__ coldiv, double* __restrict__ Ct, int ldct) {
+                                               const double* __restrict__ coldiv, double* __restrict__ Ct, int ldct,
+                                               const double* __restrict__ Cin, int ldcin) {
     __shared__ double red[SPLIT == 4 ? 3 * 256 : 1];
     const int wave = threadIdx.x >> 6, lane = threadIdx.x & 63;
     int i0, j0, kbeg, kend;
@@ -72,7 +73,7 @@
                 Ct[(size_t)col * ldct + row] = coldiv ? v / coldiv[col] : v;
             } else {
                 double* c = C + (size_t)row * ldc + col;
-                *c = (beta == 0.0) ? v : fma(beta, *c, v);
+                *c = (beta == 0.0) ? v : fma(beta, Cin != nullptr ? Cin[(size_t)row * ldcin + col] : *c, v);
             }
         }
     }
@@ -80,23 +81,35 @@
 
 }
 
-extern "C" int sober_dgemm(int transa, int transb, int m, int n, int k, double alpha, const double* A,
-                           int lda, const double* B, int ldb, double beta, double* C, int ldc,
-                           void* stream) {
+static int dgemm_launch(int transa, int transb, int m, int n, int k, double alpha, const double* A, int lda, const double* B,
+                        int ldb, double beta, const double* Cin, int ldcin, double* C, int ldc, void* stream) {
     if (!A || !B || !C || m <= 0 || n <= 0 || k <= 0) return SOBER_E_ARG;
-    if (lda < (transa ? m : k) || ldb < (transb ? k : n) || ldc < n) return SOBER_E_ARG;
+    if (lda < (transa ? m : k) || ldb < (transb ? k : n) || ldc < n || (Cin && ldcin < n)) return SOBER_E_ARG;
     const long tiles = (long)((n + 15) / 16) * ((m + 15) / 16);
     if (tiles <= 2048 && k >= 64) {
         dim3 grid((n + 15) / 16, (m + 15) / 16);
         hipLaunchKernelGGL(sober::k_dgemm<4>, grid, dim3(256), 0, (hipStream_t)stream, transa, transb, m, n, k,
-                           alpha, A, lda, B, ldb, beta, C, ldc, (const double*)nullptr, (double*)nullptr, 0);
+                           alpha, A, lda, B, ldb, beta, C, ldc, (const double*)nullptr, (double*)nullptr, 0, Cin, ldcin);
     } else {
         dim3 grid((n + 31) / 32, (m + 31) / 32);
         hipLaunchKernelGGL(sober::k_dgemm<1>, grid, dim3(256), 0, (hipStream_t)stream, transa, transb, m, n, k,
-                           alpha, A, lda, B, ldb, beta, C, ldc, (const double*)nullptr, (double*)nullptr, 0);
+                           alpha, A, lda, B, ldb, beta, C, ldc, (const double*)nullptr, (double*)nullptr, 0, Cin, ldcin);
     }
     LAUNCH_CHECK();
     return 0;
+}
+
+extern "C" int sober_dgemm(int transa, int transb, int m, int n, int k, double alpha, const double* A,
+                           int lda, const double* B, int ldb, double beta, double* C, int ldc,
+                           void* stream) {
+    return dgemm_launch(transa, transb, m, n, k, alpha, A, lda, B, ldb, beta, nullptr, 0, C, ldc, stream);
+}
+
+extern "C" int sober_dgemm_cin(int transa, int transb, int m, int n, int k, double alpha, const double* A, int lda,
+                               const double* B, int ldb, double beta, const double* Cin, int ldcin, double* C, int ldc,
+                               void* stream) {
+    if (!Cin) return SOBER_E_ARG;
+    return dgemm_launch(transa, transb, m, n, k, alpha, A, lda, B, ldb, beta, Cin, ldcin, C, ldc, stream);
 }
 
 extern "C" int sober_dgemm_coldiv_t(int m, int n, int k, const double* A, int lda, const double* B, int ldb,
@@ -106,11 +119,11 @@
     if (tiles <= 2048 && k >= 64) {
         dim3 grid((n + 15) / 16, (m + 15) / 16);
         hipLaunchKernelGGL(sober::k_dgemm<4>, grid, dim3(256), 0, (hipStream_t)stream, 0, 0, m, n, k, 1.0, A, lda, B, ldb,
-                           0.0, (double*)nullptr, 0, coldiv, Ct, ldct);
+                           0.0, (double*)nullptr, 0, coldiv, Ct, ldct, (const double*)nullptr, 0);
     } else {
         dim3 grid((n + 31) / 32, (m + 31) / 32);
         hipLaunchKernelGGL(sober::k_dgemm<1>, grid, dim3(256), 0, (hipStream_t)stream, 0, 0, m, n, k, 1.0, A, lda, B, ldb,
-                           0.0, (double*)nullptr, 0, coldiv, Ct, ldct);
+                           0.0, (double*)nullptr, 0, coldiv, Ct, ldct, (const double*)nullptr, 0);
     }
     LAUNCH_CHECK();
     return 0;
diff --git a/sober_amd/csrc/internal.hpp b/sober_amd/csrc/internal.hpp
--- a/sober_amd/csrc/internal.hpp
+++ b/sober_amd/csrc/internal.hpp
@@ -6,7 +6,17 @@
 int scale_points2(const double* Xa, int64_t na, int64_t lda, const double* Xb, int64_t nb, int64_t ldb, int d,
                   const double* lengthscale, int ls_len, double* out, int dt, void* stream);
 
-int transpose_projection(const double* Q, int s, int M, const double* mean, double* Ut, double* P, int ldp, void* stream);
+int transpose_projection(const double* Q, int s, int M, const double* mean, double* Ut, double* P, int ldp, const void* flags,
+                         void* h_flags_dev, int64_t flags_bytes, void* stream);
+
+void* host_mirror(void* h);
+
+int level_update_queued(const int32_t* idx_cur, int64_t R_ub, int S, const int32_t* keep_rank, const double* w_star,
+                        const double* tot, double* mu, int32_t* idx_new, const int64_t* dR_cur, int64_t* dR_next,
+                        int64_t R_ub_next, int need_keep, double* cls_scale, int32_t* cls_sof, int64_t R_known,
+                        int64_t* h_dR_next_dev, void* stream);
+int final_commit(const int32_t* idx, int n, const int32_t* keep_rank, const double* w_star, const int32_t* n_keep,
+                 int64_t row_offset, double* mu, int64_t N, int64_t* out_idx, double* out_w, int32_t* h_n_keep_dev, void* stream);
 
 int64_t probe_mc_flag_bytes(int n_shifts);
 int nystrom_flags_init(void* flags_block, int64_t flags_bytes, void* probe_ws, int64_t ws_flag_bytes, int32_t* info,
diff --git a/sober_amd/csrc/level_exec.cpp b/sober_amd/csrc/level_exec.cpp
--- a/sober_amd/csrc/level_exec.cpp
+++ b/sober_amd/csrc/level_exec.cpp
@@ -3,6 +3,7 @@
 #include <cstdlib>
 
 #include "../../include/sober_hip.h"
+#include "internal.hpp"
 #include "switches.hpp"
 
 extern "C" int sober_level_job_size(void) { return (int)sizeof(sober_level_job); }
@@ -197,6 +198,7 @@
             return SOBER_E_ARG;
     }
     hipStream_t st = (hipStream_t)stream;
+    int64_t* h_dR_dev = (int64_t*)sober::host_mirror(j->h_dR);
     if (!first_sums_ready) LX_TRY(sober_set_i64(j->dR, R0, stream));
     hipError_t e = hipSuccess;
     for (int l = 0; l < L; ++l) {
@@ -267,12 +269,13 @@
             LX_TRY(sober_car_device_ex(j->X_tmp, n, S, n + 1, j->tot, j->keep_rank, j->w_star, j->keep_rank + S, j->mu_out,
                                        nullptr, j->car_ws, j->car_ws_bytes, j->car_mode, stream));
         }
-        LX_TRY(sober_level_update_queued_ex(cur, Rub[l], S, j->keep_rank, j->w_star, j->tot, j->mu, nxt, j->dR + l,
-                                            j->dR + l + 1, Rub[l + 1], l < D ? b : 0, j->cls_scale, j->cls_sof,
-                                            (l == 0 && first_sums_ready) ? R0 : (int64_t)-1, stream));
+        LX_TRY(sober::level_update_queued(cur, Rub[l], S, j->keep_rank, j->w_star, j->tot, j->mu, nxt, j->dR + l,
+                                          j->dR + l + 1, Rub[l + 1], l < D ? b : 0, j->cls_scale, j->cls_sof,
+                                          (l == 0 && first_sums_ready) ? R0 : (int64_t)-1,
+                                          h_dR_dev ? h_dR_dev + l + 1 : nullptr, stream));
     }
     for (int k = 0; k < 4; ++k) j->ev[k] = nullptr;
-    e = hipMemcpyAsync(j->h_dR, j->dR, sizeof(int64_t) * (size_t)(L + 1), hipMemcpyDeviceToHost, st);
+    if (!h_dR_dev) e = hipMemcpyAsync(j->h_dR, j->dR, sizeof(int64_t) * (size_t)(L + 1), hipMemcpyDeviceToHost, st);
     if (e != hipSuccess) return (int)e;
     e = hipStreamSynchronize(st);
     if (e != hipSuccess) return (int)e;
@@ -383,8 +386,10 @@
     if (f->cand_sc) LX_TRY(sober_gather_f64(j->mu, idx, R, f->mu_live, stream));
     LX_TRY(sober_car_device_ex(j->X_tmp, n, R, n + 1, f->mu_live, j->keep_rank, j->w_star, j->keep_rank + S, j->mu_out,
                                nullptr, j->car_ws, j->car_ws_bytes, j->car_mode, stream));
-    LX_TRY(sober_final_commit(idx, R, j->keep_rank, j->w_star, j->keep_rank + S, f->row_offset, j->mu, f->N, f->out_idx,
-                              f->out_w, stream));
+    int32_t* h_dev = (int32_t*)sober::host_mirror(j->h_flags);
+    LX_TRY(sober::final_commit(idx, R, j->keep_rank, j->w_star, j->keep_rank + S, f->row_offset, j->mu, f->N, f->out_idx,
+                               f->out_w, h_dev ? h_dev + S : nullptr, stream));
+    if (h_dev) return 0;
     hipError_t e = hipMemcpyAsync(j->h_flags + S, j->keep_rank + S, sizeof(int32_t), hipMemcpyDeviceToHost, (hipStream_t)stream);
     return e == hipSuccess ? 0 : (int)e;
 }
diff --git a/sober_amd/csrc/misc.hip b/sober_amd/csrc/misc.hip
--- a/sober_amd/csrc/misc.hip
+++ b/sober_amd/csrc/misc.hip
@@ -154,6 +154,50 @@
     }
 }
 
+__global__ __launch_bounds__(256) void k_sum_partials_flat(const double* __restrict__ partG, const double* __restrict__ partTot,
+                                                           int n_chunks, int n_rows, int ldg, int S,
+                                                           const double* __restrict__ extraG, const double* __restrict__ extraTot,
+                                                           int n_xchunks, int n_xcols, double* __restrict__ G, int ldo,
+                                                           double* __restrict__ tot, const int64_t* __restrict__ dR, int chunked) {
+    if (dR != nullptr) {
+        const int64_t R = __hip_atomic_load(dR, __ATOMIC_RELAXED, __HIP_MEMORY_SCOPE_AGENT);
+        if (R <= S) return;
+        const int64_t E = R / S, left = R - E * S;
+        n_chunks = chunked ? level_chunks_tani_for(n_rows, (R + S - 1) / S, S) : level_parts_mfma_for(n_rows, (R + S - 1) / S, S);
+        n_xchunks = left <= 0 ? 0 : (chunked ? level_chunks_tani_for(n_rows, (left + n_xcols - 1) / n_xcols, n_xcols)
+                                             : level_parts_mfma_for(n_rows, (left + n_xcols - 1) / n_xcols, n_xcols));
+        if (left <= 0) { extraG = nullptr; extraTot = nullptr; }
+    }
+    const unsigned total = (unsigned)(n_rows + 1) * (unsigned)S;
+    for (unsigned t = blockIdx.x * blockDim.x + threadIdx.x; t < total; t += gridDim.x * blockDim.x) {
+        const int row = (int)(t / (unsigned)S), s = (int)(t - (unsigned)row * (unsigned)S);
+        const bool fold = (extraG != nullptr) && (s == S - 1);
+        const bool is_tot = row >= n_rows;
+        if (is_tot && (tot == nullptr || partTot == nullptr)) continue;
+        const double* src = is_tot ? partTot + s : partG + (size_t)row * ldg + s;
+        const size_t step = is_tot ? (size_t)ldg : (size_t)n_rows * ldg;
+        double acc = 0.0;
+        for (int c0 = 0; c0 < n_chunks; c0 += 8) {
+            double p[8];
+#pragma unroll
+            for (int u = 0; u < 8; ++u) p[u] = src[(size_t)min(c0 + u, n_chunks - 1) * step];
+#pragma unroll
+            for (int u = 0; u < 8; ++u)
+                if (c0 + u < n_chunks) acc += p[u];
+        }
+        if (fold && !(is_tot && extraTot == nullptr)) {
+            const double* xsrc = is_tot ? extraTot : extraG + (size_t)row * n_xcols;
+            const size_t xstep = is_tot ? (size_t)n_xcols : (size_t)n_rows * n_xcols;
+            double ex = 0.0;
+            for (int c = 0; c < n_xchunks; ++c)
+                for (int q = 0; q < n_xcols; ++q) ex += xsrc[(size_t)c * xstep + q];
+            acc += ex;
+        }
+        if (is_tot) tot[s] = acc;
+        else G[(size_t)row * ldo + s] = acc;
+    }
+}
+
 __global__ void k_barycentres(const double* __restrict__ Xtr, int ldx, int n, int S,
                               const double* __restrict__ tot, double* __restrict__ X_tmp) {
     const int t = blockIdx.x * blockDim.x + threadIdx.x;
@@ -198,7 +242,7 @@
                                       double* __restrict__ mu, int32_t* __restrict__ idx_new,
                                       const int64_t* __restrict__ dR_cur, int64_t* __restrict__ dR_next,
                                       int64_t R_ub_next, int need_keep, double* __restrict__ cls_scale,
-                                      int32_t* __restrict__ cls_sof, int64_t R_known) {
+                                      int32_t* __restrict__ cls_sof, int64_t R_known, int64_t* __restrict__ h_dR_next) {
     const int64_t t = (int64_t)blockIdx.x * blockDim.x + threadIdx.x;
     const int64_t R = R_known >= 0 ? R_known : __hip_atomic_load(dR_cur, __ATOMIC_RELAXED, __HIP_MEMORY_SCOPE_AGENT);
     const int64_t E = R > 0 ? R / S : 0, ES = E * S, r = R - ES;
@@ -207,7 +251,11 @@
     const int64_t R_new = E * (int64_t)n_keep + (last_kept ? r : 0);
     const bool stop = R <= S || n_keep <= 0 || n_keep > S || R_new >= R || R_new > R_ub_next ||
                       (need_keep > 0 && (n_keep != need_keep || r != 0));
-    if (t == 0) *dR_next = stop ? -1 : R_new;
+    if (t == 0) {
+        const int64_t v = stop ? -1 : R_new;
+        *dR_next = v;
+        if (h_dR_next != nullptr) *h_dR_next = v;
+    }
     if (stop) return;
     if (cls_scale != nullptr && t < S) {
         const int k = keep_rank[t];
@@ -263,7 +311,9 @@
     out_w[k] = w;
 }
 
-__global__ void k_zero_unless_failed(double* __restrict__ mu, int64_t N, const int32_t* __restrict__ n_keep) {
+__global__ void k_zero_unless_failed(double* __restrict__ mu, int64_t N, const int32_t* __restrict__ n_keep,
+                                     int32_t* __restrict__ h_n_keep) {
+    if (h_n_keep != nullptr && blockIdx.x == 0 && threadIdx.x == 0) *h_n_keep = *n_keep;
     if (*n_keep < 0) return;
     for (int64_t t = (int64_t)blockIdx.x * blockDim.x + threadIdx.x; t < N; t += (int64_t)gridDim.x * blockDim.x) mu[t] = 0.0;
 }
@@ -286,8 +336,10 @@
 __global__ __launch_bounds__(256) void k_final_commit(const int32_t* __restrict__ idx, int n, const int32_t* __restrict__ keep_rank,
                                                       const double* __restrict__ w_star, const int32_t* __restrict__ n_keep,
                                                       int64_t row_offset, double* __restrict__ mu, int64_t N,
-                                                      int64_t* __restrict__ out_idx, double* __restrict__ out_w) {
+                                                      int64_t* __restrict__ out_idx, double* __restrict__ out_w,
+                                                      int32_t* __restrict__ h_n_keep) {
     const int nk = *n_keep;
+    if (h_n_keep != nullptr && blockIdx.x == 0 && threadIdx.x == 0) *h_n_keep = nk;
     if (nk < 0) return;
     __shared__ int s_c[512];
     __shared__ double s_w[512];
@@ -373,7 +425,10 @@
 }
 
 __global__ void k_transpose_projection(const double* __restrict__ Q, int s, int M, const double* __restrict__ mean,
-                                       double* __restrict__ Ut, double* __restrict__ P, int ldp) {
+                                       double* __restrict__ Ut, double* __restrict__ P, int ldp,
+                                       const uint32_t* __restrict__ flag_src, uint32_t* __restrict__ h_flag_dst, int n_flag_words) {
+    if (h_flag_dst != nullptr && blockIdx.x == 0)
+        for (int w = threadIdx.x; w < n_flag_words; w += blockDim.x) h_flag_dst[w] = flag_src[w];
     const int t = blockIdx.x * blockDim.x + threadIdx.x;
     if (t >= s * M) return;
     const int r = t / M, c = t - r * M;
@@ -500,6 +555,7 @@
     w.car_force_giveup = getenv("SOBER_CAR_FORCE_GIVEUP") != nullptr;
     w.car_unfused = getenv("SOBER_CAR_UNFUSED") != nullptr;
     w.level_no_classes = getenv("SOBER_LEVEL_NO_CLASSES") != nullptr;
+    w.copy_readbacks = getenv("SOBER_COPY_READBACKS") != nullptr;
     w.car_exact_ratio = getenv("SOBER_CAR_EXACT_RATIO") != nullptr;
     return w;
 }
@@ -585,10 +641,22 @@
     return 0;
 }
 
-int sober::transpose_projection(const double* Q, int s, int M, const double* mean, double* Ut, double* P, int ldp, void* stream) {
+void* sober::host_mirror(void* h) {
+    if (!h || switches().copy_readbacks) return nullptr;
+    void* d = nullptr;
+    if (hipHostGetDevicePointer(&d, h, 0) != hipSuccess) {
+        (void)hipGetLastError();
+        return nullptr;
+    }
+    return d;
+}
+
+int sober::transpose_projection(const double* Q, int s, int M, const double* mean, double* Ut, double* P, int ldp,
+                                const void* flags, void* h_flags_dev, int64_t flags_bytes, void* stream) {
     if (!Q || !Ut || s <= 0 || M <= 0 || (P && ldp < M)) return SOBER_E_ARG;
+    if (h_flags_dev && (!flags || flags_bytes <= 0 || (flags_bytes & 3) || flags_bytes > 0x7fffffff)) return SOBER_E_ARG;
     hipLaunchKernelGGL(k_transpose_projection, dim3(nblk((int64_t)s * M, 256)), dim3(256), 0, (hipStream_t)stream, Q, s, M, mean,
-                       Ut, P, ldp);
+                       Ut, P, ldp, (const uint32_t*)flags, (uint32_t*)h_flags_dev, (int)(flags_bytes / 4));
     LAUNCH_CHECK();
     return 0;
 }
@@ -686,23 +754,32 @@
     if (!idx_cur || !keep_rank || !w_star || !tot || !mu || !idx_new || !dR_cur || !dR_next || R_ub <= 0 || S <= 0)
         return SOBER_E_ARG;
     hipLaunchKernelGGL(k_level_update_queued, dim3(nblk(R_ub, 256)), dim3(256), 0, (hipStream_t)stream, idx_cur, S,
-                       keep_rank, w_star, tot, mu, idx_new, dR_cur, dR_next, R_ub_next, 0, (double*)nullptr, (int32_t*)nullptr, (int64_t)-1);
-    LAUNCH_CHECK();
-    return 0;
-}
-
-extern "C" int sober_level_update_queued_ex(const int32_t* idx_cur, int64_t R_ub, int S, const int32_t* keep_rank,
-                                            const double* w_star, const double* tot, double* mu, int32_t* idx_new,
-                                            const int64_t* dR_cur, int64_t* dR_next, int64_t R_ub_next, int need_keep,
-                                            double* cls_scale, int32_t* cls_sof, int64_t R_known, void* stream) {
+                       keep_rank, w_star, tot, mu, idx_new, dR_cur, dR_next, R_ub_next, 0, (double*)nullptr, (int32_t*)nullptr, (int64_t)-1,
+                       (int64_t*)nullptr);
+    LAUNCH_CHECK();
+    return 0;
+}
+
+int sober::level_update_queued(const int32_t* idx_cur, int64_t R_ub, int S, const int32_t* keep_rank, const double* w_star,
+                               const double* tot, double* mu, int32_t* idx_new, const int64_t* dR_cur, int64_t* dR_next,
+                               int64_t R_ub_next, int need_keep, double* cls_scale, int32_t* cls_sof, int64_t R_known,
+                               int64_t* h_dR_next_dev, void* stream) {
     if (!idx_cur || !keep_rank || !w_star || !tot || !mu || !idx_new || (!dR_cur && R_known < 0) || !dR_next || R_ub <= 0 ||
         S <= 0 || need_keep < 0 || need_keep > S || (need_keep > 0 && (!cls_scale || !cls_sof)))
         return SOBER_E_ARG;
     hipLaunchKernelGGL(k_level_update_queued, dim3(nblk(R_ub, 256)), dim3(256), 0, (hipStream_t)stream, idx_cur, S,
                        keep_rank, w_star, tot, mu, idx_new, dR_cur, dR_next, R_ub_next, need_keep,
-                       need_keep > 0 ? cls_scale : nullptr, need_keep > 0 ? cls_sof : nullptr, R_known);
-    LAUNCH_CHECK();
-    return 0;
+                       need_keep > 0 ? cls_scale : nullptr, need_keep > 0 ? cls_sof : nullptr, R_known, h_dR_next_dev);
+    LAUNCH_CHECK();
+    return 0;
+}
+
+extern "C" int sober_level_update_queued_ex(const int32_t* idx_cur, int64_t R_ub, int S, const int32_t* keep_rank,
+                                            const double* w_star, const double* tot, double* mu, int32_t* idx_new,
+                                            const int64_t* dR_cur, int64_t* dR_next, int64_t R_ub_next, int need_keep,
+                                            double* cls_scale, int32_t* cls_sof, int64_t R_known, void* stream) {
+    return sober::level_update_queued(idx_cur, R_ub, S, keep_rank, w_star, tot, mu, idx_new, dR_cur, dR_next, R_ub_next, need_keep,
+                                      cls_scale, cls_sof, R_known, nullptr, stream);
 }
 
 extern "C" int sober_level_update_queued_cls(const int32_t* idx_cur, int64_t R_ub, int S, const int32_t* keep_rank,
@@ -713,9 +790,15 @@
         need_keep <= 0 || need_keep > S || !cls_scale || !cls_sof)
         return SOBER_E_ARG;
     hipLaunchKernelGGL(k_level_update_queued, dim3(nblk(R_ub, 256)), dim3(256), 0, (hipStream_t)stream, idx_cur, S,
-                       keep_rank, w_star, tot, mu, idx_new, dR_cur, dR_next, R_ub_next, need_keep, cls_scale, cls_sof, (int64_t)-1);
-    LAUNCH_CHECK();
-    return 0;
+                       keep_rank, w_star, tot, mu, idx_new, dR_cur, dR_next, R_ub_next, need_keep, cls_scale, cls_sof, (int64_t)-1,
+                       (int64_t*)nullptr);
+    LAUNCH_CHECK();
+    return 0;
+}
+
+static unsigned sum_partials_blocks(int n_rows, int S) {
+    const int64_t nb = ((int64_t)(n_rows + 1) * S + 255) / 256;
+    return (unsigned)(nb < 2048 ? nb : 2048);
 }
 
 extern "C" int sober_sum_partials(const double* partG, const double* partTot, int n_chunks,
@@ -724,9 +807,22 @@
                                   int ldo, double* tot, void* stream) {
     if (!partG || !G || n_chunks <= 0 || n_rows <= 0 || S <= 0 || ldg < S || ldo < S) return SOBER_E_ARG;
     if (extraG && (n_xchunks <= 0 || n_xcols <= 0)) return SOBER_E_ARG;
+    if ((int64_t)(n_rows + 1) * S > 0x7fffffffLL) return SOBER_E_ARG;
+    hipLaunchKernelGGL(k_sum_partials_flat, dim3(sum_partials_blocks(n_rows, S)), dim3(256), 0, (hipStream_t)stream, partG, partTot,
+                       n_chunks, n_rows, ldg, S, extraG, extraTot, n_xchunks, n_xcols, G, ldo, tot, (const int64_t*)nullptr, 0);
+    LAUNCH_CHECK();
+    return 0;
+}
+
+extern "C" int sober_sum_partials_ref(const double* partG, const double* partTot, int n_chunks, int n_rows, int ldg, int S,
+                                      const double* extraG, const double* extraTot, int n_xchunks, int n_xcols, double* G,
+                                      int ldo, double* tot, const int64_t* dR, int chunked, void* stream) {
+    if (!partG || !G || n_rows <= 0 || S <= 0 || ldg < S || ldo < S) return SOBER_E_ARG;
+    if (dR ? (!partTot || !extraG || !extraTot || !tot || n_xcols <= 0)
+           : (n_chunks <= 0 || (extraG && (n_xchunks <= 0 || n_xcols <= 0)))) return SOBER_E_ARG;
     dim3 grid(nblk(S, 64), (unsigned)(n_rows + 1));
-    hipLaunchKernelGGL(k_sum_partials, grid, dim3(64), 0, (hipStream_t)stream, partG, partTot, n_chunks,
-                       n_rows, ldg, S, extraG, extraTot, n_xchunks, n_xcols, G, ldo, tot, (const int64_t*)nullptr, 0);
+    hipLaunchKernelGGL(k_sum_partials, grid, dim3(64), 0, (hipStream_t)stream, partG, partTot, dR ? 0 : n_chunks, n_rows, ldg, S,
+                       extraG, extraTot, dR ? 0 : n_xchunks, n_xcols, G, ldo, tot, dR, chunked);
     LAUNCH_CHECK();
     return 0;
 }
@@ -735,11 +831,10 @@
                                          const double* extraG, const double* extraTot, int n_xcols, double* G,
                                          int ldo, double* tot, const int64_t* dR, int chunked, void* stream) {
     if (!partG || !partTot || !extraG || !extraTot || !G || !tot || !dR || n_rows <= 0 || S <= 0 || ldg < S || ldo < S ||
-        n_xcols <= 0)
+        n_xcols <= 0 || (int64_t)(n_rows + 1) * S > 0x7fffffffLL)
         return SOBER_E_ARG;
-    dim3 grid(nblk(S, 64), (unsigned)(n_rows + 1));
-    hipLaunchKernelGGL(k_sum_partials, grid, dim3(64), 0, (hipStream_t)stream, partG, partTot, 0, n_rows, ldg, S,
-                       extraG, extraTot, 0, n_xcols, G, ldo, tot, dR, chunked);
+    hipLaunchKernelGGL(k_sum_partials_flat, dim3(sum_partials_blocks(n_rows, S)), dim3(256), 0, (hipStream_t)stream, partG, partTot,
+                       0, n_rows, ldg, S, extraG, extraTot, 0, n_xcols, G, ldo, tot, dR, chunked);
     LAUNCH_CHECK();
     return 0;
 }
@@ -824,16 +919,22 @@
 extern "C" int sober_final_commit(const int32_t* idx, int n, const int32_t* keep_rank, const double* w_star,
                                   const int32_t* n_keep, int64_t row_offset, double* mu, int64_t N, int64_t* out_idx,
                                   double* out_w, void* stream) {
+    return sober::final_commit(idx, n, keep_rank, w_star, n_keep, row_offset, mu, N, out_idx, out_w, nullptr, stream);
+}
+
+int sober::final_commit(const int32_t* idx, int n, const int32_t* keep_rank, const double* w_star, const int32_t* n_keep,
+                        int64_t row_offset, double* mu, int64_t N, int64_t* out_idx, double* out_w, int32_t* h_n_keep_dev,
+                        void* stream) {
     if (!idx || !keep_rank || !w_star || !n_keep || !mu || !out_idx || !out_w || n <= 0 || N <= 0) return SOBER_E_ARG;
     int64_t nb = nblk(N, 256);
     if (nb > 4096) nb = 4096;
     if (n <= 512) {
         hipLaunchKernelGGL(k_final_commit, dim3((unsigned)nb), dim3(256), 0, (hipStream_t)stream, idx, n, keep_rank, w_star, n_keep,
-                           row_offset, mu, N, out_idx, out_w);
+                           row_offset, mu, N, out_idx, out_w, h_n_keep_dev);
         LAUNCH_CHECK();
         return 0;
     }
-    hipLaunchKernelGGL(k_zero_unless_failed, dim3((unsigned)nb), dim3(256), 0, (hipStream_t)stream, mu, N, n_keep);
+    hipLaunchKernelGGL(k_zero_unless_failed, dim3((unsigned)nb), dim3(256), 0, (hipStream_t)stream, mu, N, n_keep, h_n_keep_dev);
     LAUNCH_CHECK();
     hipLaunchKernelGGL(k_final_scatter_guarded, dim3(nblk(n, 256)), dim3(256), 0, (hipStream_t)stream, idx, n, keep_rank,
                        w_star, n_keep, row_offset, mu, out_idx, out_w);
diff --git a/sober_amd/csrc/nystrom_exec.cpp b/sober_amd/csrc/nystrom_exec.cpp
--- a/sober_amd/csrc/nystrom_exec.cpp
+++ b/sober_amd/csrc/nystrom_exec.cpp
@@ -108,10 +108,13 @@
     }
     if (j->P && (j->T ? j->n_obs <= 0 : false)) return SOBER_E_ARG;
     const int ldp = M + (j->T ? j->n_obs : 0);
-    NX_TRY(sober::transpose_projection(Q, s, M, j->mean_nys, j->Ut, j->P, ldp, stream));
+    void* h_dev = sober::host_mirror(j->h_flags_block);
+    NX_TRY(sober::transpose_projection(Q, s, M, j->mean_nys, j->Ut, j->P, ldp, j->flags_block, h_dev,
+                                       sober_nystrom_flags_bytes(n_r, niter), stream));
     if (j->P && j->T) NX_TRY(sober_dgemm(0, 0, s, j->n_obs, M, -1.0, j->P, ldp, j->T, j->n_obs, 0.0, j->P + M, ldp, stream));
-    NX_HIP(hipMemcpyAsync(j->h_flags_block, j->flags_block, (size_t)sober_nystrom_flags_bytes(n_r, niter),
-                          hipMemcpyDeviceToHost, st));
+    if (!h_dev)
+        NX_HIP(hipMemcpyAsync(j->h_flags_block, j->flags_block, (size_t)sober_nystrom_flags_bytes(n_r, niter),
+                              hipMemcpyDeviceToHost, st));
     return 0;
 }
 
@@ -131,6 +134,6 @@
     NX_TRY(sober_dgemm(0, 1, n_obs, n_obs, n_obs, 1.0, S_cache, ld_s, S_cache, ld_s, 0.0, W, n_obs, stream));
     const double* KXn = Kall + (size_t)M * M;
     NX_TRY(sober_dgemm(1, 0, M, n_obs, n_obs, 1.0, KXn, M, W, n_obs, 0.0, T, n_obs, stream));
-    NX_HIP(hipMemcpyAsync(G, Kall, sizeof(double) * (size_t)M * M, hipMemcpyDeviceToDevice, (hipStream_t)stream));
-    return sober_dgemm(0, 0, M, M, n_obs, -1.0, T, n_obs, KXn, M, 1.0, G, M, stream);
+    if (G == Kall) return sober_dgemm(0, 0, M, M, n_obs, -1.0, T, n_obs, KXn, M, 1.0, G, M, stream);
+    return sober_dgemm_cin(0, 0, M, M, n_obs, -1.0, T, n_obs, KXn, M, 1.0, Kall, M, G, M, stream);
 }
diff --git a/sober_amd/csrc/switches.hpp b/sober_amd/csrc/switches.hpp
--- a/sober_amd/csrc/switches.hpp
+++ b/sober_amd/csrc/switches.hpp
@@ -7,6 +7,7 @@
     bool car_unfused;
     bool car_exact_ratio;
     bool level_no_classes;
+    bool copy_readbacks;
 };
 const Switches& switches();
 }
```

New measurement: 27.58 million (median of 4 runs). No clear change (+0.7%).
